# kspalaiologos/bzip3

Hardware: AMD Instinct MI355X
Metric: MiB/s encode+decode round-trip, 8 MiB blocks (higher is better)
Workload: dtype u8

## Files before the change

bzip3_amd/__init__.py:

```python
import ctypes as C
import os

_HERE = os.path.dirname(os.path.abspath(__file__))
LIB_PATH = os.path.join(_HERE, "lib", "libbzip3.so")

BZ3_OK = 0
BZ3_ERR_OUT_OF_BOUNDS = -1
BZ3_ERR_BWT = -2
BZ3_ERR_CRC = -3
BZ3_ERR_MALFORMED_HEADER = -4
BZ3_ERR_TRUNCATED_DATA = -5
BZ3_ERR_DATA_TOO_BIG = -6
BZ3_ERR_INIT = -7
BZ3_ERR_DATA_SIZE_TOO_SMALL = -8

T_NAMES = ["crc", "rle", "lzp", "bwt", "cm", "copy", "_6", "_7"]

_lib = None


def _declare(L, strict=True):
    vp, i32, u32, sz = C.c_void_p, C.c_int32, C.c_uint32, C.c_size_t
    sig = {
        "bz3_version": (C.c_char_p, []),
        "bz3_last_error": (C.c_int8, [vp]),
        "bz3_strerror": (C.c_char_p, [vp]),
        "bz3_new": (vp, [i32]),
        "bz3_free": (None, [vp]),
        "bz3_bound": (sz, [sz]),
        "bz3_compress": (C.c_int, [u32, vp, vp, sz, C.POINTER(sz)]),
        "bz3_decompress": (C.c_int, [vp, vp, sz, C.POINTER(sz)]),
        "bz3_min_memory_needed": (sz, [i32]),
        "bz3_encode_block": (i32, [vp, vp, i32]),
        "bz3_decode_block": (i32, [vp, vp, sz, i32, i32]),
        "bz3_encode_blocks": (None, [vp, vp, vp, i32]),
        "bz3_decode_blocks": (None, [vp, vp, vp, vp, vp, i32]),
        "bz3_orig_size_sufficient_for_decode": (C.c_int, [vp, sz, i32]),
        "bz3_hip_device_count": (C.c_int, []),
        "bz3_hip_bind_device": (C.c_int, [C.c_int]),
        "bz3_hip_state_device": (C.c_int, [vp]),
        "bz3_hip_set_cm_mode": (C.c_int, [C.c_int]),
        "bz3_hip_cm_blocks_given_up": (C.c_uint, []),
        "bz3_hip_cm_blocks_routed_full": (C.c_uint, []),
        "bz3_hip_debug_bwt_big_rounds": (None, [C.c_int]),
        "bz3_hip_debug_set_unbwt_log_stride": (None, [C.c_int]),
        "bz3_hip_debug_peak_concurrent_groups": (C.c_int, [C.c_int]),
        "bz3_hip_debug_front_end_ring": (C.c_int, []),
        "bz3_hip_debug_arena_swap_buffers": (C.c_int, [C.c_int]),
        "bz3_hip_cm_variant_for": (C.c_int, [C.c_int, C.c_int, C.c_int]),
        "bz3_hip_set_lean_states": (C.c_int, [C.c_int]),
        "bz3_hip_release_cached_memory": (None, []),
        "bz3_hip_set_keep_workspace": (C.c_int, [C.c_int]),
        "bz3_hip_set_front_end_duo": (C.c_int, [C.c_int]),
        "bz3_hip_set_workspace_headroom": (None, [C.c_longlong]),
        "bz3_hip_workspace_headroom": (sz, []),
        "bz3_hip_debug_headroom_events": (C.c_uint, [C.c_int, C.POINTER(C.c_uint)]),
        "bz3_hip_debug_ring_contexts": (sz, [sz, sz, sz, sz, sz, sz, C.c_int, sz]),
        "bz3_hip_debug_arena_slack": (sz, [sz]),
        "bz3_hip_debug_cm_launches": (C.c_uint, [C.c_int]),
        "bz3_hip_debug_workspace_bytes": (sz, [sz, C.c_int]),
        "bz3_hip_debug_cached_bytes": (sz, [C.c_int]),
        "bz3_hip_encode_block_device": (i32, [vp, vp, i32]),
        "bz3_hip_decode_block_device": (i32, [vp, vp, sz, i32, i32]),
        "bz3_hip_encode_blocks_device": (None, [vp, vp, vp, i32]),
        "bz3_hip_decode_blocks_device": (None, [vp, vp, vp, vp, vp, i32]),
        "bz3_hip_compress_device": (C.c_int, [u32, vp, vp, sz, C.POINTER(sz)]),
        "bz3_hip_decompress_device": (C.c_int, [vp, vp, sz, C.POINTER(sz)]),
        "bz3_hip_frame_decoded_size_device": (C.c_int, [vp, sz, C.POINTER(sz)]),
        "bz3_hip_compress_device_many": (C.c_int, [u32, i32, C.POINTER(vp), C.POINTER(sz), C.POINTER(vp), C.POINTER(sz), C.POINTER(C.c_int)]),
        "bz3_hip_decompress_device_many": (C.c_int, [i32, C.POINTER(vp), C.POINTER(sz), C.POINTER(vp), C.POINTER(sz), C.POINTER(C.c_int)]),
        "bz3_hip_frame_decoded_sizes_device": (C.c_int, [i32, C.POINTER(vp), C.POINTER(sz), C.POINTER(sz), C.POINTER(C.c_int)]),
        "bz3_hip_debug_copy_segments": (i32, [vp, vp, C.POINTER(C.c_uint64), i32]),
        "bz3_hip_compress_device_planes": (C.c_int, [u32, u32, vp, vp, sz, C.POINTER(sz)]),
        "bz3_hip_decompress_device_planes": (C.c_int, [u32, vp, vp, sz, C.POINTER(sz)]),
        "bz3_hip_compress_device_planes_many": (C.c_int, [u32, i32, C.POINTER(u32), C.POINTER(vp), C.POINTER(sz), C.POINTER(vp), C.POINTER(sz), C.POINTER(C.c_int)]),
        "bz3_hip_decompress_device_planes_many": (C.c_int, [i32, C.POINTER(u32), C.POINTER(vp), C.POINTER(sz), C.POINTER(vp), C.POINTER(sz), C.POINTER(C.c_int)]),
        "bz3_hip_debug_planes": (i32, [vp, vp, C.POINTER(C.c_uint64), i32]),
        "bz3_hip_compress_device_delta": (C.c_int, [u32, u32, vp, vp, vp, sz, C.POINTER(sz)]),
        "bz3_hip_decompress_device_delta": (C.c_int, [u32, vp, vp, sz, vp, sz, C.POINTER(sz)]),
        "bz3_hip_compress_device_delta_many": (C.c_int, [u32, i32, C.POINTER(u32), C.POINTER(vp), C.POINTER(vp), C.POINTER(sz), C.POINTER(vp), C.POINTER(sz), C.POINTER(C.c_int)]),
        "bz3_hip_decompress_device_delta_many": (C.c_int, [i32, C.POINTER(u32), C.POINTER(vp), C.POINTER(sz), C.POINTER(vp), C.POINTER(sz), C.POINTER(vp), C.POINTER(sz), C.POINTER(C.c_int)]),
        "bz3_hip_crc32c_device": (C.c_int, [vp, sz, u32, C.POINTER(u32)]),
        "bz3_hip_crc32c_device_many": (C.c_int, [i32, C.POINTER(vp), C.POINTER(sz), C.POINTER(u32), C.POINTER(u32)]),
        "bz3_hip_debug_crc_launches": (C.c_uint, [C.c_int]),
        "bz3_hip_debug_delta": (i32, [vp, vp, vp, C.POINTER(C.c_uint64), i32]),
        "bz3_hip_decompress_device_range": (C.c_int, [u32, vp, sz, C.c_uint64, vp, sz, vp, C.POINTER(sz)]),
        "bz3_hip_decompress_device_range_many": (C.c_int, [i32, C.POINTER(u32), C.POINTER(vp), C.POINTER(sz), C.POINTER(C.c_uint64), C.POINTER(vp), C.POINTER(sz),
                                                           C.POINTER(vp), C.POINTER(sz), C.POINTER(C.c_int)]),
        "bz3_hip_debug_range": (i32, [vp, vp, vp, C.POINTER(C.c_uint64), i32]),
        "bz3_hip_decompress_device_strided": (C.c_int, [u32, vp, sz, C.c_uint64, C.c_uint64, C.c_uint64, C.c_uint64, vp, sz, vp, C.POINTER(sz)]),
        "bz3_hip_decompress_device_strided_many": (C.c_int, [i32, C.POINTER(u32), C.POINTER(vp), C.POINTER(sz), C.POINTER(C.c_uint64), C.POINTER(vp), C.POINTER(sz),
                                                             C.POINTER(vp), C.POINTER(sz), C.POINTER(C.c_int)]),
        "bz3_hip_debug_strided": (i32, [vp, vp, vp, C.POINTER(C.c_uint64), i32]),
        "bz3_hip_decompress_device_select": (C.c_int, [u32, vp, sz, C.c_uint64, C.c_uint64, C.c_uint64, C.c_uint64, C.POINTER(C.c_uint64), vp, sz, vp, C.POINTER(sz)]),
        "bz3_hip_decompress_device_select_many": (C.c_int, [i32, C.POINTER(u32), C.POINTER(vp), C.POINTER(sz), C.POINTER(C.c_uint64), C.POINTER(C.POINTER(C.c_uint64)),
                                                            C.POINTER(vp), C.POINTER(sz), C.POINTER(vp), C.POINTER(sz), C.POINTER(C.c_int)]),
        "bz3_hip_debug_select": (i32, [vp, vp, vp, C.POINTER(C.c_uint64), i32, C.POINTER(C.c_uint64), C.c_uint64]),
        "bz3_hip_update_device_range": (C.c_int, [u32, vp, sz, C.c_uint64, vp, sz, vp, vp, C.POINTER(sz)]),
        "bz3_hip_update_device_range_many": (C.c_int, [i32, C.POINTER(u32), C.POINTER(vp), C.POINTER(sz), C.POINTER(C.c_uint64), C.POINTER(vp), C.POINTER(sz), C.POINTER(vp),
                                                       C.POINTER(vp), C.POINTER(sz), C.POINTER(C.c_int)]),
        "bz3_hip_debug_patch": (i32, [vp, vp, vp, C.POINTER(C.c_uint64), i32]),
        "bz3_hip_last_timings": (None, [vp, C.POINTER(C.c_float)]),
        "bz3_hip_last_bwt_stats": (None, [vp, C.POINTER(i32), C.POINTER(i32), C.POINTER(C.c_uint64)]),
        "bz3_hip_stage_crc32c": (u32, [vp, sz, u32]),
        "bz3_hip_stage_mrle_encode": (i32, [vp, i32, vp]),
        "bz3_hip_stage_mrle_decode": (C.c_int, [vp, vp, i32, i32]),
        "bz3_hip_stage_lzp_encode": (i32, [vp, i32, vp]),
        "bz3_hip_stage_lzp_decode": (i32, [vp, i32, vp, i32]),
        "bz3_hip_debug_lzp_encode": (i32, [vp, i32, vp, vp]),
        "bz3_hip_stage_bwt": (i32, [vp, vp, i32]),
        "bz3_hip_stage_unbwt": (i32, [vp, vp, i32, i32]),
        "bz3_hip_debug_unbwt_many": (i32, [vp, vp, vp, vp, i32]),
        "bz3_hip_debug_bwt_many": (i32, [vp, vp, vp, vp, i32]),
        "bz3_hip_debug_set_bwt_batch": (None, [C.c_int]),
        "bz3_hip_stage_last_ms": (C.c_float, []),
        "bz3_hip_debug_sort_u32": (i32, [vp, u32, C.c_int, C.c_int, vp, vp]),
        "bz3_hip_debug_scan_u32": (i32, [vp, u32, vp]),
        "bz3_hip_debug_cu_masks": (i32, [C.c_int, C.c_int, vp, vp]),
        "bz3_hip_set_collect_window_us": (None, [C.c_int]),
        "bz3_hip_debug_collected_batches": (C.c_uint, [C.c_int, C.POINTER(C.c_uint)]),
        "bz3_hip_stage_cm_encode": (i32, [vp, i32, vp]),
        "bz3_hip_stage_cm_decode": (None, [vp, i32, vp, i32]),
        "bz3_hip_stage_cm_decode_many": (C.c_float, [vp, i32, vp, i32, i32, vp]),
        "bz3_hip_stage_cm_encode_many": (C.c_float, [vp, i32, vp, C.POINTER(i32), i32]),
        "bz3_hip_encode_stream": (C.c_int, [C.c_int, C.c_int, i32, i32]),
        "bz3_hip_decode_stream": (C.c_int, [C.c_int, C.c_int, i32]),
    }
    for name, (res, args) in sig.items():
        if not strict and not hasattr(L, name):
            continue
        fn = getattr(L, name)
        fn.restype = res
        fn.argtypes = args
    return L


EXPORTED_SYMBOLS = None


def _share_hip_runtime_with_torch():
    if os.environ.get("BZ3_HIP_SYSTEM_RUNTIME") == "1":
        return
    try:
        import importlib.util

        spec = importlib.util.find_spec("torch")
        if spec is None or not spec.origin:
            return
        cand = os.path.join(os.path.dirname(spec.origin), "lib", "libamdhip64.so")
        if os.path.exists(cand):
            C.CDLL(cand, mode=C.RTLD_GLOBAL)
    except Exception:
        pass


def load(path=None):
    global _lib
    if _lib is not None and path is None:
        return _lib
    if path is None:
        _share_hip_runtime_with_torch()
    p = path or LIB_PATH
    if not os.path.exists(p):
        raise RuntimeError(
            f"{p} is missing: the HIP extension has not been built (python -m bzip3_amd.build). "
            "bzip3_amd has no CPU or PyTorch fallback by design."
        )
    L = _declare(C.CDLL(p), strict=path is None)
    if path is None:
        _lib = L
    return L


def _cbuf(data, cap):
    cap = max(1, cap)
    if len(data) == cap:
        return (C.c_uint8 * cap).from_buffer_copy(data)
    buf = (C.c_uint8 * cap)()
    if len(data):
        C.memmove(buf, data if isinstance(data, bytes) else bytes(data), len(data))
    return buf


class StageApi:

    def __init__(self, lib=None):
        self.lib = lib or load()

    def crc32c(self, data, init=1):
        return self.lib.bz3_hip_stage_crc32c(_cbuf(data, len(data)), len(data), init)

    def mrle_encode(self, data):
        out = (C.c_uint8 * (len(data) + 64))()
        n = self.lib.bz3_hip_stage_mrle_encode(_cbuf(data, len(data)), len(data), out)
        return C.string_at(out, n)

    def mrle_decode(self, data, outlen, maxin=None):
        maxin = len(data) if maxin is None else maxin
        out = (C.c_uint8 * max(1, outlen))()
        rc = self.lib.bz3_hip_stage_mrle_decode(_cbuf(data, len(data)), out, outlen, maxin)
        return rc, C.string_at(out, outlen)

    def lzp_encode(self, data):
        out = (C.c_uint8 * (len(data) + 64))()
        n = self.lib.bz3_hip_stage_lzp_encode(_cbuf(data, len(data)), len(data), out)
        return n, (C.string_at(out, n) if n > 0 else b"")

    def lzp_encode_stats(self, data):
        out = (C.c_uint8 * (len(data) + 64))()
        st = (C.c_uint32 * 6)()
        n = self.lib.bz3_hip_debug_lzp_encode(_cbuf(data, len(data)), len(data), out, st)
        keys = ("end_pos", "n_matches", "iterations", "evaluated", "event_cap", "window_positions")
        return n, (C.string_at(out, n) if n > 0 else b""), dict(zip(keys, (int(x) for x in st)))

    def lzp_decode(self, data, maxout):
        out = (C.c_uint8 * max(8, maxout))()
        n = self.lib.bz3_hip_stage_lzp_decode(_cbuf(data, len(data)), len(data), out, maxout)
        return n, (C.string_at(out, n) if n > 0 else b"")

    def bwt(self, data):
        out = (C.c_uint8 * max(1, len(data)))()
        idx = self.lib.bz3_hip_stage_bwt(_cbuf(data, len(data)), out, len(data))
        return idx, C.string_at(out, len(data))

    def unbwt(self, data, idx):
        out = (C.c_uint8 * max(1, len(data)))()
        rc = self.lib.bz3_hip_stage_unbwt(_cbuf(data, len(data)), out, len(data), idx)
        return rc, C.string_at(out, len(data))

    def bwt_many(self, blocks):
        k = len(blocks)
        ins = [_cbuf(d, len(d)) for d in blocks]
        outs = [(C.c_uint8 * max(1, len(d)))() for d in blocks]
        inp = (C.c_void_p * max(1, k))(*[C.cast(b, C.c_void_p) for b in ins])
        outp = (C.c_void_p * max(1, k))(*[C.cast(b, C.c_void_p) for b in outs])
        n = (C.c_int32 * max(1, k))(*[len(d) for d in blocks])
        idx = (C.c_int32 * max(1, k))()
        rc = self.lib.bz3_hip_debug_bwt_many(inp, outp, n, idx, k)
        return rc, [(int(i), C.string_at(o, len(d))) for i, o, d in zip(idx, outs, blocks)]

    def unbwt_many(self, jobs):
        k = len(jobs)
        ins = [_cbuf(d, len(d)) for d, _ in jobs]
        outs = [(C.c_uint8 * max(1, len(d)))() for d, _ in jobs]
        inp = (C.c_void_p * max(1, k))(*[C.cast(b, C.c_void_p) for b in ins])
        outp = (C.c_void_p * max(1, k))(*[C.cast(b, C.c_void_p) for b in outs])
        n = (C.c_int32 * max(1, k))(*[len(d) for d, _ in jobs])
        idx = (C.c_int32 * max(1, k))(*[i for _, i in jobs])
        rc = self.lib.bz3_hip_debug_unbwt_many(inp, outp, n, idx, k)
        return rc, [C.string_at(o, len(d)) for o, (d, _) in zip(outs, jobs)]

    def cm_encode(self, data):
        out = (C.c_uint8 * (len(data) + len(data) // 50 + 64))()
        n = self.lib.bz3_hip_stage_cm_encode(_cbuf(data, len(data)), len(data), out)
        return C.string_at(out, n)

    def cm_decode(self, data, n):
        out = (C.c_uint8 * max(1, n))()
        self.lib.bz3_hip_stage_cm_decode(_cbuf(data, len(data)), len(data), out, n)
        return C.string_at(out, n)


class State:

    def __init__(self, block_size, lib=None):
        self.lib = lib or load()
        self.block_size = block_size
        self.ptr = self.lib.bz3_new(block_size)
        if not self.ptr:
            raise RuntimeError(f"bz3_new({block_size}) returned NULL (invalid size, no HIP device, or out of device memory)")

    def close(self):
        if self.ptr:
            self.lib.bz3_free(self.ptr)
            self.ptr = None

    def __del__(self):
        try:
            self.close()
        except Exception:
            pass

    def __enter__(self):
        return self

    def __exit__(self, *a):
        self.close()

    @property
    def last_error(self):
        return self.lib.bz3_last_error(self.ptr)

    def strerror(self):
        return self.lib.bz3_strerror(self.ptr).decode()

    def timings(self):
        t = (C.c_float * 8)()
        self.lib.bz3_hip_last_timings(self.ptr, t)
        return {T_NAMES[i]: t[i] for i in range(6)}

    def bwt_stats(self):
        r, p, e = C.c_int32(), C.c_int32(), C.c_uint64()
        self.lib.bz3_hip_last_bwt_stats(self.ptr, C.byref(r), C.byref(p), C.byref(e))
        return {"rounds": r.value, "radix_passes": p.value, "sorted_elements": e.value}

    def encode_block(self, data):
        cap = self.lib.bz3_bound(max(len(data), self.block_size)) + 64
        buf = _cbuf(data, cap)
        n = self.lib.bz3_encode_block(self.ptr, buf, len(data))
        return n, self.last_error, (C.string_at(buf, n) if n > 0 else b"")

    def decode_block(self, data, orig_size, buffer_size=None, comp_size=None):
        cap = self.lib.bz3_bound(self.block_size) + 64
        buffer_size = cap if buffer_size is None else buffer_size
        comp_size = len(data) if comp_size is None else comp_size
        buf = _cbuf(data, max(cap, buffer_size, len(data) + 1))
        n = self.lib.bz3_decode_block(self.ptr, buf, buffer_size, comp_size, orig_size)
        return n, self.last_error, (C.string_at(buf, n) if n > 0 else b"")


def encode_block(data, block_size, lib=None):
    with State(block_size, lib) as st:
        return st.encode_block(data)


def decode_block(data, orig_size, block_size, lib=None, **kw):
    with State(block_size, lib) as st:
        return st.decode_block(data, orig_size, **kw)


class Bz3Error(RuntimeError):

    def __init__(self, code, what, out=None, index=None, codes=None, outs=None):
        super().__init__(f"{what} failed with {code} ({_ERR_NAMES.get(code, 'unknown error')})" + ("" if index is None else f" at frame {index}"))
        self.code = code
        self.out = out
        self.index = index
        self.codes = codes
        self.outs = outs


_ERR_NAMES = {v: k for k, v in globals().items() if k.startswith("BZ3_ERR_")}


def _device_u8(x, what):
    import torch

    if not isinstance(x, torch.Tensor) or x.device.type != "cuda" or x.dtype != torch.uint8 or not x.is_contiguous():
        raise TypeError(f"{what} must be a contiguous torch.uint8 tensor on a GPU")
    return x


def _planes_arg(planes, n):
    ks = [int(planes)] * n if isinstance(planes, int) else [int(k) for k in planes]
    if len(ks) != n:
        raise ValueError(f"planes: {len(ks)} element sizes for {n} tensors")
    for k in ks:
        if k not in (1, 2, 4, 8):
            raise ValueError(f"planes must be 1, 2, 4 or 8, not {k}")
    return ks


def _base_u8(base, x, what, same_size=True):
    if base is None:
        return None
    base = _device_u8(base, what)
    if base.device != x.device:
        raise ValueError(f"{what} is on {base.device}, the tensor on {x.device}")
    if same_size and base.numel() != x.numel():
        raise ValueError(f"{what} holds {base.numel()} bytes, the tensor {x.numel()}")
    return base


def _bases_arg(bases, n):
    bases = [None] * n if bases is None else list(bases)
    if len(bases) != n:
        raise ValueError(f"bases: {len(bases)} entries for {n} tensors")
    return bases


def _ptrs_or_null(ts):
    return (C.c_void_p * len(ts))(*[None if t is None else t.data_ptr() for t in ts])


def compress_tensor(x, block_size=16 << 20, lib=None, planes=1, base=None):
    import torch

    x = _device_u8(x, "x")
    (k,) = _planes_arg(planes, 1)
    base = _base_u8(base, x, "base")
    L = lib or load()
    n = x.numel()
    out = torch.empty(L.bz3_bound(n), dtype=torch.uint8, device=x.device)
    size = C.c_size_t(out.numel())
    torch.cuda.synchronize(x.device)
    rc = L.bz3_hip_compress_device_delta(block_size, k, C.c_void_p(x.data_ptr()), None if base is None else C.c_void_p(base.data_ptr()),
                                         C.c_void_p(out.data_ptr()), n, C.byref(size))
    if rc != BZ3_OK:
        raise Bz3Error(rc, "bz3_hip_compress_device_delta")
    return out[: size.value]


def decompress_tensor(frame, out=None, lib=None, planes=1, base=None):
    import torch

    frame = _device_u8(frame, "frame")
    (k,) = _planes_arg(planes, 1)
    base = _base_u8(base, frame, "base", same_size=False)
    L = lib or load()
    torch.cuda.synchronize(frame.device)
    if out is None:
        need = C.c_size_t(0)
        L.bz3_hip_frame_decoded_size_device(C.c_void_p(frame.data_ptr()), frame.numel(), C.byref(need))
        out = torch.empty(need.value, dtype=torch.uint8, device=frame.device)
    else:
        out = _device_u8(out, "out")
    size = C.c_size_t(out.numel())
# ... 947 lines not shown
```

bzip3_amd/csrc/api_context.hip:

```cpp
#include "api_internal.hpp"

using namespace bz3;
using namespace bz3::api;

namespace {

std::mutex g_mu;
std::vector<DeviceCtx *> g_ctx;
int g_device_count = -1;
std::atomic<int> g_bound_device{-2};
std::atomic<unsigned> g_rr{0};
std::atomic<unsigned> g_headroom_trims{0}, g_headroom_releases{0};

#ifndef BZ3_EMU
__attribute__((constructor)) static void bz3_hip_on_load() {
    const char * e = getenv("BZ3_HIP_SET_HW_QUEUES");
    if (!e || atoi(e) != 0) (void)setenv("GPU_MAX_HW_QUEUES", "8", 0);
}
#endif

}

namespace bz3 {
namespace api {

std::atomic<int> g_lean{-1};
std::atomic<int> g_front_end_ring{0};
std::atomic<int> g_arena_swaps{0};
std::atomic<unsigned> g_cm_given_up{0};
std::atomic<unsigned> g_crc_launches{0};
std::atomic<unsigned> g_cm_launches{0};
std::atomic<unsigned> g_cm_routed_full{0};
std::atomic<int> g_cm_mode{-2};
std::atomic<long long> g_ws_headroom{-1};
std::atomic<int> g_keep_ws{-1};
std::atomic<int> g_front_duo{-1};
std::atomic<int> g_groups_running{0}, g_groups_peak{0};
Collector g_collect;
std::atomic<int> g_collect_window_us{200};
std::atomic<unsigned> g_collect_batches{0}, g_collect_largest{0};

void DeviceCtx::cu_masks(int cus, int reserve, std::vector<uint32_t> & side, std::vector<uint32_t> & main) {
    const int words = (cus + 31) / 32;
    side.assign((size_t)words, 0u);
    main.assign((size_t)words, 0u);
    for (int i = 0; i < cus; i++) main[(size_t)(i >> 5)] |= 1u << (i & 31);
    const int per = reserve / 8 > 0 ? reserve / 8 : 1;
    for (int a = 0; a < 8 && a * 32 < cus; a++)
        for (int t = 0; t < per && t < 8; t++) {
            const int j = t & 3;
            const int i = 32 * a + 8 * j + ((a + 2 * j + (t >> 2)) & 7);
            if (i < cus) {
                side[(size_t)(i >> 5)] |= 1u << (i & 31);
                main[(size_t)(i >> 5)] &= ~(1u << (i & 31));
            }
        }
}

void DeviceCtx::ensure_aux() {
    if (aux_ready) return;
    hipStream_t st[AUX] = {}, sm[AUX] = {}, rs = nullptr, du = nullptr;
    hipEvent_t e0[AUX] = {}, e1[AUX] = {}, ep = nullptr;
    int reserved = 0, device_cus = 0;
    try {
        HIP_CHECK(hipEventCreate(&ep));
#ifndef BZ3_EMU
        const int want = cu_reserve_setting();
        int real_cus = 0;
        if (hipDeviceGetAttribute(&real_cus, hipDeviceAttributeMultiprocessorCount, device) != hipSuccess) real_cus = 0;
        if (want >= 8 && real_cus >= 64 && real_cus % 32 == 0) {
            std::vector<uint32_t> side, mainm;
            cu_masks(real_cus, want, side, mainm);
            bool ok = hipExtStreamCreateWithCUMask(&rs, (uint32_t)mainm.size(), mainm.data()) == hipSuccess;
            for (int k = 0; ok && k < RING_SLOTS; k++) ok = hipExtStreamCreateWithCUMask(&sm[k], (uint32_t)side.size(), side.data()) == hipSuccess;
            if (!ok) {
                (void)hipGetLastError();
                if (rs) (void)hipStreamDestroy(rs);
                rs = nullptr;
                for (int k = 0; k < AUX; k++) {
                    if (sm[k]) (void)hipStreamDestroy(sm[k]);
                    sm[k] = nullptr;
                }
            } else {
                for (uint32_t wd : side) reserved += __builtin_popcount(wd);
                device_cus = real_cus;
            }
        }
#endif
        for (int k = 0; k < AUX; k++) {
            HIP_CHECK(hipStreamCreateWithFlags(&st[k], hipStreamNonBlocking));
            HIP_CHECK(hipEventCreate(&e0[k]));
            HIP_CHECK(hipEventCreate(&e1[k]));
        }
        HIP_CHECK(hipStreamCreateWithFlags(&du, hipStreamNonBlocking));
    } catch (...) {
        if (du) (void)hipStreamDestroy(du);
        if (ep) (void)hipEventDestroy(ep);
        if (rs) (void)hipStreamDestroy(rs);
        for (int k = 0; k < AUX; k++)
            if (sm[k]) (void)hipStreamDestroy(sm[k]);
        for (int k = 0; k < AUX; k++) {
            if (st[k]) (void)hipStreamDestroy(st[k]);
            if (e0[k]) (void)hipEventDestroy(e0[k]);
            if (e1[k]) (void)hipEventDestroy(e1[k]);
        }
        throw;
    }
    ev_prep = ep;
    duo = du;
    rest = rs;
    for (int k = 0; k < AUX; k++) aux_m[k] = sm[k];
    reserved_cus = reserved;
    real_cus = device_cus;
    for (int k = 0; k < AUX; k++) {
        aux[k] = st[k];
        ev_d0[k] = e0[k];
        ev_d1[k] = e1[k];
    }
    aux_ready = true;
}

u8 * DeviceCtx::temp_get(size_t cap) {
    std::lock_guard<std::mutex> lk(temp_mu);
    for (size_t k = 0; k < temps_free.size(); k++)
        if (temps_free[k].second >= cap) {
            auto t = temps_free[k];
            temps_free.erase(temps_free.begin() + (long)k);
            temps_out.push_back(t);
            return t.first;
        }
    u8 * p = nullptr;
    if (hipMalloc((void **)&p, cap) != hipSuccess) {
        (void)hipGetLastError();
        (void)hipDeviceSynchronize();
        for (auto & t : temps_free) (void)hipFree(t.first);
        temps_free.clear();
        HIP_CHECK(hipMalloc((void **)&p, cap));
    }
    temps_out.push_back({p, cap});
    return p;
}

void DeviceCtx::temp_put(u8 * p) {
    if (!p) return;
    std::lock_guard<std::mutex> lk(temp_mu);
    for (size_t k = 0; k < temps_out.size(); k++)
        if (temps_out[k].first == p) {
            temps_free.push_back(temps_out[k]);
            temps_out.erase(temps_out.begin() + (long)k);
            return;
        }
}

void DeviceCtx::temp_trim() {
    std::lock_guard<std::mutex> lk(temp_mu);
    if (temps_free.empty()) return;
    (void)hipDeviceSynchronize();
    for (auto & t : temps_free) (void)hipFree(t.first);
    temps_free.clear();
}

size_t DeviceCtx::temp_idle_bytes() {
    std::lock_guard<std::mutex> lk(temp_mu);
    size_t b = 0;
    for (auto & t : temps_free) b += t.second;
    return b;
}

Arena DeviceCtx::arena_for(size_t bytes) {
    if (bytes > ws_cap) {
        if (ws) HIP_CHECK(hipFree(ws));
        ws = nullptr;
        ws_cap = 0;
        size_t want = bytes + arena_slack(bytes);
        HIP_CHECK(hipMalloc((void **)&ws, want));
        ws_cap = want;
    }
    Arena a;
    a.base = ws;
    a.cap = ws_cap;
    a.used = 0;
    return a;
}

int device_count() {
    std::lock_guard<std::mutex> lk(g_mu);
    if (g_device_count < 0) {
        int n = 0;
        if (hipGetDeviceCount(&n) != hipSuccess) n = 0;
        g_device_count = n;
        g_ctx.assign((size_t)(n > 0 ? n : 0), nullptr);
    }
    return g_device_count;
}

DeviceCtx * get_ctx(int dev) {
    const int n = device_count();
    if (dev < 0 || dev >= n) return nullptr;
    std::lock_guard<std::mutex> lk(g_mu);
    if (!g_ctx[dev]) {
        HIP_CHECK(hipSetDevice(dev));
        DeviceCtx * c = new DeviceCtx;
        c->device = dev;
        CrcTables t;
        memset(&t, 0, sizeof t);
        crc_build_tables(t);
        HIP_CHECK(hipMalloc((void **)&c->d_crc, sizeof(CrcTables)));
        HIP_CHECK(hipMemcpy(c->d_crc, &t, sizeof t, hipMemcpyHostToDevice));
#ifndef BZ3_EMU
        int cus = 0;
        if (hipDeviceGetAttribute(&cus, hipDeviceAttributeMultiprocessorCount, dev) == hipSuccess && cus > 0) c->cus = cus;
#endif
        if (const char * e = getenv("BZ3_HIP_CUS"))
            if (atoi(e) > 0) c->cus = atoi(e);
        g_ctx[dev] = c;
    }
    return g_ctx[dev];
}

int pick_device() {
    const int n = device_count();
    if (n <= 0) return -1;
    int b = g_bound_device.load();
    if (b == -2) {
        const char * e = getenv("BZ3_HIP_DEVICE");
        b = (e && *e) ? atoi(e) : -1;
        if (b >= n) b = -1;
        g_bound_device.store(b);
    }
    if (b >= 0) return b;
    return (int)(g_rr.fetch_add(1) % (unsigned)n);
}

void enforce_headroom(DeviceCtx * ctx, hipStream_t s) {
    const size_t h = ws_headroom();
    size_t free_b = 0, total_b = 0;
    if (!h || hipMemGetInfo(&free_b, &total_b) != hipSuccess || free_b >= h) return;
    if (ctx->temp_idle_bytes() > 0) {
        ctx->temp_trim();
        g_headroom_trims.fetch_add(1);
        if (hipMemGetInfo(&free_b, &total_b) != hipSuccess || free_b >= h) return;
    }
    if (ctx->ws) {
        (void)hipStreamSynchronize(s);
        (void)hipDeviceSynchronize();
        (void)hipFree(ctx->ws);
        ctx->ws = nullptr;
        ctx->ws_cap = 0;
        g_headroom_releases.fetch_add(1);
    }
}

void state_release(bz3_state * st) {
    if (!st) return;
    (void)hipSetDevice(st->device);
    if (st->stream) (void)hipStreamSynchronize(st->stream);
    if (st->ev0) (void)hipEventDestroy(st->ev0);
    if (st->ev1) (void)hipEventDestroy(st->ev1);
    if (st->d_swap && st->lean && st->ctx) st->ctx->temp_put(st->d_swap);
    else if (st->d_swap) (void)hipFree(st->d_swap);
    if (st->d_io) (void)hipFree(st->d_io);
    if (st->d_words) (void)hipFree(st->d_words);
    if (st->stream) (void)hipStreamDestroy(st->stream);
    delete st;
}

bz3_state * new_state_on(int32_t block_size, int dev) {
    if (block_size < KiB65 || block_size > MiB511) return nullptr;
    bz3_state * st = nullptr;
    try {
        DeviceCtx * ctx = get_ctx(dev);
        if (!ctx) return nullptr;
        st = new bz3_state;
        st->block_size = block_size;
        st->device = dev;
        st->ctx = ctx;
        HIP_CHECK(hipSetDevice(dev));
        HIP_CHECK(hipStreamCreateWithFlags(&st->stream, hipStreamNonBlocking));
        st->xs = st->stream;
        HIP_CHECK(hipEventCreate(&st->ev0));
        HIP_CHECK(hipEventCreate(&st->ev1));
        st->cap = (bz3_bound((size_t)block_size) + 4096 + 255) & ~(size_t)255;
        st->lean = lean_states();
        if (!st->lean) HIP_CHECK(hipMalloc((void **)&st->d_swap, st->cap));
        HIP_CHECK(hipMalloc((void **)&st->d_words, 64 * sizeof(u32)));
        st->last_error = BZ3_OK;
        return st;
    } catch (const HipError & e) {
        fprintf(stderr, "bzip3_amd: bz3_new failed: %s (%s:%d)\n", e.what, e.file, e.line);
        state_release(st);
        return nullptr;
    } catch (const std::bad_alloc &) {
        state_release(st);
        return nullptr;
    }
}

}
}

extern "C" {

BZIP3_API unsigned bz3_hip_cm_blocks_routed_full(void) { return g_cm_routed_full.load(); }
BZIP3_API void bz3_hip_set_workspace_headroom(long long bytes) { g_ws_headroom.store(bytes < 0 ? -1 : bytes); }
BZIP3_API size_t bz3_hip_workspace_headroom(void) { return ws_headroom(); }
BZIP3_API unsigned bz3_hip_debug_headroom_events(int reset, unsigned * releases) {
    const unsigned t = reset ? g_headroom_trims.exchange(0) : g_headroom_trims.load();
    const unsigned r = reset ? g_headroom_releases.exchange(0) : g_headroom_releases.load();
    if (releases) *releases = r;
    return t;
}
BZIP3_API size_t bz3_hip_debug_ring_contexts(size_t free_b, size_t have, size_t need, size_t fixed, size_t ctx_bytes, size_t cap, int lean, size_t headroom) {
    return ring_contexts_for(free_b, have, need, fixed, ctx_bytes, cap, lean != 0, headroom);
}
BZIP3_API size_t bz3_hip_debug_workspace_bytes(size_t block_bytes, int which) {
    return which == 0 ? workspace_bytes_for((u64)block_bytes + 64) : lzp_encode_ctx_bytes((u64)block_bytes + 64) + 65536;
}
BZIP3_API unsigned bz3_hip_debug_cm_launches(int reset) { return reset ? g_cm_launches.exchange(0) : g_cm_launches.load(); }
BZIP3_API size_t bz3_hip_debug_arena_slack(size_t bytes) { return DeviceCtx::arena_slack(bytes); }
BZIP3_API size_t bz3_hip_debug_cached_bytes(int device) {
    DeviceCtx * c = nullptr;
    {
        std::lock_guard<std::mutex> lk(g_mu);
        if (device >= 0 && (size_t)device < g_ctx.size()) c = g_ctx[(size_t)device];
    }
    if (!c) return 0;
    std::lock_guard<std::mutex> lk(c->mu);
    return c->ws_cap + c->temp_idle_bytes();
}
BZIP3_API int bz3_hip_set_front_end_duo(int on) {
    g_front_duo.store(on < 0 ? -1 : (on ? 1 : 0));
    return 0;
}
BZIP3_API int bz3_hip_set_keep_workspace(int on) {
    g_keep_ws.store(on < 0 ? -1 : (on ? 1 : 0));
    return 0;
}
BZIP3_API void bz3_hip_set_collect_window_us(int us) { g_collect_window_us.store(us < 0 ? 200 : us); }
BZIP3_API unsigned bz3_hip_debug_collected_batches(int reset, unsigned * largest) {
// ... 83 lines not shown
```

bzip3_amd/csrc/api_encode.hip:

```cpp
#include "api_internal.hpp"

using namespace bz3;
using namespace bz3::api;

namespace {

__global__ void k_write_header(u8 * __restrict__ b, const u32 * __restrict__ crc, const u32 * __restrict__ idx_word, u32 model, u32 lzp_size, u32 rle_size) {
    if (threadIdx.x != 0) return;
    const u32 c = *crc, idx = *idx_word;
    b[0] = (u8)c; b[1] = (u8)(c >> 8); b[2] = (u8)(c >> 16); b[3] = (u8)(c >> 24);
    b[4] = (u8)idx; b[5] = (u8)(idx >> 8); b[6] = (u8)(idx >> 16); b[7] = (u8)(idx >> 24);
    b[8] = (u8)model;
    u32 o = 9;
    if (model & 2u) { b[o] = (u8)lzp_size; b[o + 1] = (u8)(lzp_size >> 8); b[o + 2] = (u8)(lzp_size >> 16); b[o + 3] = (u8)(lzp_size >> 24); o += 4; }
    if (model & 4u) { b[o] = (u8)rle_size; b[o + 1] = (u8)(rle_size >> 8); b[o + 2] = (u8)(rle_size >> 16); b[o + 3] = (u8)(rle_size >> 24); }
}

__global__ void __launch_bounds__(64) k_store_small(u8 * __restrict__ b, u32 n, const u32 * __restrict__ crc) {
    const u32 t = threadIdx.x;
    const u8 v = t < n ? b[t] : (u8)0;
    __syncthreads();
    if (t < n) b[8 + t] = v;
    if (t == 0) {
        const u32 c = *crc;
        b[0] = (u8)c; b[1] = (u8)(c >> 8); b[2] = (u8)(c >> 16); b[3] = (u8)(c >> 24);
        b[4] = b[5] = b[6] = b[7] = 0xFF;
    }
}

void encode_front_a(bz3_state * st, u8 * buf, s32 data_size, Arena & arena, Arena & ctx_arena, LzpEncodeCtx & c) {
    st->pending = bz3_state::FAILED;
    st->result = -1;
    c.active = false;
    if (st->skip) return;
    if (data_size > st->block_size || data_size < 0) {
        st->last_error = BZ3_ERR_DATA_TOO_BIG;
        return;
    }
    hipStream_t s = st->xs;
    for (float & x : st->t) x = 0.f;
    double t0 = now_ms();
    crc32c_device(buf, (u64)data_size, 1u, st->ctx->d_crc, st->d_words, s);
    st->user = buf;
    st->size = data_size;
    if (data_size < 64) {
        launch(k_store_small, dim3(1), dim3(64), 0, s, buf, (u32)data_size, (const u32 *)(st->d_words + 1));
        st->pending = bz3_state::ENC_STORED;
        return;
    }
    if (st->timed) {
        HIP_CHECK(hipStreamSynchronize(s));
        st->t[BZ3_HIP_T_CRC] = (float)(now_ms() - t0);
    }

    u32 n = (u32)data_size;
    lean_borrow(st);
    u8 *b1 = buf, *b2 = st->d_swap;
    st->model = 0;
    st->rle_size = 0;
    t0 = now_ms();
    {
        MrleEncScratch sc;
        const size_t mk = arena.mark();
        mrle_encode_size(b1, n, sc, arena, s);
        st->rle_size = (s32)(32u + read_word(s, sc.total));
        if (st->rle_size < (s32)n) {
            mrle_encode_write(b1, n, sc, b2, s);
            if (st->timed) HIP_CHECK(hipStreamSynchronize(s));
            u8 * tmp = b1; b1 = b2; b2 = tmp;
            n = (u32)st->rle_size;
            st->model |= 4;
        }
        arena.release(mk);
    }
    st->t[BZ3_HIP_T_RLE] = (float)(now_ms() - t0);
    st->b1 = b1;
    st->b2 = b2;
    st->n_cm = n;
    t0 = now_ms();
    lzp_encode_prepare(b1, n, c, ctx_arena, arena, s);
    st->t[BZ3_HIP_T_LZP] = (float)(now_ms() - t0);
    st->pending = bz3_state::ENC_CODED;
}

bool encode_front_b_collect(bz3_state * st, Arena & arena, const LzpEncodeCtx & c, float driver_ms, BwtBatchItem & item, u8 *& copy_to) {
    if (st->pending != bz3_state::ENC_CODED) return false;
    st->pending = bz3_state::FAILED;
    hipStream_t s = st->xs;
    u8 *b1 = st->b1, *b2 = st->b2;
    u32 n = st->n_cm;
    double t0 = now_ms();
    const s32 lzp_size = lzp_encode_finish(c, b2, arena, s);
    if (lzp_size > 0 && lzp_size < (s32)n) {
        u8 * tmp = b1; b1 = b2; b2 = tmp;
        n = (u32)lzp_size;
        st->model |= 2;
    }
    st->lzp_size = lzp_size;
    st->t[BZ3_HIP_T_LZP] += driver_ms + (float)(now_ms() - t0);

    u32 * const d_idx = st->d_words + 6;
    u32 * const d_out8 = st->d_words + 8;
    copy_to = nullptr;
    if (!st->lean) {
        item = BwtBatchItem{b1, n, b2, d_idx, d_out8, &st->bwt, 0};
    } else {
        u8 * tail = st->user + bz3_bound((size_t)st->size) - n;
        if (b1 != st->user) {
            item = BwtBatchItem{b1, n, tail, d_idx, d_out8, &st->bwt, 0};
        } else {
            item = BwtBatchItem{b1, n, b2, d_idx, d_out8, &st->bwt, 0};
            copy_to = tail;
        }
    }
    st->b1 = b1;
    st->b2 = b2;
    st->n_cm = n;
    return true;
}

void encode_front_b_transform(bz3_state * const * owners, BwtBatchItem * items, size_t count, Arena & arena, hipStream_t s) {
    std::vector<u32> sizes(count);
    for (size_t k = 0; k < count; k++) sizes[k] = items[k].n;
    for (size_t at = 0; at < count;) {
        const double t0 = now_ms();
        u32 b = 1;
        if (items[at].n < 2) {
            (void)bwt_forward(items[at].in, items[at].n, items[at].out, arena, s, items[at].stats, items[at].d_idx, items[at].d_outside);
        } else {
            u32 avail = 0;
            while (at + avail < count && avail < BWT_MAX_BATCH && items[at + avail].n >= 2) avail++;
            b = bwt_batch_size(sizes.data() + at, avail, arena.cap - arena.used);
            bwt_forward_batch(items + at, b, arena, s);
        }
        bool timed = false;
        for (u32 k = 0; k < b; k++) timed = timed || owners[at + k]->timed;
        if (timed) {
            HIP_CHECK(hipStreamSynchronize(s));
            const float each = (float)(now_ms() - t0) / (float)b;
            for (u32 k = 0; k < b; k++)
                if (owners[at + k]->timed) owners[at + k]->t[BZ3_HIP_T_BWT] = each;
        }
        at += b;
    }
}

void encode_front_b_header(bz3_state * st, const BwtBatchItem & item, u8 * copy_to) {
    hipStream_t s = st->xs;
    u8 *b1 = st->b1, *b2 = st->b2;
    const u32 n = st->n_cm;
    if (st->lean) {
        if (copy_to) HIP_CHECK(hipMemcpyAsync(copy_to, b2, n, hipMemcpyDeviceToDevice, s));
        b2 = copy_to ? copy_to : item.out;
        b1 = st->user;
    }
    s32 overhead = 2;
    if (st->model & 2) overhead++;
    if (st->model & 4) overhead++;
    launch(k_write_header, dim3(1), dim3(64), 0, s, b1, (const u32 *)(st->d_words + 1), (const u32 *)item.d_idx, (u32)st->model, (u32)st->lzp_size, (u32)st->rle_size);
    if (st->lean && !st->hold_swap) lean_return(st);
    st->b1 = b1;
    st->b2 = b2;
    st->overhead = overhead;
    st->pending = bz3_state::ENC_CODED;
}

void encode_finish(bz3_state * st, float cm_ms) {
    const bz3_state::Pending p = st->pending;
    st->pending = bz3_state::NONE;
    if (p == bz3_state::FAILED || p == bz3_state::NONE) return;
    HIP_CHECK(hipStreamSynchronize(st->xs));
    if (p == bz3_state::ENC_STORED) {
        st->result = st->size + 8;
        return;
    }
    st->t[BZ3_HIP_T_CM] = cm_ms;
    const u32 coded = read_word(st->xs, st->d_words + 2);
    if (coded == 0xFFFFFFFFu) {
        st->last_error = BZ3_ERR_BWT;
        return;
    }
    const s32 total = (s32)coded + st->overhead * 4 + 1;
    if (st->lean) {
        const u32 sw = read_word(st->xs, st->d_words + 3);
        if (sw != 0xFFFFFFFFu && coded > sw)
            HIP_CHECK(hipMemcpyAsync(st->user + st->overhead * 4 + 1 + sw, st->side, coded - sw, hipMemcpyDeviceToDevice, st->xs));
        HIP_CHECK(hipStreamSynchronize(st->xs));
    }
    st->last_error = BZ3_OK;
    if (st->b1 != st->user) {
        double t0 = now_ms();
        HIP_CHECK(hipMemcpyAsync(st->user, st->b1, (size_t)total, hipMemcpyDeviceToDevice, st->xs));
        HIP_CHECK(hipStreamSynchronize(st->xs));
        st->t[BZ3_HIP_T_COPY] += (float)(now_ms() - t0);
    }
    st->result = total;
}

void pipeline_shape(s32 contexts, s32 n, s32 & window, s32 & ns) {
    if (contexts < 2) contexts = 2;
    ns = 2;
    for (s32 cand = DeviceCtx::RING_SLOTS; cand > 2; cand--)
        if (contexts / cand >= 3 && n >= cand * 3) {
            ns = cand;
            break;
        }
    window = contexts / ns;
    if (window > 8) window = 8;
    if (const char * e = getenv("BZ3_HIP_LZP_PIPE")) {
        int w = 0, q = 0;
        if (sscanf(e, "%d,%d", &w, &q) == 2 && w >= 1 && q >= 2 && q <= DeviceCtx::AUX) {
            window = w;
            ns = q;
        }
    }
    if (window > n) window = n;
    if (window < 1) window = 1;
}

}

namespace bz3 {
namespace api {

void encode_group(bz3_state ** sts, u8 ** bufs, const s32 * sizes, s32 n) {
    if (n <= 0) return;
    bz3_state * lead = sts[0];
    DeviceGuard g(lead->device);
    std::lock_guard<std::mutex> lk(lead->ctx->mu);
    for (s32 i = 0; i < n; i++) {
        sts[i]->xs = lead->stream;
        sts[i]->timed = i == 0;
    }
    size_t need = 0, need_a = 0, need_b = 0;
    for (s32 i = 0; i < n; i++) {
        const u64 nb = (u64)(sizes[i] > 0 ? sizes[i] : 0) + 64;
        const size_t w = workspace_bytes_for(nb), wa = front_a_scratch_bytes(nb), wb = front_b_scratch_bytes(nb);
        if (w > need) need = w;
        if (wa > need_a) need_a = wa;
        if (wb > need_b) need_b = wb;
    }
    const bool duo_wanted = front_end_duo() && n >= 16;
    if (duo_wanted) need = need_a + need_b + 65536;
    u64 n_max = 64;
    for (s32 i = 0; i < n; i++)
        if (sizes[i] > 0 && (u64)sizes[i] > n_max) n_max = (u64)sizes[i];
    const size_t ctx_bytes = lzp_encode_ctx_bytes(n_max + 64) + 65536;
    const size_t headroom = ws_headroom();
    const size_t fixed = (size_t)n * (sizeof(CmEncodeJob) + CM_SIDE_BYTES + 256) + cm_scratch_bytes((size_t)n) + 65536 + (size_t)DeviceCtx::AUX * 8 * (sizeof(LzpDriverJob) + 256);
    size_t bwt_extra = 0;
    if (n > 1) {
        const u32 sz[BWT_MAX_BATCH] = {(u32)n_max, (u32)n_max, (u32)n_max, (u32)n_max};
        const u32 b = bwt_batch_size(sz, (u32)(n < (s32)BWT_MAX_BATCH ? n : (s32)BWT_MAX_BATCH), ~(size_t)0);
        bwt_extra = (size_t)(b - 1) * bwt_workspace_bytes(n_max + 64);
    }
    size_t contexts = ((size_t)32 << 30) / ctx_bytes, contexts_beside_runs = contexts;
    {
        size_t free_b = 0, total_b = 0;
        const s32 full = DeviceCtx::RING_SLOTS * 8;
        if (lead->lean && lead->ctx->temp_idle_bytes() > 0 && hipMemGetInfo(&free_b, &total_b) == hipSuccess) {
            if (ring_contexts_for(free_b, lead->ctx->ws_cap, need, fixed, ctx_bytes, lead->cap, true, headroom) < (size_t)(n < full ? n : full)) lead->ctx->temp_trim();
        }
        if (hipMemGetInfo(&free_b, &total_b) == hipSuccess) {
            contexts = ring_contexts_for(free_b, lead->ctx->ws_cap, need, fixed, ctx_bytes, lead->cap, lead->lean, headroom);
            contexts_beside_runs = ring_contexts_for(free_b, lead->ctx->ws_cap, need + bwt_extra, fixed, ctx_bytes, lead->cap, lead->lean, headroom);
        }
    }
    s32 window = 1, ns = 2;
    pipeline_shape((s32)(contexts < 1024 ? contexts : 1024), n, window, ns);
    if (contexts_beside_runs < (size_t)ns * (size_t)window) bwt_extra = 0;
    lead->ctx->ensure_aux();
    hipStream_t s = lead->stream;
    DrainOnUnwind drain{s, lead->ctx->aux, DeviceCtx::AUX};
    static const bool front_rest = [] { const char * e = getenv("BZ3_HIP_FRONT_REST"); return e && atoi(e) != 0; }();
    if (front_rest && lead->ctx->rest && n > 1) {
        s = lead->ctx->rest;
        for (s32 i = 0; i < n; i++) sts[i]->xs = s;
    }
    DrainOnUnwind drain_rest{s == lead->stream ? nullptr : s, nullptr, 0};
    Arena arena;
    for (;;) {
        try {
            arena = lead->ctx->arena_for(need + bwt_extra + (size_t)ns * (size_t)window * (ctx_bytes + sizeof(LzpDriverJob) + 256) +
                                         (size_t)n * (sizeof(CmEncodeJob) + CM_SIDE_BYTES + 256) + cm_scratch_bytes((size_t)n) + 65536);
            break;
        } catch (const HipError &) {
            if (ns == 2 && window == 1 && bwt_extra == 0) throw;
            (void)hipGetLastError();
            if (bwt_extra) bwt_extra = 0;
            else if (ns > 2) ns = 2;
            else window = (window + 1) / 2;
        }
    }
    g_front_end_ring.store(window | (ns << 16));
    CmEncodeJob * d_jobs = arena.take<CmEncodeJob>((size_t)n);
    u8 * sides = arena.take<u8>((size_t)n * CM_SIDE_BYTES);
    struct Window {
        s32 w0 = 0, w1 = 0;
        Arena slot;
        LzpDriverJob * d_lz = nullptr;
        std::vector<LzpEncodeCtx> ctxs;
        std::vector<LzpDriverJob> lz;
    } win[DeviceCtx::AUX];
    for (int k = 0; k < ns; k++) {
        win[k].slot.base = arena.take<char>((size_t)window * ctx_bytes);
        win[k].slot.cap = (size_t)window * ctx_bytes;
        win[k].d_lz = arena.take<LzpDriverJob>((size_t)window);
    }
    std::vector<CmEncodeJob> jobs;
    std::vector<s32> job_owner;
    std::vector<BwtBatchItem> fb_items;
    std::vector<bz3_state *> fb_owner;
    std::vector<u8 *> fb_copy;
    std::vector<s32> fb_slot;
    const s32 nwin = (n + window - 1) / window;
    const s32 lag = ns - 1;
    static const bool trace_rings = getenv("BZ3_HIP_TRACE_RINGS") != nullptr;
    double tr_prep = 0, tr_wait = 0, tr_fin = 0, tr_t0 = now_ms();
    auto prepare = [&](s32 k, hipStream_t sp, Arena & scr, hipEvent_t ev) {
        const int q = (int)(k % ns);
        Window & w = win[q];
        w.w0 = k * window;
        w.w1 = (w.w0 + window < n) ? w.w0 + window : n;
        w.slot.used = 0;
        w.ctxs.assign((size_t)(w.w1 - w.w0), LzpEncodeCtx());
        w.lz.clear();
        for (s32 i = w.w0; i < w.w1; i++) {
            sts[i]->xs = sp;
            sts[i]->hold_swap = false;
            encode_front_a(sts[i], bufs[i], sizes[i], scr, w.slot, w.ctxs[(size_t)(i - w.w0)]);
            if (sts[i]->pending == bz3_state::ENC_CODED && w.ctxs[(size_t)(i - w.w0)].active) w.lz.push_back(lzp_driver_job(w.ctxs[(size_t)(i - w.w0)]));
        }
        HIP_CHECK(hipEventRecord(ev, sp));
        if (!w.lz.empty()) {
            hipStream_t sq = lead->ctx->aux[q];
            HIP_CHECK(hipStreamWaitEvent(sq, ev, 0));
            HIP_CHECK(hipEventRecord(lead->ctx->ev_d0[q], sq));
            lzp_driver_batch(w.lz.data(), w.d_lz, (u32)w.lz.size(), sq);
            HIP_CHECK(hipEventRecord(lead->ctx->ev_d1[q], sq));
        }
    };
    auto finish = [&](s32 j, hipStream_t sf, Arena & scr, std::vector<bz3_state *> * held) {
        const int q = (int)(j % ns);
        Window & w = win[q];
        float driver_ms = 0.f;
        if (!w.lz.empty()) {
            const double t0 = now_ms();
            HIP_CHECK(hipEventSynchronize(lead->ctx->ev_d1[q]));
            (void)hipEventElapsedTime(&driver_ms, lead->ctx->ev_d0[q], lead->ctx->ev_d1[q]);
            tr_wait += now_ms() - t0;
        }
        fb_items.clear();
        fb_owner.clear();
        fb_copy.clear();
        fb_slot.assign((size_t)(w.w1 - w.w0), -1);
        for (s32 i = w.w0; i < w.w1; i++) {
            sts[i]->xs = sf;
            BwtBatchItem item{};
            u8 * copy_to = nullptr;
            if (encode_front_b_collect(sts[i], scr, w.ctxs[(size_t)(i - w.w0)], driver_ms, item, copy_to)) {
                fb_slot[(size_t)(i - w.w0)] = (s32)fb_items.size();
                fb_items.push_back(item);
                fb_owner.push_back(sts[i]);
                fb_copy.push_back(copy_to);
            }
        }
        encode_front_b_transform(fb_owner.data(), fb_items.data(), fb_items.size(), scr, sf);
        for (s32 i = w.w0; i < w.w1; i++) {
            const s32 slot = fb_slot[(size_t)(i - w.w0)];
            if (slot >= 0) {
                sts[i]->hold_swap = held != nullptr;
                encode_front_b_header(sts[i], fb_items[(size_t)slot], fb_copy[(size_t)slot]);
                sts[i]->hold_swap = false;
            }
            if (sts[i]->pending == bz3_state::ENC_CODED) {
                CmEncodeJob j2{dev_addr(sts[i]->b2), dev_addr(sts[i]->b1 + sts[i]->overhead * 4 + 1), dev_addr(sts[i]->d_words + 2), sts[i]->n_cm, 0u};
                if (sts[i]->lean) {
                    sts[i]->side = sides + (size_t)i * CM_SIDE_BYTES;
                    j2.gap = (u32)(sts[i]->b2 - (sts[i]->b1 + sts[i]->overhead * 4 + 1));
                    j2.side = dev_addr(sts[i]->side);
                    j2.side_cap = CM_SIDE_BYTES;
                }
                jobs.push_back(j2);
                job_owner.push_back(i);
            }
            if (held) {
                if (sts[i]->lean && sts[i]->d_swap) held->push_back(sts[i]);
            } else {
                lean_return(sts[i]);
            }
        }
    };
    const bool duo = duo_wanted && nwin >= 3 && lead->ctx->aux_ready && s == lead->stream;
    if (!duo) {
        for (s32 k = 0; k < nwin + lag; k++) {
            const double tr_a = now_ms();
            if (k < nwin) prepare(k, s, arena, lead->ctx->ev_prep);
            const double tr_b = now_ms();
            tr_prep += tr_b - tr_a;
            if (k >= lag) finish(k - lag, s, arena, nullptr);
            tr_fin += now_ms() - tr_b;
        }
    } else {
        g_front_end_ring.fetch_or(1 << 29);
        hipStream_t sA = lead->ctx->duo;
        DrainOnUnwind drain_duo{sA, nullptr, 0};
        Arena scr_a;
        scr_a.base = arena.take<char>(need_a);
        scr_a.cap = need_a;
        struct Events {
            std::vector<hipEvent_t> e;
            ~Events() {
                for (hipEvent_t x : e)
                    if (x) (void)hipEventDestroy(x);
            }
        } evs;
        evs.e.assign((size_t)2 * (size_t)nwin, nullptr);
        for (auto & x : evs.e) HIP_CHECK(hipEventCreateWithFlags(&x, hipEventDisableTiming));
        hipEvent_t * evA = evs.e.data(), * evB = evs.e.data() + nwin;
        struct Shared {
            std::mutex m;
            std::condition_variable cv;
            s32 prepared = 0, finished = 0;
            bool abort = false;
            std::exception_ptr err;
            std::mutex pool;
            hipEvent_t last_return = nullptr;
            double prep_ms = 0;
        } sh;
        const int device = lead->device;
        std::thread ta([&] {
            try {
                DeviceGuard gd(device);
                for (s32 k = 0; k < nwin; k++) {
                    {
                        std::unique_lock<std::mutex> ul(sh.m);
                        sh.cv.wait(ul, [&] { return sh.abort || sh.finished >= k - ns + 1; });
                        if (sh.abort) return;
                    }
                    const double t0 = now_ms();
                    if (k >= ns) HIP_CHECK(hipStreamWaitEvent(sA, evB[k - ns], 0));
                    {
                        hipEvent_t ev = nullptr;
                        const s32 w0 = k * window, w1 = (w0 + window < n) ? w0 + window : n;
                        {
                            std::lock_guard<std::mutex> pl(sh.pool);
                            for (s32 i = w0; i < w1; i++) lean_borrow(sts[i]);
                            ev = sh.last_return;
                        }
                        if (ev) HIP_CHECK(hipStreamWaitEvent(sA, ev, 0));
                    }
                    prepare(k, sA, scr_a, evA[k]);
                    {
                        std::lock_guard<std::mutex> ul(sh.m);
                        sh.prepared = k + 1;
                        sh.prep_ms += now_ms() - t0;
                    }
                    sh.cv.notify_all();
                }
            } catch (...) {
                {
                    std::lock_guard<std::mutex> ul(sh.m);
                    sh.err = std::current_exception();
                    sh.abort = true;
                }
                sh.cv.notify_all();
            }
        });
        struct Joiner {
            std::thread & t;
            Shared & sh;
            int live = std::uncaught_exceptions();
            ~Joiner() {
                if (std::uncaught_exceptions() > live) {
                    std::lock_guard<std::mutex> ul(sh.m);
                    sh.abort = true;
                }
                sh.cv.notify_all();
                if (t.joinable()) t.join();
            }
        } joiner{ta, sh};
        std::vector<bz3_state *> held;
        for (s32 j = 0; j < nwin; j++) {
            const double tr_b = now_ms();
            {
                std::unique_lock<std::mutex> ul(sh.m);
                sh.cv.wait(ul, [&] { return sh.abort || sh.prepared >= j + 1; });
                if (sh.abort) break;
            }
            HIP_CHECK(hipStreamWaitEvent(s, evA[j], 0));
            held.clear();
            finish(j, s, arena, &held);
            HIP_CHECK(hipEventRecord(evB[j], s));
            {
                std::lock_guard<std::mutex> pl(sh.pool);
                for (bz3_state * st : held) lean_return(st);
                sh.last_return = evB[j];
            }
            {
                std::lock_guard<std::mutex> ul(sh.m);
                sh.finished = j + 1;
            }
            sh.cv.notify_all();
            tr_fin += now_ms() - tr_b;
        }
        ta.join();
        if (sh.err) std::rethrow_exception(sh.err);
        HIP_CHECK(hipStreamSynchronize(sA));
        tr_prep = sh.prep_ms;
        for (s32 i = 0; i < n; i++) sts[i]->xs = s;
    }
    if (trace_rings)
        fprintf(stderr, "[bz3 rings] encode front end: %d blocks, %d windows of %d x %d slots: %.1f ms = CRC / mRLE / LZP prepare %.1f + waiting for a window's LZP drivers %.1f + LZP emit / BWT / header %.1f\n",
                (int)n, (int)nwin, (int)window, (int)ns, now_ms() - tr_t0, tr_prep, tr_wait, tr_fin - tr_wait);
    if (s != lead->stream) {
        HIP_CHECK(hipStreamSynchronize(s));
        s = lead->stream;
        for (s32 i = 0; i < n; i++) sts[i]->xs = s;
    }
    std::vector<char> to_full(jobs.size(), 0);
    if (jobs.size() > (size_t)lead->ctx->cus) {
        std::vector<u32> outside(jobs.size(), 0u);
        for (size_t k = 0; k < jobs.size(); k++) HIP_CHECK(hipMemcpyAsync(&outside[k], sts[job_owner[k]]->d_words + 8, 4, hipMemcpyDeviceToHost, lead->stream));
        HIP_CHECK(hipStreamSynchronize(lead->stream));
        for (size_t k = 0; k < jobs.size(); k++) to_full[k] = outside[k] > jobs[k].n / 4u ? 1 : 0;
    }
    const float cm_ms = run_cm_jobs(lead->ctx, arena, jobs, d_jobs, lead->stream, lead->ev0, lead->ev1,
                                    [](const CmEncodeJob * j, u32 nj, hipStream_t st, int variant) { cm_encode_batch(j, nj, st, variant); }, &to_full);
    for (s32 i = 0; i < n; i++) encode_finish(sts[i], cm_ms);
    size_t slack = (size_t)16 << 30;
    if (const char * e = getenv("BZ3_HIP_WS_KEEP_MB")) slack = (size_t)strtoull(e, nullptr, 10) << 20;
    if (lead->ctx->ws_cap > 2 * need + slack && !(keep_workspace() && lead->lean)) {
        HIP_CHECK(hipStreamSynchronize(s));
        (void)hipFree(lead->ctx->ws);
        lead->ctx->ws = nullptr;
        lead->ctx->ws_cap = 0;
        g_front_end_ring.fetch_or(1 << 30);
    }
    enforce_headroom(lead->ctx, lead->stream);
}

}
}
```

bzip3_amd/csrc/api_hooks.hip:

```cpp
#include "api_internal.hpp"

using namespace bz3;
using namespace bz3::api;

namespace {

struct StageEnv {
    DeviceCtx * ctx = nullptr;
    hipStream_t s = nullptr;
    std::vector<void *> allocs;
    std::unique_lock<std::mutex> lock;
    StageEnv() {
        int dev = pick_device();
        if (dev < 0) {
            fprintf(stderr, "bzip3_amd: no HIP device available -- this library has no CPU code path\n");
            abort();
        }
        ctx = get_ctx(dev);
        HIP_CHECK(hipSetDevice(dev));
        HIP_CHECK(hipStreamCreateWithFlags(&s, hipStreamNonBlocking));
        lock = std::unique_lock<std::mutex>(ctx->mu);
    }
    ~StageEnv() {
        (void)hipStreamSynchronize(s);
        for (void * p : allocs) (void)hipFree(p);
        (void)hipStreamDestroy(s);
    }
    u8 * dev(size_t bytes, const void * init = nullptr, size_t init_bytes = 0) {
        void * p = nullptr;
        HIP_CHECK(hipMalloc(&p, bytes + 4096));
        allocs.push_back(p);
        if (init && init_bytes) HIP_CHECK(hipMemcpy(p, init, init_bytes, hipMemcpyHostToDevice));
        return (u8 *)p;
    }
    void down(void * host, const void * d, size_t bytes) {
        HIP_CHECK(hipStreamSynchronize(s));
        if (bytes) HIP_CHECK(hipMemcpy(host, d, bytes, hipMemcpyDeviceToHost));
    }
    u32 word(const u32 * d) {
        u32 v = 0;
        down(&v, d, 4);
        return v;
    }
};

template <typename F>
auto stage_guard(F && f) -> decltype(f()) {
    try {
        return f();
    } catch (const HipError & e) {
        fprintf(stderr, "bzip3_amd: HIP failure '%s' at %s:%d\n", e.what, e.file, e.line);
        abort();
    }
}

}

extern "C" {

BZIP3_API uint32_t bz3_hip_stage_crc32c(const uint8_t * data, size_t n, uint32_t init) {
    return stage_guard([&]() -> u32 {
        StageEnv e;
        u8 * d = e.dev(n + 16, data, n);
        u32 * w = (u32 *)e.dev(64);
        crc32c_device(d, n, init, e.ctx->d_crc, w, e.s);
        return e.word(w + 1);
    });
}

BZIP3_API int32_t bz3_hip_stage_mrle_encode(const uint8_t * in, int32_t n, uint8_t * out) {
    return stage_guard([&]() -> s32 {
        StageEnv e;
        u8 * d = e.dev((size_t)n + 16, in, (size_t)n);
        u8 * o = e.dev((size_t)n + 64);
        Arena a = e.ctx->arena_for(workspace_bytes_for((u64)n + 64));
        MrleEncScratch sc;
        mrle_encode_size(d, (u32)n, sc, a, e.s);
        const s32 size = (s32)(32u + e.word(sc.total));
        mrle_encode_write(d, (u32)n, sc, o, e.s);
        e.down(out, o, (size_t)size);
        return size;
    });
}

BZIP3_API int bz3_hip_stage_mrle_decode(const uint8_t * in, uint8_t * out, int32_t outlen, int32_t maxin) {
    return stage_guard([&]() -> int {
        if (maxin < 32) return 1;
        StageEnv e;
        u8 * d = e.dev((size_t)maxin + 16, in, (size_t)maxin);
        u8 * o = e.dev((size_t)outlen + 64);
        u32 * w = (u32 *)e.dev(64);
        Arena a = e.ctx->arena_for(workspace_bytes_for((u64)maxin + 64));
        mrle_decode(d, (u32)maxin, o, (u32)outlen, w, a, e.s);
        const u32 got = e.word(w);
        e.down(out, o, (size_t)(got < (u32)outlen ? got : (u32)outlen));
        return got != (u32)outlen;
    });
}

BZIP3_API int32_t bz3_hip_stage_lzp_encode(const uint8_t * in, int32_t n, uint8_t * out) {
    return stage_guard([&]() -> s32 {
        StageEnv e;
        u8 * d = e.dev((size_t)n + 64, in, (size_t)n);
        u8 * o = e.dev((size_t)n + 64);
        Arena a = e.ctx->arena_for(workspace_bytes_for((u64)n + 64));
        const s32 r = lzp_encode(d, (u32)n, o, a, e.s);
        if (r > 0) e.down(out, o, (size_t)r);
        return r;
    });
}

BZIP3_API int32_t bz3_hip_debug_lzp_encode(const uint8_t * in, int32_t n, uint8_t * out, uint32_t stats[6]) {
    return stage_guard([&]() -> s32 {
        StageEnv e;
        u8 * d = e.dev((size_t)n + 64, in, (size_t)n);
        u8 * o = e.dev((size_t)n + 64);
        Arena a = e.ctx->arena_for(workspace_bytes_for((u64)n + 64));
        LzDriverOut drv;
        const s32 r = lzp_encode(d, (u32)n, o, a, e.s, &drv);
        if (r > 0) e.down(out, o, (size_t)r);
        if (stats) {
            stats[0] = drv.end_pos;
            stats[1] = drv.n_matches;
            stats[2] = drv.iterations;
            stats[3] = drv.evaluated;
            lzp_driver_geometry(stats[4], stats[5]);
        }
        return r;
    });
}

BZIP3_API int32_t bz3_hip_stage_lzp_decode(const uint8_t * in, int32_t n, uint8_t * out, int32_t max) {
    return stage_guard([&]() -> s32 {
        StageEnv e;
        u8 * d = e.dev((size_t)n + 64, in, (size_t)n);
        u8 * o = e.dev((size_t)max + 64);
        Arena a = e.ctx->arena_for(workspace_bytes_for((u64)n + 64));
        if (n < 4) return -1;
        u32 * d_result = a.take<u32>(4);
        LzpDecodeJob job{dev_addr(d), dev_addr(o), dev_addr(a.take<u32>(LZP_LUT_WORDS)), dev_addr(d_result), (u32)n, (u32)max};
        LzpDecodeJob * d_job = a.take<LzpDecodeJob>(1);
        lzp_decode_batch(&job, d_job, 1, e.s);
        const s32 r = (s32)e.word(d_result);
        if (r > 0) e.down(out, o, (size_t)r);
        return r;
    });
}

static std::atomic<float> g_stage_ms{0.f};
BZIP3_API float bz3_hip_stage_last_ms(void) { return g_stage_ms.load(); }

BZIP3_API int32_t bz3_hip_stage_bwt(const uint8_t * in, uint8_t * out, int32_t n) {
    return stage_guard([&]() -> s32 {
        StageEnv e;
        u8 * d = e.dev((size_t)n + 64, in, (size_t)n);
        u8 * o = e.dev((size_t)n + 64);
        Arena a = e.ctx->arena_for(workspace_bytes_for((u64)n + 64));
        HIP_CHECK(hipStreamSynchronize(e.s));
        const auto t0 = std::chrono::steady_clock::now();
        const s32 idx = bwt_forward(d, (u32)n, o, a, e.s, nullptr);
        g_stage_ms.store(std::chrono::duration<float, std::milli>(std::chrono::steady_clock::now() - t0).count());
        e.down(out, o, (size_t)n);
        return idx;
    });
}

BZIP3_API int32_t bz3_hip_debug_bwt_many(const uint8_t * const * in, uint8_t * const * out, const int32_t * n, int32_t * idx_out, int32_t count) {
    return stage_guard([&]() -> s32 {
        if (count < 0 || (count > 0 && (!in || !out || !n || !idx_out))) return -1;
        u64 largest = 0;
        for (s32 k = 0; k < count; k++) {
            if (n[k] < 0) return -1;
            if ((u64)n[k] > largest) largest = (u64)n[k];
        }
        std::vector<BwtBatchItem> items;
        std::vector<u32> sizes;
        std::vector<s32> owner;
        StageEnv e;
        for (s32 k = 0; k < count; k++) {
            idx_out[k] = n[k];
            if (n[k] == 1) out[k][0] = in[k][0];
            if (n[k] < 2) continue;
            const u8 * d = e.dev((size_t)n[k] + 64, in[k], (size_t)n[k]);
            items.push_back(BwtBatchItem{d, (u32)n[k], e.dev((size_t)n[k] + 64), nullptr, nullptr, nullptr, 0});
            sizes.push_back((u32)n[k]);
            owner.push_back(k);
        }
        if (items.empty()) return 0;
        const size_t plain = workspace_bytes_for(largest + 64), full = (size_t)BWT_MAX_BATCH * bwt_workspace_bytes(largest + 64);
        Arena a = e.ctx->arena_for(plain > full ? plain : full);
        HIP_CHECK(hipStreamSynchronize(e.s));
        const auto t0 = std::chrono::steady_clock::now();
        for (size_t at = 0; at < items.size();) {
            const u32 b = bwt_batch_size(sizes.data() + at, (u32)(items.size() - at), a.cap - a.used);
            bwt_forward_batch(items.data() + at, b, a, e.s);
            at += b;
        }
        g_stage_ms.store(std::chrono::duration<float, std::milli>(std::chrono::steady_clock::now() - t0).count());
        for (size_t j = 0; j < items.size(); j++) {
            e.down(out[owner[j]], items[j].out, (size_t)items[j].n);
            idx_out[owner[j]] = items[j].idx;
        }
        return 0;
    });
}
BZIP3_API void bz3_hip_debug_set_bwt_batch(int b) { bwt_set_batch(b); }

BZIP3_API int32_t bz3_hip_stage_unbwt(const uint8_t * in, uint8_t * out, int32_t n, int32_t idx) {
    return stage_guard([&]() -> s32 {
        if (n < 0) return -1;
        if (n <= 1) {
            if (idx != n) return -1;
            if (n == 1) out[0] = in[0];
            return 0;
        }
        if (idx <= 0 || idx > n) return -1;
        StageEnv e;
        u8 * d = e.dev((size_t)n + 64, in, (size_t)n);
        u8 * o = e.dev((size_t)n + 64);
        Arena a = e.ctx->arena_for(workspace_bytes_for((u64)n + 64));
        HIP_CHECK(hipStreamSynchronize(e.s));
        const auto t0 = std::chrono::steady_clock::now();
        bwt_inverse(d, (u32)n, (u32)idx, o, a, e.s);
        HIP_CHECK(hipStreamSynchronize(e.s));
        g_stage_ms.store(std::chrono::duration<float, std::milli>(std::chrono::steady_clock::now() - t0).count());
        e.down(out, o, (size_t)n);
        return 0;
    });
}

BZIP3_API int32_t bz3_hip_debug_unbwt_many(const uint8_t * const * in, uint8_t * const * out, const int32_t * n, const int32_t * idx, int32_t count) {
    return stage_guard([&]() -> s32 {
        if (count < 0 || (count > 0 && (!in || !out || !n || !idx))) return -1;
        u64 largest = 0;
        for (s32 k = 0; k < count; k++) {
            if (n[k] < 0 || (n[k] <= 1 ? idx[k] != n[k] : (idx[k] <= 0 || idx[k] > n[k]))) return -1;
            if ((u64)n[k] > largest) largest = (u64)n[k];
        }
        std::vector<UbBatchItem> items;
        std::vector<u32> sizes;
        std::vector<s32> owner;
        StageEnv e;
        for (s32 k = 0; k < count; k++) {
            if (n[k] == 1) out[k][0] = in[k][0];
            if (n[k] < 2) continue;
            const u8 * d = e.dev((size_t)n[k] + 64, in[k], (size_t)n[k]);
            items.push_back(UbBatchItem{d, e.dev((size_t)n[k] + 64), (u32)n[k], (u32)idx[k]});
            sizes.push_back((u32)n[k]);
            owner.push_back(k);
        }
        if (items.empty()) return 0;
        const size_t plain = workspace_bytes_for(largest + 64), full = unbwt_batch_workspace_bytes(largest + 64, UB_MAX_BATCH);
        Arena a = e.ctx->arena_for(plain > full ? plain : full);
        HIP_CHECK(hipStreamSynchronize(e.s));
        const auto t0 = std::chrono::steady_clock::now();
        for (size_t at = 0; at < items.size();) {
            const u32 b = unbwt_batch_size(sizes.data() + at, (u32)(items.size() - at), a.cap - a.used, 0u);
            bwt_inverse_batch(items.data() + at, b, a, e.s);
            HIP_CHECK(hipStreamSynchronize(e.s));
            at += b;
        }
        g_stage_ms.store(std::chrono::duration<float, std::milli>(std::chrono::steady_clock::now() - t0).count());
        for (size_t j = 0; j < items.size(); j++) e.down(out[owner[j]], items[j].out, (size_t)items[j].n);
        return 0;
    });
}

BZIP3_API int32_t bz3_hip_debug_cu_masks(int cus, int reserve, uint32_t * side, uint32_t * rest) {
    if (cus < 32 || cus > 1024 || reserve < 8 || !side || !rest) return -1;
    std::vector<uint32_t> a, b;
    DeviceCtx::cu_masks(cus, reserve, a, b);
    for (size_t k = 0; k < a.size(); k++) {
        side[k] = a[k];
        rest[k] = b[k];
    }
    return (int32_t)a.size();
}

BZIP3_API int32_t bz3_hip_debug_scan_u32(uint32_t * data, uint32_t n, uint32_t * total) {
    return stage_guard([&]() -> s32 {
        if (n == 0) return -1;
        StageEnv e;
        u32 * d = (u32 *)e.dev((size_t)n * 4 + 64, data, (size_t)n * 4);
        u32 * t = (u32 *)e.dev(64);
        Arena a = e.ctx->arena_for(scan_temp_words(n) * 4 + (1u << 20));
        exclusive_scan_u32(d, n, t, a, e.s);
        e.down(data, d, (size_t)n * 4);
        if (total) *total = e.word(t);
        return 0;
    });
}

BZIP3_API int32_t bz3_hip_debug_sort_u32(const uint32_t * keys, uint32_t n, int key_bits, int digit_bits, uint32_t * sorted_keys, uint32_t * sorted_index) {
    return stage_guard([&]() -> s32 {
        if ((digit_bits != 8 && digit_bits != 9) || key_bits < 1 || key_bits > 32 || n == 0) return -1;
        StageEnv e;
        u32 * k[2] = {(u32 *)e.dev((size_t)n * 4 + 64, keys, (size_t)n * 4), (u32 *)e.dev((size_t)n * 4 + 64)};
        u32 * v[2] = {(u32 *)e.dev((size_t)n * 4 + 64), (u32 *)e.dev((size_t)n * 4 + 64)};
        Arena a = e.ctx->arena_for(radix_temp_bytes(n, digit_bits) + (1u << 20));
        int cur = 0, passes = 0;
        for (int shift = 0; shift < key_bits; shift += digit_bits, passes++) {
            const u32 * vin = passes ? v[cur] : nullptr;
            if (digit_bits == 9) radix_pass_bits<u32, 9>(k[cur], k[cur ^ 1], vin, v[cur ^ 1], n, shift, 0xFFFFFFFFu, 0u, a, e.s);
            else radix_pass<u32>(k[cur], k[cur ^ 1], vin, v[cur ^ 1], n, shift, 0xFFFFFFFFu, 0u, a, e.s);
            cur ^= 1;
        }
        e.down(sorted_keys, k[cur], (size_t)n * 4);
        e.down(sorted_index, v[cur], (size_t)n * 4);
        return passes;
    });
}

extern "C++" template <class Job, class Launch>
void stage_cm_job(StageEnv & e, Job job, Launch && go) {
    const int variant = cm_variant_for(e.ctx, 1, std::is_same<Job, CmEncodeJob>::value);
    u32 * status = nullptr;
    if (cm_variant_has_rows(variant)) {
        job.spill = dev_addr(e.dev(CM_SPILL_BYTES));
        status = (u32 *)e.dev(64);
        HIP_CHECK(hipMemsetAsync(status, 0, 64, e.s));
        job.status = dev_addr(status);
        job.miss_base = cm_variant_is_test(variant) ? 64u : CM_MISS_BASE;
        job.miss_shift = cm_variant_is_test(variant) ? 3u : CM_MISS_SHIFT;
    }
    Job * d_job = (Job *)e.dev(sizeof job, &job, sizeof job);
    go(d_job, 1u, e.s, variant);
    if (cm_variant_has_rows(variant) && e.word(status) != 0u) {
        g_cm_given_up.fetch_add(1u);
        go(d_job, 1u, e.s, (int)CM_VARIANT_FULL);
    }
}

BZIP3_API int32_t bz3_hip_stage_cm_encode(const uint8_t * in, int32_t n, uint8_t * out) {
    return stage_guard([&]() -> s32 {
        StageEnv e;
        u8 * d = e.dev((size_t)n + 64, in, (size_t)n);
        u8 * o = e.dev(bz3_bound((size_t)n) + 64);
        u32 * w = (u32 *)e.dev(64);
        const char * dbg = getenv("BZ3_CM_DEBUG");
        CmEncodeJob job{dev_addr(d), dev_addr(o), dev_addr(w), (u32)n, dbg ? (u32)atoi(dbg) : 0u};
        const char * tg = getenv("BZ3_CM_TEST_GAP");
        u8 * side = nullptr;
        if (tg) {
            const size_t g = (size_t)atol(tg);
            const char * ts = getenv("BZ3_CM_TEST_SIDE");
            const size_t side_cap = ts ? (size_t)atol(ts) : CM_SIDE_BYTES;
            u8 * both = e.dev(g + (size_t)n + 64);
            HIP_CHECK(hipMemcpy(both + g, d, (size_t)n, hipMemcpyDeviceToDevice));
            side = e.dev(side_cap + 64);
            o = both;
            job.in = dev_addr(both + g);
            job.out = dev_addr(both);
            job.gap = (u32)g;
            job.side = dev_addr(side);
            job.side_cap = (u32)side_cap;
        }
        stage_cm_job(e, job, [](const CmEncodeJob * j, u32 nj, hipStream_t st, int variant) { cm_encode_batch(j, nj, st, variant); });
        const u32 coded = e.word(w), sw = e.word(w + 1);
        if (coded == 0xFFFFFFFFu) return -1;
        const u32 head = (tg && sw < coded) ? sw : coded;
        e.down(out, o, (size_t)head);
        if (head < coded) e.down(out + head, side, (size_t)(coded - head));
        return (s32)coded;
    });
}

BZIP3_API void bz3_hip_stage_cm_decode(const uint8_t * in, int32_t in_size, uint8_t * out, int32_t n) {
    stage_guard([&]() -> int {
        StageEnv e;
        u8 * d = e.dev((size_t)in_size + 64, in, (size_t)in_size);
        u8 * o = e.dev((size_t)n + 64);
        const char * dbg = getenv("BZ3_CM_DEBUG");
        CmDecodeJob job{dev_addr(d), dev_addr(o), (u32)in_size, (u32)n, dbg ? (u32)atoi(dbg) : 0u, 0u};
        stage_cm_job(e, job, [](const CmDecodeJob * j, u32 nj, hipStream_t st, int variant) { cm_decode_batch(j, nj, st, variant); });
        e.down(out, o, (size_t)n);
        return 0;
    });
}

BZIP3_API float bz3_hip_stage_cm_decode_many(const uint8_t * in, int32_t in_size, uint8_t * out, int32_t n, int32_t copies, uint64_t * counters) {
    return stage_guard([&]() -> float {
        StageEnv e;
        if (copies < 1 || n < 256) return -1.f;
        u8 * d = e.dev((size_t)in_size + 64, in, (size_t)in_size);
        const size_t stride = ((size_t)n + 64 + 255) & ~(size_t)255;
        u8 * o = e.dev(stride * (size_t)copies);
        const char * dbg = getenv("BZ3_CM_DEBUG");
        const u32 debug = dbg ? (u32)atoi(dbg) : 0u;
        const int variant = cm_variant_for(e.ctx, (size_t)copies, false);
        u8 * spill = cm_variant_has_rows(variant) ? e.dev(CM_SPILL_BYTES * (size_t)copies) : nullptr;
        u32 * status = (u32 *)e.dev(4 * (size_t)copies + 64);
        HIP_CHECK(hipMemsetAsync(status, 0, 4 * (size_t)copies, e.s));
        std::vector<CmDecodeJob> jobs;
        for (int32_t k = 0; k < copies; k++) {
            CmDecodeJob j{dev_addr(d), dev_addr(o + stride * (size_t)k), (u32)in_size, (u32)n, debug, 0u};
            if (spill) {
                j.spill = dev_addr(spill + CM_SPILL_BYTES * (size_t)k);
                j.status = dev_addr(status + k);
                j.miss_base = CM_MISS_BASE;
                j.miss_shift = CM_MISS_SHIFT;
            }
            jobs.push_back(j);
        }
        CmDecodeJob * d_jobs = (CmDecodeJob *)e.dev(sizeof(CmDecodeJob) * jobs.size(), jobs.data(), sizeof(CmDecodeJob) * jobs.size());
        hipEvent_t e0, e1;
        HIP_CHECK(hipEventCreate(&e0));
        HIP_CHECK(hipEventCreate(&e1));
        HIP_CHECK(hipEventRecord(e0, e.s));
        cm_decode_batch(d_jobs, (u32)copies, e.s, variant, (debug & 15u) == 3u);
        HIP_CHECK(hipEventRecord(e1, e.s));
        HIP_CHECK(hipStreamSynchronize(e.s));
        float ms = 0.f;
        (void)hipEventElapsedTime(&ms, e0, e1);
        (void)hipEventDestroy(e0);
        (void)hipEventDestroy(e1);
        e.down(out, o, (size_t)n);
        if (counters)
            for (int32_t k = 0; k < copies; k++) e.down(counters + 16 * (size_t)k, o + stride * (size_t)k, 128);
        if (getenv("BZ3_CM_MANY_CHECK")) {
            std::vector<u8> other((size_t)n);
            for (int32_t k = 1; k < copies; k++) {
                e.down(other.data(), o + stride * (size_t)k, (size_t)n);
                if (memcmp(other.data(), out, (size_t)n) != 0) return -2.f;
            }
        }
        return ms;
    });
}

BZIP3_API float bz3_hip_stage_cm_encode_many(const uint8_t * in, int32_t n, uint8_t * out, int32_t * coded, int32_t copies) {
    return stage_guard([&]() -> float {
        StageEnv e;
        if (copies < 1 || n < 1) return -1.f;
        u8 * d = e.dev((size_t)n + 64, in, (size_t)n);
        const size_t stride = (bz3_bound((size_t)n) + 64 + 255) & ~(size_t)255;
        u8 * o = e.dev(stride * (size_t)copies);
        u32 * w = (u32 *)e.dev(16 * (size_t)copies + 64);
        const char * dbg = getenv("BZ3_CM_DEBUG");
        const u32 debug = dbg ? (u32)atoi(dbg) : 0u;
        const int variant = cm_variant_for(e.ctx, (size_t)copies, true);
        u8 * spill = cm_variant_has_rows(variant) ? e.dev(CM_SPILL_BYTES * (size_t)copies) : nullptr;
        u32 * status = (u32 *)e.dev(4 * (size_t)copies + 64);
        HIP_CHECK(hipMemsetAsync(status, 0, 4 * (size_t)copies, e.s));
        u32 * claim = getenv("BZ3_CM_NO_CLAIM") ? nullptr : (u32 *)e.dev(CM_CLAIM_WORDS * 4);
        if (claim) HIP_CHECK(hipMemsetAsync(claim, 0, CM_CLAIM_WORDS * 4, e.s));
        std::vector<CmEncodeJob> jobs;
        for (int32_t k = 0; k < copies; k++) {
            CmEncodeJob j{dev_addr(d), dev_addr(o + stride * (size_t)k), dev_addr(w + 4 * (size_t)k), (u32)n, debug};
            j.claim = claim ? dev_addr(claim) : 0;
            if (spill) {
                j.spill = dev_addr(spill + CM_SPILL_BYTES * (size_t)k);
                j.status = dev_addr(status + k);
                j.miss_base = CM_MISS_BASE;
                j.miss_shift = CM_MISS_SHIFT;
            }
            jobs.push_back(j);
        }
        CmEncodeJob * d_jobs = (CmEncodeJob *)e.dev(sizeof(CmEncodeJob) * jobs.size(), jobs.data(), sizeof(CmEncodeJob) * jobs.size());
        hipEvent_t e0, e1;
        HIP_CHECK(hipEventCreate(&e0));
        HIP_CHECK(hipEventCreate(&e1));
        HIP_CHECK(hipEventRecord(e0, e.s));
        cm_encode_batch(d_jobs, (u32)copies, e.s, variant);
        HIP_CHECK(hipEventRecord(e1, e.s));
        HIP_CHECK(hipStreamSynchronize(e.s));
        float ms = 0.f;
        (void)hipEventElapsedTime(&ms, e0, e1);
        (void)hipEventDestroy(e0);
        (void)hipEventDestroy(e1);
        const u32 got = e.word(w);
        if (coded) *coded = (int32_t)got;
        if (got != 0xFFFFFFFFu && got <= bz3_bound((size_t)n) && !(debug & 15u)) {
            e.down(out, o, (size_t)got);
            if (getenv("BZ3_CM_MANY_CHECK")) {
                std::vector<u8> other((size_t)got);
                for (int32_t k = 1; k < copies; k++) {
                    if (e.word(w + 4 * (size_t)k) != got) return -2.f;
                    e.down(other.data(), o + stride * (size_t)k, (size_t)got);
                    if (memcmp(other.data(), out, (size_t)got) != 0) return -2.f;
                }
            }
        }
        return ms;
    });
}

}
```

bzip3_amd/csrc/api_internal.hpp:

```cpp
#pragma once
#include <atomic>
#include <chrono>
#include <condition_variable>
#include <cstdio>
#include <cstdlib>
#include <exception>
#include <mutex>
#include <new>
#include <stdexcept>
#include <thread>
#include <type_traits>
#include <vector>

#include "../../include/bz3_hip.h"
#include "prims.hpp"
#include "sort.hpp"
#include "stages.hpp"

namespace bz3 {
namespace api {

constexpr s32 KiB65 = 65 * 1024;
constexpr s32 MiB511 = 511 * 1024 * 1024;

inline double now_ms() {
    return std::chrono::duration<double, std::milli>(std::chrono::steady_clock::now().time_since_epoch()).count();
}

inline u32 rd_le32(const u8 * p) { return (u32)p[0] | ((u32)p[1] << 8) | ((u32)p[2] << 16) | ((u32)p[3] << 24); }
inline void wr_le32(u8 * p, u32 v) {
    p[0] = (u8)v; p[1] = (u8)(v >> 8); p[2] = (u8)(v >> 16); p[3] = (u8)(v >> 24);
}

struct DeviceCtx {
    int device = 0;
    std::mutex mu;
    CrcTables * d_crc = nullptr;
    char * ws = nullptr;
    size_t ws_cap = 0;
    int cus = 256;
    static constexpr int AUX = 8;
    static constexpr int RING_SLOTS = 4;
    hipStream_t aux[AUX] = {};
    hipStream_t duo = nullptr;
    hipEvent_t ev_prep = nullptr, ev_d0[AUX] = {}, ev_d1[AUX] = {};
    bool aux_ready = false;
    hipStream_t rest = nullptr;
    hipStream_t aux_m[AUX] = {};
    int reserved_cus = 0;
    int real_cus = 0;
    static int reserved_cus_wanted() { return cu_reserve_setting(); }
    static int cu_reserve_setting() {
        static const int v = [] {
            const char * e = getenv("BZ3_HIP_CU_RESERVE");
            return e ? atoi(e) : 64;
        }();
        return v;
    }
    static void cu_masks(int cus, int reserve, std::vector<uint32_t> & side, std::vector<uint32_t> & main);
    void ensure_aux();

    std::mutex temp_mu;
    std::vector<std::pair<u8 *, size_t>> temps_free;
    std::vector<std::pair<u8 *, size_t>> temps_out;
    u8 * temp_get(size_t cap);
    void temp_put(u8 * p);
    void temp_trim();
    size_t temp_idle_bytes();

    static size_t arena_slack(size_t bytes) {
        const size_t s16 = bytes >> 4, cap = (size_t)512 << 20;
        return (s16 < cap ? s16 : cap) + ((size_t)1 << 20);
    }
    Arena arena_for(size_t bytes);
};

extern std::atomic<int> g_lean, g_cm_mode, g_keep_ws, g_front_duo;
extern std::atomic<long long> g_ws_headroom;
extern std::atomic<int> g_front_end_ring, g_arena_swaps, g_groups_running, g_groups_peak;
extern std::atomic<unsigned> g_cm_given_up, g_crc_launches, g_cm_launches, g_cm_routed_full;

inline size_t front_a_scratch_bytes(u64 n) { return (size_t)n * 30 + radix_temp_bytes(n, 9) + scan_temp_words(n / 8 + 4096) * 4 + (4u << 20); }
inline size_t front_b_scratch_bytes(u64 n) { return bwt_workspace_bytes(n) + (size_t)(n / 1024 + 4096) * 4; }
inline size_t workspace_bytes_for(u64 n) {
    size_t a = bwt_workspace_bytes(n), b = unbwt_workspace_bytes(n);
    size_t c = (size_t)n * 30 + radix_temp_bytes(n, 9) + scan_temp_words(n / 8 + 4096) * 4 + (4u << 20);
    size_t m = a > b ? a : b;
    return m > c ? m : c;
}

inline int cm_mode() {
    int m = g_cm_mode.load();
    if (m == -2) {
        const char * e = getenv("BZ3_HIP_CM_MODE");
        m = -1;
        if (e && !strcmp(e, "full")) m = CM_VARIANT_FULL;
        else if (e && !strcmp(e, "rows")) m = CM_VARIANT_ROWS;
        else if (e && !strcmp(e, "rows3")) m = CM_VARIANT_ROWS3;
#ifdef BZ3_EMU
        else if (e && !strcmp(e, "rows-test")) m = CM_VARIANT_ROWS_TEST;
#endif
        g_cm_mode.store(m);
    }
    return m;
}

inline bool lean_states() {
    int v = g_lean.load();
    if (v < 0) {
        const char * e = getenv("BZ3_HIP_LEAN");
        v = (e && *e && strcmp(e, "0")) ? 1 : 0;
        g_lean.store(v);
    }
    return v != 0;
}

inline int cm_variant_for(const DeviceCtx * ctx, size_t njobs, bool encode) {
    (void)encode;
    const int m = cm_mode();
    const size_t c = (size_t)ctx->cus;
    if (m >= 0) return m;
    if (njobs > 2 * c) return CM_VARIANT_ROWS3;
    if (njobs > c) return CM_VARIANT_ROWS;
    return CM_VARIANT_FULL;
}

inline size_t cm_scratch_bytes(size_t njobs) { return njobs * (CM_SPILL_BYTES + 256) + 4096 + CM_CLAIM_WORDS * 4 + 256; }

template <class Job, class Launch>
float run_cm_jobs(const DeviceCtx * ctx, Arena & arena, std::vector<Job> & jobs, Job * d_jobs, hipStream_t s, hipEvent_t ev0, hipEvent_t ev1, Launch && go,
                  const std::vector<char> * to_full = nullptr) {
    if (jobs.empty()) return 0.f;
    std::vector<Job> direct;
    if (to_full && cm_mode() < 0 && cm_variant_has_rows(cm_variant_for(ctx, jobs.size(), std::is_same<Job, CmEncodeJob>::value))) {
        std::vector<Job> keep;
        for (size_t i = 0; i < jobs.size(); i++) ((*to_full)[i] ? direct : keep).push_back(jobs[i]);
        if (!direct.empty()) {
            g_cm_routed_full.fetch_add((unsigned)direct.size());
            jobs.swap(keep);
        }
    }
    if (jobs.empty()) {
        float ms0 = 0.f;
        HIP_CHECK(hipMemcpyAsync(d_jobs, direct.data(), sizeof(Job) * direct.size(), hipMemcpyHostToDevice, s));
        HIP_CHECK(hipEventRecord(ev0, s));
        g_cm_launches.fetch_add(1);
        go(d_jobs, (u32)direct.size(), s, (int)CM_VARIANT_FULL);
        HIP_CHECK(hipEventRecord(ev1, s));
        HIP_CHECK(hipStreamSynchronize(s));
        (void)hipEventElapsedTime(&ms0, ev0, ev1);
        jobs.swap(direct);
        return ms0;
    }
    const int variant = cm_variant_for(ctx, jobs.size(), std::is_same<Job, CmEncodeJob>::value);
    const size_t mk = arena.mark();
    if constexpr (std::is_same<Job, CmEncodeJob>::value) {
        static const bool no_claim = getenv("BZ3_CM_NO_CLAIM") != nullptr;
        if (!no_claim) {
            u32 * claim = arena.take<u32>(CM_CLAIM_WORDS);
            HIP_CHECK(hipMemsetAsync(claim, 0, CM_CLAIM_WORDS * sizeof(u32), s));
            for (auto & j : jobs) j.claim = dev_addr(claim);
            for (auto & j : direct) j.claim = dev_addr(claim);
        }
    }
    u32 * d_status = nullptr;
    if (cm_variant_has_rows(variant)) {
        u8 * spill = arena.take<u8>(jobs.size() * CM_SPILL_BYTES);
        d_status = arena.take<u32>(jobs.size());
        HIP_CHECK(hipMemsetAsync(d_status, 0, jobs.size() * 4, s));
        for (size_t i = 0; i < jobs.size(); i++) {
            jobs[i].spill = dev_addr(spill + i * CM_SPILL_BYTES);
            jobs[i].status = dev_addr(d_status + i);
            jobs[i].miss_base = cm_variant_is_test(variant) ? 64u : CM_MISS_BASE;
            jobs[i].miss_shift = cm_variant_is_test(variant) ? 3u : CM_MISS_SHIFT;
        }
    }
    float ms = 0.f, ms2 = 0.f;
    HIP_CHECK(hipMemcpyAsync(d_jobs, jobs.data(), sizeof(Job) * jobs.size(), hipMemcpyHostToDevice, s));
    HIP_CHECK(hipEventRecord(ev0, s));
    g_cm_launches.fetch_add(1);
    go(d_jobs, (u32)jobs.size(), s, variant);
    HIP_CHECK(hipEventRecord(ev1, s));
    HIP_CHECK(hipStreamSynchronize(s));
    (void)hipEventElapsedTime(&ms, ev0, ev1);
    if (cm_variant_has_rows(variant)) {
        std::vector<u32> status(jobs.size());
        HIP_CHECK(hipMemcpyAsync(status.data(), d_status, jobs.size() * 4, hipMemcpyDeviceToHost, s));
        HIP_CHECK(hipStreamSynchronize(s));
        std::vector<Job> again;
        for (size_t i = 0; i < jobs.size(); i++)
            if (status[i]) again.push_back(jobs[i]);
        g_cm_given_up.fetch_add((unsigned)again.size());
        again.insert(again.end(), direct.begin(), direct.end());
        direct.clear();
        if (!again.empty()) {
            HIP_CHECK(hipMemcpyAsync(d_jobs, again.data(), sizeof(Job) * again.size(), hipMemcpyHostToDevice, s));
            HIP_CHECK(hipEventRecord(ev0, s));
            g_cm_launches.fetch_add(1);
            go(d_jobs, (u32)again.size(), s, (int)CM_VARIANT_FULL);
            HIP_CHECK(hipEventRecord(ev1, s));
            HIP_CHECK(hipStreamSynchronize(s));
            (void)hipEventElapsedTime(&ms2, ev0, ev1);
        }
    }
    if (!direct.empty()) {
        HIP_CHECK(hipMemcpyAsync(d_jobs, direct.data(), sizeof(Job) * direct.size(), hipMemcpyHostToDevice, s));
        HIP_CHECK(hipEventRecord(ev0, s));
        g_cm_launches.fetch_add(1);
        go(d_jobs, (u32)direct.size(), s, (int)CM_VARIANT_FULL);
        HIP_CHECK(hipEventRecord(ev1, s));
        HIP_CHECK(hipStreamSynchronize(s));
        float ms3 = 0.f;
        (void)hipEventElapsedTime(&ms3, ev0, ev1);
        ms2 += ms3;
    }
    arena.release(mk);
    return ms + ms2;
}

}
}

struct bz3_state {
    s32 block_size = 0;
    s8 last_error = BZ3_OK;
    int device = 0;
    bz3::api::DeviceCtx * ctx = nullptr;
    hipStream_t stream = nullptr;
    hipStream_t xs = nullptr;
    u8 * d_swap = nullptr;
    bool lean = false;
    bool timed = true;
    u8 * d_io = nullptr;
    size_t cap = 0;
    u32 * d_words = nullptr;
    hipEvent_t ev0 = nullptr, ev1 = nullptr;
    float t[BZ3_HIP_T_COUNT] = {0};
    bz3::BwtStats bwt;

    enum Pending { NONE, ENC_STORED, ENC_CODED, DEC_STORED, DEC_CODED, FAILED } pending = NONE;
    u8 * user = nullptr;
    u8 * b1 = nullptr, * b2 = nullptr;
    s32 size = 0, overhead = 0, result = -1;
    u32 n_cm = 0;
    const u8 * cm_in = nullptr;
    u32 cm_in_size = 0;
    u8 * side = nullptr;
    bool hold_swap = false;
    bool skip = false;
    size_t buffer_size = 0;
    u32 crc = 0;
    s32 bwt_idx = 0, model = 0, lzp_size = -1, rle_size = -1, orig_size = 0, size_before_bwt = 0, size_src = 0;
};

namespace bz3 {
namespace api {

struct DeviceGuard {
    explicit DeviceGuard(int d) { HIP_CHECK(hipSetDevice(d)); }
};

struct DrainOnUnwind {
    hipStream_t main;
    hipStream_t * side;
    int n_side;
    int live = std::uncaught_exceptions();
    ~DrainOnUnwind() {
        if (std::uncaught_exceptions() > live) {
            if (main) (void)hipStreamSynchronize(main);
            for (int k = 0; k < n_side; k++)
                if (side[k]) (void)hipStreamSynchronize(side[k]);
        }
    }
};

inline u32 read_word(hipStream_t s, const u32 * d) {
    u32 v = 0;
    HIP_CHECK(hipMemcpyAsync(&v, d, 4, hipMemcpyDeviceToHost, s));
    HIP_CHECK(hipStreamSynchronize(s));
    return v;
}

inline bool sizes_fit(size_t buffer_size, s32 lzp_size, s32 rle_size, s32 orig_size) {
    const size_t a = lzp_size < 0 ? 0 : (size_t)lzp_size, b = rle_size < 0 ? 0 : (size_t)rle_size, c = orig_size < 0 ? 0 : (size_t)orig_size;
    return a <= buffer_size && b <= buffer_size && c <= buffer_size;
}

inline size_t ws_headroom() {
    static const long long env = [] {
        const char * e = getenv("BZ3_HIP_WS_HEADROOM_MB");
        return e && *e ? (long long)strtoull(e, nullptr, 10) << 20 : (long long)4 << 30;
    }();
    const long long v = g_ws_headroom.load();
    return (size_t)(v < 0 ? env : v);
}
inline size_t ring_contexts_for(size_t free_b, size_t have, size_t need, size_t fixed, size_t ctx_bytes, size_t cap, bool lean, size_t headroom) {
    const size_t total = free_b + have;
    const size_t base = need + fixed;
    if (total <= base || !ctx_bytes) return 0;
    size_t by_share = (total - base) / 10 * 7 / ctx_bytes;
    const size_t aside = headroom + ((size_t)513 << 20) + ((size_t)64 << 20);
    const size_t room = total > base + aside ? total - base - aside : 0;
    if (!lean) {
        const size_t by_room = room / ctx_bytes;
        return by_share < by_room ? by_share : by_room;
    }
    return room / (ctx_bytes + cap);
}
void enforce_headroom(DeviceCtx * ctx, hipStream_t s);

#ifndef BZ3_FRONT_DUO_DEFAULT
#define BZ3_FRONT_DUO_DEFAULT 0
#endif
inline bool keep_workspace() {
    static const bool env_on = [] {
        const char * e = getenv("BZ3_HIP_KEEP_WS");
        return e && atoi(e) != 0;
    }();
    const int v = g_keep_ws.load();
    return v < 0 ? env_on : v != 0;
}
inline bool front_end_duo() {
    static const int env_on = [] {
        const char * e = getenv("BZ3_HIP_FRONT_DUO");
        return e ? (atoi(e) != 0 ? 1 : 0) : BZ3_FRONT_DUO_DEFAULT;
    }();
    const int v = g_front_duo.load();
    return v < 0 ? env_on != 0 : v != 0;
}
inline void lean_borrow(bz3_state * st) {
    if (st->lean && !st->d_swap) st->d_swap = st->ctx->temp_get(st->cap);
}
inline void lean_return(bz3_state * st) {
    if (st->lean && st->d_swap) {
        st->ctx->temp_put(st->d_swap);
        st->d_swap = nullptr;
    }
}
constexpr u32 CM_SIDE_BYTES = 64 * 1024;

struct SingleReq {
    bz3_state * st;
    u8 * buffer;
    size_t buffer_size;
    s32 size, orig_size;
    bool done = false;
};
struct Collector {
    std::mutex mu;
    std::condition_variable cv;
    std::vector<SingleReq *> pending[2];
    bool leader[2] = {false, false};
    size_t last_size[2] = {0, 0};
    int lonely[2] = {0, 0};
};
extern Collector g_collect;
extern std::atomic<int> g_collect_window_us;
extern std::atomic<unsigned> g_collect_batches, g_collect_largest;

int device_count();
DeviceCtx * get_ctx(int dev);
int pick_device();
bz3_state * new_state_on(int32_t block_size, int dev);
void state_release(bz3_state * st);
void encode_group(bz3_state ** sts, u8 ** bufs, const s32 * sizes, s32 n);
void decode_group(bz3_state ** sts, u8 ** bufs, const size_t * buffer_sizes, const s32 * sizes, const s32 * orig_sizes, const u8 * hdrs, s32 n);
void run_encode(bz3_state ** states, void ** buffers, s32 * sizes, s32 n, bool host);
void run_decode(bz3_state ** states, void ** buffers, const size_t * buffer_sizes, const s32 * sizes, const s32 * orig_sizes, const u8 * hdrs, s32 n, bool host);

}
}
```

bzip3_amd/csrc/lzp.hip:

```cpp
#include "prims.hpp"
#include "sort.hpp"
#include "stages.hpp"

namespace bz3 {

constexpr int LZ_HASH_BITS = 18;
constexpr int LZ_MIN = 40;
constexpr u8 LZ_ESC = 0xF2;
constexpr int LZ_DRV = 1024;
constexpr int LZ_BLOCK = 256;
constexpr int LZ_ITEMS = 16;
constexpr int LZ_ETILE = LZ_BLOCK * LZ_ITEMS;

__device__ __forceinline__ u32 lz_hash(u32 ctx) { return ((ctx >> 15) ^ ctx ^ (ctx >> 3)) & ((1u << LZ_HASH_BITS) - 1u); }
__device__ __forceinline__ bool lz_eq4(const u8 * __restrict__ a, const u8 * __restrict__ b) { return load_u32_any(a) == load_u32_any(b); }
__device__ __forceinline__ bool lz_skipped(const u32 * __restrict__ skip, u32 p) { return (skip[p >> 5] >> (p & 31)) & 1u; }

__global__ void __launch_bounds__(LZ_BLOCK) k_lzp_hash(const u8 * __restrict__ in, u32 n, u32 * __restrict__ keys) {
    const u32 k = blockIdx.x * LZ_BLOCK + threadIdx.x;
    if (k + 4 < n) keys[k] = lz_hash(load_be32(in + k));
}

__device__ __forceinline__ size_t lz_lk(u32 p) { return 2 * (size_t)p; }

// ... 135 lines not shown
    __syncthreads();
    const u64 left = (u64)m - tile_base;
    const u32 count = left < (u64)RS_TILE ? (u32)left : (u32)RS_TILE;
#pragma unroll
    for (int q = 0; q < LZB_ROUNDS; q++) {
        const u32 j = (u32)q * RS_BLOCK + threadIdx.x;
        if (j < count) {
            LzLinkRec rec{stage[3u * j], stage[3u * j + 1u], stage[3u * j + 2u]};
            out[gdelta[((rec.p - 4u) >> shift) & (LZB_RADIX - 1u)] + j] = rec;
        }
    }
}

constexpr int LZL_ITEMS = 8;
__global__ void __launch_bounds__(LZ_BLOCK) k_lzp_links_local(const LzLinkRec * __restrict__ rec, u32 m, u32 tiles, u32 * __restrict__ link) {
    const u32 tile = lzb_tile_of_block(blockIdx.x, tiles);
    if (tile >= tiles) return;
    const u64 base = (u64)tile * (LZ_BLOCK * LZL_ITEMS) + threadIdx.x;
    LzLinkRec x[LZL_ITEMS];
#pragma unroll
    for (int k = 0; k < LZL_ITEMS; k++) {
        const u64 i = base + (u64)k * LZ_BLOCK;
        x[k] = rec[i < m ? i : (u64)m - 1];
    }
#pragma unroll
    for (int k = 0; k < LZL_ITEMS; k++)
        if (base + (u64)k * LZ_BLOCK < m) *reinterpret_cast<uint2 *>(link + lz_lk(x[k].p)) = make_uint2(x[k].prev, x[k].next);
}

__device__ __forceinline__ u32 lz_candidate(u32 * __restrict__ prev, const u32 * __restrict__ skip, u32 p) {
    u32 v = prev[lz_lk(p)];
    if (v == 0 || !lz_skipped(skip, v)) return v;
    u32 steps = 0;
    while (v != 0 && lz_skipped(skip, v)) { v = prev[lz_lk(v)]; steps++; }
    if (steps > 1) {
        u32 x = prev[lz_lk(p)];
        prev[lz_lk(p)] = v;
        while (x != v && x != 0) {
            const u32 nx = prev[lz_lk(x)];
            prev[lz_lk(x)] = v;
            x = nx;
        }
    }
    return v;
}

__device__ __forceinline__ bool lz_pretest(const u8 * __restrict__ in, u32 p, u32 v) {
    const u32 a0 = load_u32_any(in + p), b0 = load_u32_any(in + v);
    const u32 a1 = load_u32_any(in + p + LZ_MIN - 4), b1 = load_u32_any(in + v + LZ_MIN - 4);
    return ((a0 ^ b0) | (a1 ^ b1)) == 0;
}

__device__ __forceinline__ u64 lz_eqmask48(const u8 * __restrict__ in, u32 p, u32 v) {
    u32 x[12];
#pragma unroll
    for (int w = 0; w < 12; w++) x[w] = load_u32_any(in + p + 4 * w) ^ load_u32_any(in + v + 4 * w);
    u64 mask = 0;
#pragma unroll
    for (int w = 0; w < 12; w++) {
        const u32 t = x[w];
        const u32 nib = ((t & 0xFFu) == 0 ? 1u : 0u) | ((t & 0xFF00u) == 0 ? 2u : 0u) | ((t & 0xFF0000u) == 0 ? 4u : 0u) | ((t & 0xFF000000u) == 0 ? 8u : 0u);
        mask |= (u64)nib << (4 * w);
    }
    return mask;
}

__global__ void __launch_bounds__(LZ_BLOCK) k_lzp_static(const u8 * __restrict__ in, u32 n, const u32 * __restrict__ prev, u32 * __restrict__ cand_bits,
                                                        u32 nwords) {
    const u32 main_end = n - (LZ_MIN + 32);
    const u64 wave_global = (u64)blockIdx.x * (LZ_BLOCK / WAVE) + wave_id();
    const u64 stride = (u64)gridDim.x * (LZ_BLOCK / WAVE);
    const u64 last = (u64)n - 1;
    for (u64 base = wave_global * (4 * WAVE); base < (u64)nwords * 32; base += stride * (4 * WAVE)) {
        u32 v[4];
        bool live[4];
#pragma unroll
        for (int q = 0; q < 4; q++) {
            const u64 p = base + (u64)q * WAVE + lane_id();
            live[q] = p >= 4 && p < main_end;
            v[q] = prev[lz_lk((u32)(p < last ? p : last))];
        }
        u32 a0[4], b0[4], a1[4], b1[4];
#pragma unroll
        for (int q = 0; q < 4; q++) {
            const u64 p = base + (u64)q * WAVE + lane_id();
            const u32 pp = live[q] ? (u32)p : 0u, vv = live[q] ? v[q] : 0u;
            a0[q] = load_u32_any(in + pp);
            b0[q] = load_u32_any(in + vv);
            a1[q] = load_u32_any(in + pp + LZ_MIN - 4);
            b1[q] = load_u32_any(in + vv + LZ_MIN - 4);
        }
#pragma unroll
        for (int q = 0; q < 4; q++) {
            const bool ev = live[q] && v[q] > 0 && ((a0[q] ^ b0[q]) | (a1[q] ^ b1[q])) == 0;
            const u64 bits = __ballot(ev);
            if (lane_id() == 0) {
                const u32 w = (u32)((base + (u64)q * WAVE) >> 5);
                if (w < nwords) cand_bits[w] = (u32)bits;
                if (w + 1 < nwords) cand_bits[w + 1] = (u32)(bits >> 32);
            }
        }
    }
}

constexpr int LZ_EV_CAP = 2048;
constexpr int LZ_WIN_WORDS = 4 * LZ_DRV;



__global__ void __launch_bounds__(LZ_DRV) k_lzp_driver(const LzpDriverJob * __restrict__ jobs) {
    const u8 * __restrict__ in = global_ptr<const u8>(jobs[blockIdx.x].in);
    const u32 n = jobs[blockIdx.x].n;
    u32 * __restrict__ prev = global_ptr<u32>(jobs[blockIdx.x].prev);
    const u32 * __restrict__ next = global_ptr<const u32>(jobs[blockIdx.x].next);
    u32 * __restrict__ cand_bits = global_ptr<u32>(jobs[blockIdx.x].cand_bits);
    const u32 nwords = jobs[blockIdx.x].nwords;
    u32 * __restrict__ skip = global_ptr<u32>(jobs[blockIdx.x].skip);
    u32 * __restrict__ mstart = global_ptr<u32>(jobs[blockIdx.x].mstart);
    u32 * __restrict__ mpos = global_ptr<u32>(jobs[blockIdx.x].mpos);
    u32 * __restrict__ mlen = global_ptr<u32>(jobs[blockIdx.x].mlen);
    LzDriverOut * __restrict__ result = global_ptr<LzDriverOut>(jobs[blockIdx.x].result);
    __shared__ u32 cq[LZ_EV_CAP];
    __shared__ u32 ev_ref[LZ_EV_CAP];
    __shared__ u64 ev_mask[LZ_EV_CAP];
    __shared__ u32 red[LZ_DRV / WAVE + 1];
    __shared__ u32 s_cur, s_heur, s_accept, s_len, s_matches;
    const u32 tid = threadIdx.x;
    const u32 main_end = n - (LZ_MIN + 32);
    u32 iterations = 0, evaluated = 0;
    if (tid == 0) { s_cur = 4; s_heur = 0; s_matches = 0; }
    __syncthreads();
    for (;;) {
        const u32 cur = s_cur;
        if (cur >= main_end) break;
        iterations++;
        const u32 w0 = (cur >> 5) & ~3u;
        u32 word[4];
        u32 cnt = 0;
        {
            const u32 wb = w0 + 4u * tid;
            uint4 q4 = make_uint4(0u, 0u, 0u, 0u);
            if (wb + 3 < nwords) q4 = *reinterpret_cast<const uint4 *>(cand_bits + wb);
            else {
                if (wb < nwords) q4.x = cand_bits[wb];
                if (wb + 1 < nwords) q4.y = cand_bits[wb + 1];
                if (wb + 2 < nwords) q4.z = cand_bits[wb + 2];
            }
            word[0] = q4.x; word[1] = q4.y; word[2] = q4.z; word[3] = q4.w;
#pragma unroll
            for (int k = 0; k < 4; k++) {
                const u32 w = wb + (u32)k;
                if (w < (cur >> 5)) word[k] = 0;
                else if (w == (cur >> 5)) word[k] &= 0xFFFFFFFFu << (cur & 31u);
                cnt += (u32)__popc(word[k]);
            }
        }
        u32 total;
        const u32 pre = block_excl_add<LZ_DRV>(cnt, red, total);
        const bool included = pre + cnt <= (u32)LZ_EV_CAP;
        const u32 cut_word = block_min<LZ_DRV>(included ? 0xFFFFFFFFu : w0 + 4u * tid, red);
        const u32 cut_events = block_min<LZ_DRV>(included ? 0xFFFFFFFFu : pre, red);
        const u32 nev = cut_events == 0xFFFFFFFFu ? total : cut_events;
        u32 window_end = cut_word == 0xFFFFFFFFu ? (w0 + (u32)LZ_WIN_WORDS) * 32u : cut_word * 32u;
        if (window_end > main_end || window_end < cur) window_end = main_end;
        if (included && cnt) {
            u32 o = pre;
#pragma unroll
            for (int k = 0; k < 4; k++) {
                u32 b = word[k];
                const u32 pos0 = (w0 + 4u * tid + (u32)k) * 32u;
                while (b) {
                    const int bit = __ffs((int)b) - 1;
                    b &= b - 1;
                    cq[o++] = pos0 + (u32)bit;
                }
            }
        }
        __syncthreads();
        if (nev == 0) {
            if (tid == 0) s_cur = window_end;
            __syncthreads();
            continue;
        }
        if (tid == 0) s_accept = 0xFFFFFFFFu;
        for (u32 b0 = 0, sub = WAVE; b0 < nev; b0 += sub, sub = LZ_DRV) {
            const u32 b1 = (nev - b0 < sub) ? nev : b0 + sub;
            evaluated += b1 - b0;
            {
                const u32 e = b0 + tid;
                if (e < b1) {
                    const u32 q = cq[e];
                    u32 v = 0;
                    if (q < main_end) {
                        v = lz_candidate(prev, skip, q);
                        if (v > 0 && !lz_pretest(in, q, v)) v = 0;
                    }
                    ev_mask[e] = v > 0 ? lz_eqmask48(in, q, v) : 0ull;
                    ev_ref[e] = v;
                }
            }
            __syncthreads();
            if (tid == 0) {
                u32 heur = s_heur;
                u32 accept = 0xFFFFFFFFu;
                for (u32 e = b0; e < b1; e++) {
                    if (ev_ref[e] == 0) continue;
                    const u32 p = cq[e];
                    const u64 mask = ev_mask[e];
                    if (heur > p && ((mask >> (heur - p)) & 0xFull) != 0xFull) continue;
                    u32 len = 4;
                    while (len < (u32)LZ_MIN && p + len < main_end && ((mask >> len) & 0xFull) == 0xFull) len += 4;
                    if (len < (u32)LZ_MIN) {
                        if (heur < p + len) heur = p + len;
                        continue;
                    }
                    accept = e;
                    break;
                }
                s_heur = heur;
                s_accept = accept;
            }
            __syncthreads();
            if (s_accept != 0xFFFFFFFFu) break;
        }
        const u32 accept = s_accept;
        if (accept == 0xFFFFFFFFu) {
            if (tid == 0) s_cur = window_end;
            __syncthreads();
            continue;
        }
        const u32 p = cq[accept], v = ev_ref[accept];
        u32 len = LZ_MIN;
        for (;;) {
            const u32 off = len + 4u * tid;
            const bool ok = (p + off < main_end) && lz_eq4(in + p + off, in + v + off);
            const u32 first_bad = block_min<LZ_DRV>(ok ? 0xFFFFFFFFu : off, red);
            if (first_bad != 0xFFFFFFFFu) { len = first_bad; break; }
            len += 4u * LZ_DRV;
        }
        if (tid == 0) {
            len += in[p + len] == in[v + len];
            len += in[p + len] == in[v + len];
            len += in[p + len] == in[v + len];
            const u32 k = s_matches;
            mpos[k] = p;
            mlen[k] = len;
            mstart[p >> 5] |= 1u << (p & 31u);
            s_len = len;
            s_matches = k + 1;
            s_cur = p + len;
        }
        __syncthreads();
        len = s_len;
        {
            const u32 a = p + 1, b = p + len;
            for (u32 w = (a >> 5) + tid; w <= ((b - 1) >> 5); w += LZ_DRV) {
                const u32 lo = w << 5;
                u32 m = 0xFFFFFFFFu;
                if (lo < a) m &= 0xFFFFFFFFu << (a - lo);
                if (lo + 32 > b) m &= 0xFFFFFFFFu >> (lo + 32 - b);
                skip[w] |= m;
            }
            for (u32 sidx = a + tid; sidx < b; sidx += LZ_DRV) {
                const u32 nq = next[lz_lk(sidx)];
                if (nq >= b && nq < main_end) atomicOr(&cand_bits[nq >> 5], 1u << (nq & 31u));
            }
        }
        __threadfence_block();
        __syncthreads();
        l1_invalidate();
    }
    if (tid == 0) {
        result->end_pos = s_cur;
        result->n_matches = s_matches;
        result->iterations = iterations;
        result->evaluated = evaluated;
    }
}

__device__ __forceinline__ u32 lz_match_len(const u32 * __restrict__ mpos, const u32 * __restrict__ mlen, u32 nm, u32 p) {
    u32 lo = 0, hi = nm;
    while (hi - lo > 1) {
        const u32 mid = (lo + hi) >> 1;
        if (mpos[mid] <= p) lo = mid; else hi = mid;
    }
    return mlen[lo];
}

__device__ __forceinline__ u32 lz_emit_count(const u8 * __restrict__ in, u32 * __restrict__ prev, const u32 * __restrict__ skip,
                                             const u32 * __restrict__ mstart, const u32 * __restrict__ mpos, const u32 * __restrict__ mlen, u32 nm, u32 p,
                                             u32 & ml) {
    ml = 0;
    if (p < 4) return 1u;
    if (lz_skipped(skip, p)) return 0u;
    if (lz_skipped(mstart, p)) {
        ml = lz_match_len(mpos, mlen, nm, p);
        return 2u + (ml - LZ_MIN) / 254u;
    }
    if (in[p] != LZ_ESC) return 1u;
    return lz_candidate(prev, skip, p) > 0 ? 2u : 1u;
}

template <int MODE>
__global__ void __launch_bounds__(LZ_BLOCK) k_lzp_emit(const u8 * __restrict__ in, u32 n, u32 * __restrict__ prev, const u32 * __restrict__ skip,
                                                      const u32 * __restrict__ mstart, const u32 * __restrict__ mpos, const u32 * __restrict__ mlen,
                                                      const LzDriverOut * __restrict__ drv, u32 * __restrict__ tile_sum, u8 * __restrict__ out) {
    __shared__ u32 lds[LZ_BLOCK / WAVE + 1];
    const u32 nm = drv->n_matches;
    const u64 base = (u64)blockIdx.x * LZ_ETILE + (u64)threadIdx.x * LZ_ITEMS;
    u32 cnt[LZ_ITEMS], ml[LZ_ITEMS];
    u32 sum = 0;
#pragma unroll 4
    for (int k = 0; k < LZ_ITEMS; k++) {
        ml[k] = 0;
        cnt[k] = (base + k < n) ? lz_emit_count(in, prev, skip, mstart, mpos, mlen, nm, (u32)(base + k), ml[k]) : 0u;
        sum += cnt[k];
    }
    u32 tot;
    const u32 pre = block_excl_add<LZ_BLOCK>(sum, lds, tot);
    if (MODE == 0) {
        if (threadIdx.x == 0) tile_sum[blockIdx.x] = tot;
        return;
    }
    u64 o = (u64)tile_sum[blockIdx.x] + pre;
#pragma unroll 1
    for (int k = 0; k < LZ_ITEMS; k++) {
        if (cnt[k] == 0) continue;
        const u32 p = (u32)(base + k);
        if (ml[k]) {
            u32 rest = ml[k] - LZ_MIN;
            out[o++] = LZ_ESC;
            while (rest >= 254u) { rest -= 254u; out[o++] = 254; }
            out[o++] = (u8)rest;
        } else {
            out[o++] = in[p];
            if (cnt[k] == 2) out[o++] = 255;
        }
    }
}

size_t lzp_encode_ctx_bytes(u64 n) { return n * 8 + (n / 32 + 8) * 12 + (n / LZ_MIN + 8) * 8 + 4096; }

void lzp_encode_prepare(const u8 * d_in, u32 n, LzpEncodeCtx & c, Arena & tmp, hipStream_t s) { lzp_encode_prepare(d_in, n, c, tmp, tmp, s); }

void lzp_encode_prepare(const u8 * d_in, u32 n, LzpEncodeCtx & c, Arena & ctx, Arena & tmp, hipStream_t s) {
    c.active = false;
    c.in = d_in;
    c.n = n;
    if (n < LZ_MIN + 32) return;
    c.active = true;
    const u32 m = n - 4;
    c.nwords = (n + 31) / 32 + 2;
    c.prev = ctx.take<u32>(2 * (size_t)n);
    c.next = c.prev + 1;
    c.skip = ctx.take<u32>(c.nwords);
    c.mstart = ctx.take<u32>(c.nwords);
    c.cand_bits = ctx.take<u32>(c.nwords);
    c.mpos = ctx.take<u32>(n / LZ_MIN + 2);
    c.mlen = ctx.take<u32>(n / LZ_MIN + 2);
    c.d_res = reinterpret_cast<LzDriverOut *>(ctx.take<u32>(8));
    {
        const size_t mk2 = tmp.mark();
        u32 * k0 = tmp.take<u32>(m);
        u32 * v0 = tmp.take<u32>(m);
        u32 * k1 = tmp.take<u32>(3 * (size_t)m + 64);
        u32 * v1 = k1 + (((size_t)m + 63) & ~(size_t)63);
        launch(k_lzp_hash, dim3((m + LZ_BLOCK - 1) / LZ_BLOCK), dim3(LZ_BLOCK), 0, s, d_in, n, k0);
        HIP_CHECK(hipMemsetAsync(c.prev, 0, 32, s));
        static const int form = [] { const char * e = getenv("BZ3_LZP_LINKS"); return e ? atoi(e) : 2; }();
        if (form == 0) {
            radix_pass<u32>(k0, k1, (const u32 *)nullptr, v1, m, 0, 0xFFFFFFFFu, 0u, tmp, s);
            radix_pass<u32>(k1, k0, (const u32 *)v1, v0, m, 8, 0xFFFFFFFFu, 0u, tmp, s);
            radix_pass<u32>(k0, k1, (const u32 *)v0, v1, m, 16, 0xFFFFFFFFu, 0u, tmp, s);
            launch(k_lzp_links, dim3((m + LZ_BLOCK - 1) / LZ_BLOCK), dim3(LZ_BLOCK), 0, s, (const u32 *)k1, (const u32 *)v1, m, c.prev);
        } else {
            static_assert(LZ_HASH_BITS == 2 * LZB_BITS, "two digits cover the hash");
            radix_pass_bits<u32, LZB_BITS>(k0, k1, (const u32 *)nullptr, v1, m, 0, 0xFFFFFFFFu, 0u, tmp, s);
            radix_pass_bits<u32, LZB_BITS>(k1, k0, (const u32 *)v1, v0, m, LZB_BITS, 0xFFFFFFFFu, 0u, tmp, s);
            if (form == 1 || m <= 2u * RS_TILE) {
                launch(k_lzp_links, dim3((m + LZ_BLOCK - 1) / LZ_BLOCK), dim3(LZ_BLOCK), 0, s, (const u32 *)k0, (const u32 *)v0, m, c.prev);
            } else {
                LzLinkRec * rec = reinterpret_cast<LzLinkRec *>(k1);
                static_assert(sizeof(LzLinkRec) == 12, "three words");
                int nbits = 0;
                for (u32 x = m - 1; x; x >>= 1) nbits++;
                const int shift = nbits > LZB_BITS ? nbits - LZB_BITS : 0;
                const u32 tiles = (m + RS_TILE - 1) / RS_TILE;
                const size_t mk3 = tmp.mark();
                u32 * hist = tmp.take<u32>((size_t)tiles * LZB_RADIX);
                const dim3 sgrid(8u * ((tiles + 7u) / 8u));
                radix_hist_bits9(v0, m, shift, hist, tiles, s);
                exclusive_scan_u32(hist, (u64)tiles * LZB_RADIX, nullptr, tmp, s);
                launch(k_lzp_bin_scatter, sgrid, dim3(RS_BLOCK), 0, s, (const u32 *)k0, (const u32 *)v0, m, shift, (const u32 *)hist, tiles, rec);
                const u32 ltiles = (m + LZ_BLOCK * LZL_ITEMS - 1) / (LZ_BLOCK * LZL_ITEMS);
                launch(k_lzp_links_local, dim3(8u * ((ltiles + 7u) / 8u)), dim3(LZ_BLOCK), 0, s, (const LzLinkRec *)rec, m, ltiles, c.prev);
                tmp.release(mk3);
            }
        }
        tmp.release(mk2);
    }
    HIP_CHECK(hipMemsetAsync(c.skip, 0, (size_t)c.nwords * 4, s));
    HIP_CHECK(hipMemsetAsync(c.mstart, 0, (size_t)c.nwords * 4, s));
    u32 grid = (c.nwords * 32u / (4 * WAVE) + (LZ_BLOCK / WAVE)) / (LZ_BLOCK / WAVE);
    if (grid > 8192) grid = 8192;
    launch(k_lzp_static, dim3(grid), dim3(LZ_BLOCK), 0, s, d_in, n, (const u32 *)c.prev, c.cand_bits, c.nwords);
}

LzpDriverJob lzp_driver_job(const LzpEncodeCtx & c) {
    return LzpDriverJob{dev_addr(c.in), dev_addr(c.prev), dev_addr(c.next), dev_addr(c.cand_bits), dev_addr(c.skip), dev_addr(c.mstart), dev_addr(c.mpos),
                        dev_addr(c.mlen), dev_addr(c.d_res), c.n, c.nwords};
}

void lzp_driver_batch(const LzpDriverJob * h_jobs, LzpDriverJob * d_jobs, u32 njobs, hipStream_t s) {
    if (!njobs) return;
    HIP_CHECK(hipMemcpyAsync(d_jobs, h_jobs, sizeof(LzpDriverJob) * njobs, hipMemcpyHostToDevice, s));
    launch(k_lzp_driver, dim3(njobs), dim3(LZ_DRV), 0, s, (const LzpDriverJob *)d_jobs);
}

s32 lzp_encode_finish(const LzpEncodeCtx & c, u8 * d_out, Arena & tmp, hipStream_t s) {
    if (!c.active) return -1;
    const size_t mk = tmp.mark();
    const u32 n = c.n;
    const u32 tiles = (n + LZ_ETILE - 1) / LZ_ETILE;
    u32 * tile_sum = tmp.take<u32>(tiles + 1);
    u32 * d_total = tmp.take<u32>(1);
    launch(k_lzp_emit<0>, dim3(tiles), dim3(LZ_BLOCK), 0, s, c.in, n, c.prev, (const u32 *)c.skip, (const u32 *)c.mstart, (const u32 *)c.mpos, (const u32 *)c.mlen,
           (const LzDriverOut *)c.d_res, tile_sum, (u8 *)nullptr);
    exclusive_scan_u32(tile_sum, tiles, d_total, tmp, s);
    u32 total = 0;
    HIP_CHECK(hipMemcpyAsync(&total, d_total, 4, hipMemcpyDeviceToHost, s));
    HIP_CHECK(hipStreamSynchronize(s));
    static const bool trace = getenv("BZ3_HIP_TRACE") != nullptr;
    if (trace) {
        LzDriverOut h;
        HIP_CHECK(hipMemcpy(&h, c.d_res, sizeof h, hipMemcpyDeviceToHost));
        fprintf(stderr, "[bz3 lzp] n=%u matches=%u driver_iterations=%u evaluated=%u out=%u\n", n, h.n_matches, h.iterations, h.evaluated, total);
    }
    s32 result = -1;
    if (total < n - 8) {
        launch(k_lzp_emit<1>, dim3(tiles), dim3(LZ_BLOCK), 0, s, c.in, n, c.prev, (const u32 *)c.skip, (const u32 *)c.mstart, (const u32 *)c.mpos,
               (const u32 *)c.mlen, (const LzDriverOut *)c.d_res, tile_sum, d_out);
        result = (s32)total;
    }
    tmp.release(mk);
    return result;
}

s32 lzp_encode(const u8 * d_in, u32 n, u8 * d_out, Arena & tmp, hipStream_t s, LzDriverOut * h_drv) {
    const size_t mk = tmp.mark();
    LzpEncodeCtx c;
    lzp_encode_prepare(d_in, n, c, tmp, s);
    s32 r = -1;
    if (h_drv) *h_drv = LzDriverOut{0u, 0u, 0u, 0u};
    if (c.active) {
        LzpDriverJob job = lzp_driver_job(c);
        LzpDriverJob * d_job = tmp.take<LzpDriverJob>(1);
        lzp_driver_batch(&job, d_job, 1, s);
        r = lzp_encode_finish(c, d_out, tmp, s);
        if (h_drv) {
            HIP_CHECK(hipMemcpyAsync(h_drv, c.d_res, sizeof *h_drv, hipMemcpyDeviceToHost, s));
            HIP_CHECK(hipStreamSynchronize(s));
        }
    }
    tmp.release(mk);
    return r;
}

void lzp_driver_geometry(u32 & event_cap, u32 & window_positions) {
    event_cap = (u32)LZ_EV_CAP;
    window_positions = (u32)LZ_WIN_WORDS * 32u;
}

constexpr int LZD_CHUNK = 16384;

__device__ __forceinline__ u64 lz_clock() {
#ifdef BZ3_EMU
    return 0;
#else
    return (u64)__builtin_readcyclecounter();
#endif
}
template <bool PROF>
__device__ __forceinline__ void lzp_decode_block(const LzpDecodeJob * __restrict__ jobs) {
    const u8 * __restrict__ in = global_ptr<const u8>(jobs[blockIdx.x].in);
    const u32 n = jobs[blockIdx.x].n;
    u8 * __restrict__ out = global_ptr<u8>(jobs[blockIdx.x].out);
    const u32 max_out = jobs[blockIdx.x].max_out;
    u32 * __restrict__ lut = global_ptr<u32>(jobs[blockIdx.x].lut);
    s32 * __restrict__ result = global_ptr<s32>(jobs[blockIdx.x].result);
    __shared__ __attribute__((aligned(16))) u8 stage[LZD_CHUNK + 32];
    __shared__ u32 red[LZ_DRV / WAVE + 1];
    __shared__ u32 s_ip, s_op, s_copy_src, s_copy_cnt, s_fail;
    const u32 tid = threadIdx.x;
    {
        uint4 * __restrict__ lz = reinterpret_cast<uint4 *>(lut);
        for (u32 k = tid; k < (u32)(LZP_LUT_WORDS / 4); k += LZ_DRV) lz[k] = make_uint4(0u, 0u, 0u, 0u);
    }
    if (tid < 4) out[tid] = in[tid];
    if (tid == 0) { s_ip = 4; s_op = 4; s_fail = 0; }
    __threadfence();
    __syncthreads();
    u64 pc_stage = 0, pc_lits = 0, pc_lane0 = 0, pc_copy = 0, pt0 = 0, pt1 = 0, pt2 = 0, pt3 = 0;
    u32 pc_trips = 0, pc_matches = 0;
    for (;;) {
        if (PROF) pt0 = lz_clock();
        const u32 ip = s_ip, op = s_op;
        if (s_fail || ip >= n || op >= max_out) break;
        const u32 chunk = (n - ip > (u32)LZD_CHUNK) ? (u32)LZD_CHUNK : n - ip;
        const u32 j0 = tid * 16u;
        u32 w[4] = {0u, 0u, 0u, 0u};
        if (j0 + 16u <= chunk) {
            const PackedU128 q = *reinterpret_cast<const PackedU128 *>(in + ip + j0);
            w[0] = q.v[0]; w[1] = q.v[1]; w[2] = q.v[2]; w[3] = q.v[3];
        } else {
            for (u32 k = 0; k < 16u; k++)
                if (j0 + k < chunk) w[k >> 2] |= (u32)in[ip + j0 + k] << (8u * (k & 3u));
        }
        if (tid < 4) stage[12 + tid] = out[op - 4 + tid];
        *reinterpret_cast<uint4 *>(&stage[16 + j0]) = make_uint4(w[0], w[1], w[2], w[3]);
        u32 first = 0xFFFFFFFFu;
#pragma unroll
        for (int k = 3; k >= 0; k--) {
            const u32 x = w[k] ^ (0x01010101u * (u32)LZ_ESC);
            const u32 z = (x - 0x01010101u) & ~x & 0x80808080u;
            if (z) first = j0 + 4u * (u32)k + ((u32)__ffs((int)z) - 1u) / 8u;
        }
        if (first != 0xFFFFFFFFu && first >= chunk) first = 0xFFFFFFFFu;
        first = block_min<LZ_DRV>(first, red);
        if (PROF) pt1 = lz_clock();
        const bool hit = first != 0xFFFFFFFFu;
        u32 lit = hit ? first : chunk;
        bool room = true;
        if (lit > max_out - op) { lit = max_out - op; room = false; }
        if (j0 < lit) {
            u32 before = *reinterpret_cast<const u32 *>(&stage[12 + j0]);
            if (j0 + 16u <= lit) {
                PackedU128 q;
                q.v[0] = w[0]; q.v[1] = w[1]; q.v[2] = w[2]; q.v[3] = w[3];
                *reinterpret_cast<PackedU128 *>(out + op + j0) = q;
            } else {
                for (u32 k = 0; j0 + k < lit; k++) out[op + j0 + k] = (u8)(w[k >> 2] >> (8u * (k & 3u)));
            }
#pragma unroll
            for (int k = 0; k < 16; k++) {
                const u32 j = j0 + (u32)k;
                if (j < lit) atomicMax(&lut[lz_hash(__builtin_bswap32(before))], op + j);
                before = (before >> 8) | (((w[k >> 2] >> (8 * (k & 3))) & 0xFFu) << 24);
            }
        }
        __threadfence_block();
        __syncthreads();
        if (PROF) pt2 = lz_clock();
        if (tid == 0) {
            u32 i2 = ip + lit, o2 = op + lit;
            s_copy_cnt = 0;
            if (hit && room && o2 < max_out) {
                const u32 ctx = ((u32)stage[12 + lit] << 24) | ((u32)stage[13 + lit] << 16) | ((u32)stage[14 + lit] << 8) | (u32)stage[15 + lit];
                const u32 cand = atomicExch(&lut[lz_hash(ctx)], o2);
                auto rd = [&](u32 x) -> u8 { return x - ip < chunk ? stage[16u + (x - ip)] : in[x]; };
                if (cand > 0) {
                    i2++;
                    if (i2 == n) s_fail = 1;
                    else if (rd(i2) != 255) {
                        u32 len = LZ_MIN;
                        for (;;) {
                            if (i2 == n) { s_fail = 1; break; }
                            const u8 b = rd(i2++);
                            len += b;
                            if (b != 254) break;
                        }
                        if (!s_fail) {
                            u64 stop = (u64)o2 + len;
                            if (stop > max_out) stop = max_out;
                            s_copy_src = cand;
                            s_copy_cnt = (u32)(stop - o2);
                        }
                    } else {
                        i2++;
                        out[o2++] = LZ_ESC;
                    }
                } else {
                    out[o2++] = rd(i2++);
                }
            }
            s_ip = i2;
            s_op = o2;
        }
        __threadfence_block();
        __syncthreads();
        if (PROF) pt3 = lz_clock();
        const u32 cnt = s_copy_cnt;
        if (cnt) {
            const u32 dst = s_op, src = s_copy_src;
            const u32 period = dst - src;
            for (u32 j = tid; j < cnt; j += LZ_DRV) out[dst + j] = out[src + (j % period)];
            __threadfence_block();
            __syncthreads();
            if (tid == 0) s_op = dst + cnt;
            __syncthreads();
        }
        if (PROF) {
            const u64 pt4 = lz_clock();
            pc_stage += pt1 - pt0; pc_lits += pt2 - pt1; pc_lane0 += pt3 - pt2; pc_copy += pt4 - pt3;
            pc_trips++;
            pc_matches += cnt ? 1u : 0u;
        }
    }
    if (tid == 0) *result = s_fail ? -1 : (s32)s_op;
    if (PROF && tid == 0)
        printf("[bz3 lzp-decode prof] n=%u trips=%u matches=%u cycles: stage+search %llu  literals+inserts+fence %llu  lane0+fence %llu  copy %llu\n", n, pc_trips, pc_matches,
               (unsigned long long)pc_stage, (unsigned long long)pc_lits, (unsigned long long)pc_lane0, (unsigned long long)pc_copy);
}
__global__ void __launch_bounds__(LZ_DRV) k_lzp_decode(const LzpDecodeJob * __restrict__ jobs) { lzp_decode_block<false>(jobs); }
__global__ void __launch_bounds__(LZ_DRV) k_lzp_decode_prof(const LzpDecodeJob * __restrict__ jobs) { lzp_decode_block<true>(jobs); }

void lzp_decode_batch(const LzpDecodeJob * h_jobs, LzpDecodeJob * d_jobs, u32 njobs, hipStream_t s) {
    if (!njobs) return;
    HIP_CHECK(hipMemcpyAsync(d_jobs, h_jobs, sizeof(LzpDecodeJob) * njobs, hipMemcpyHostToDevice, s));
    static const bool prof = [] { const char * e = getenv("BZ3_LZP_PROF"); return e && atoi(e) != 0; }();
    if (prof) launch(k_lzp_decode_prof, dim3(njobs), dim3(LZ_DRV), 0, s, (const LzpDecodeJob *)d_jobs);
    else launch(k_lzp_decode, dim3(njobs), dim3(LZ_DRV), 0, s, (const LzpDecodeJob *)d_jobs);
}

}
```

bzip3_amd/csrc/mrle.hip:

```cpp
#include "prims.hpp"
#include "sort.hpp"
#include "stages.hpp"

namespace bz3 {

constexpr int MR_BLOCK = 256;
constexpr int MR_ITEMS = 16;
constexpr int MR_TILE = MR_BLOCK * MR_ITEMS;

__device__ __forceinline__ void load16(const u8 * __restrict__ in, u64 base, u64 n, u8 (&b)[MR_ITEMS]) {
    if (base + MR_ITEMS <= n && ((reinterpret_cast<uintptr_t>(in) + base) & 15) == 0) {
        uint4 q = *reinterpret_cast<const uint4 *>(in + base);
        const u32 w[4] = {q.x, q.y, q.z, q.w};
#pragma unroll
        for (int k = 0; k < MR_ITEMS; k++) b[k] = (u8)(w[k >> 2] >> (8 * (k & 3)));
    } else {
#pragma unroll
        for (int k = 0; k < MR_ITEMS; k++) b[k] = (base + k < n) ? in[base + k] : (u8)0;
    }
}


__global__ void __launch_bounds__(MR_BLOCK) k_mrle_heads(const u8 * __restrict__ in, u32 n, u32 * __restrict__ tile_head) {
    __shared__ u32 lds[MR_BLOCK / WAVE];
    const u64 base = (u64)blockIdx.x * MR_TILE + (u64)threadIdx.x * MR_ITEMS;
    u8 b[MR_ITEMS];
    load16(in, base, n, b);
    u8 prev = (base > 0 && base < n) ? in[base - 1] : (u8)0;
    u32 best = 0;
#pragma unroll
    for (int k = 0; k < MR_ITEMS; k++) {
        const u64 i = base + k;
        if (i < n && (i == 0 || b[k] != prev)) best = (u32)i + 1;
        prev = b[k];
    }
    best = block_max<MR_BLOCK>(best, lds);
    if (threadIdx.x == 0) tile_head[blockIdx.x] = best;
}

__global__ void __launch_bounds__(1024) k_mrle_head_spine(u32 * __restrict__ tile_head, u32 tiles) {
    __shared__ u32 lds[1024 / WAVE];
    __shared__ u32 carry_s;
    if (threadIdx.x == 0) carry_s = 0;
    __syncthreads();
    for (u32 base = 0; base < tiles; base += 1024) {
        const u32 t = base + threadIdx.x;
        const u32 v = t < tiles ? tile_head[t] : 0u;
        u32 incl = block_incl_max<1024>(v, lds);
        const u32 carry = carry_s;
        if (incl < carry) incl = carry;
        u32 excl = __shfl_up(incl, 1u);
        __shared__ u32 wave_last[1024 / WAVE];
        if (lane_id() == WAVE - 1) wave_last[wave_id()] = incl;
        __syncthreads();
        if (lane_id() == 0) excl = wave_id() == 0 ? carry : wave_last[wave_id() - 1];
        if (t < tiles) tile_head[t] = excl;
        __syncthreads();
        if (threadIdx.x == 1023) carry_s = incl;
        __syncthreads();
    }
}

struct MrleView {
    u8 b[MR_ITEMS];
    u32 r[MR_ITEMS];
    bool last[MR_ITEMS];
};

template <int BLOCK>
__device__ __forceinline__ void mrle_view(const u8 * __restrict__ in, u32 n, u32 carry, u32 * lds, MrleView & v) {
    const u64 base = (u64)blockIdx.x * MR_TILE + (u64)threadIdx.x * MR_ITEMS;
    load16(in, base, n, v.b);
    u8 prev = (base > 0 && base < n) ? in[base - 1] : (u8)0;
    u32 head1[MR_ITEMS];
    u32 run = 0;
#pragma unroll
    for (int k = 0; k < MR_ITEMS; k++) {
        const u64 i = base + k;
        if (i < n && (i == 0 || v.b[k] != prev)) run = (u32)i + 1;
        head1[k] = run;
        prev = v.b[k];
    }
    u32 incl = block_incl_max<BLOCK>(run, lds);
    u32 excl = __shfl_up(incl, 1u);
    __shared__ u32 wl[BLOCK / WAVE];
    if (lane_id() == WAVE - 1) wl[wave_id()] = incl;
    __syncthreads();
    if (lane_id() == 0) excl = wave_id() == 0 ? 0u : wl[wave_id() - 1];
    if (excl < carry) excl = carry;
    __syncthreads();
    const u8 next = (base + MR_ITEMS < n) ? in[base + MR_ITEMS] : (u8)0;
#pragma unroll
    for (int k = 0; k < MR_ITEMS; k++) {
        const u64 i = base + k;
        const u32 h1 = head1[k] ? head1[k] : excl;
        v.r[k] = (i < n) ? (u32)i - (h1 - 1) : 0u;
        const u8 nb = (k + 1 < MR_ITEMS) ? v.b[(k + 1) & (MR_ITEMS - 1)] : next;
        v.last[k] = (i < n) && (i + 1 == n || nb != v.b[k]);
    }
}

__global__ void __launch_bounds__(MR_BLOCK) k_mrle_gain(const u8 * __restrict__ in, u32 n, const u32 * __restrict__ carry, s32 * __restrict__ gain) {
    __shared__ u32 lds[MR_BLOCK / WAVE];
    __shared__ s32 g[256];
    g[threadIdx.x] = 0;
    __syncthreads();
    MrleView v;
    mrle_view<MR_BLOCK>(in, n, carry[blockIdx.x], lds, v);
    const u64 base = (u64)blockIdx.x * MR_TILE + (u64)threadIdx.x * MR_ITEMS;
    s32 acc = 0;
    int sym = -1;
#pragma unroll
    for (int k = 0; k < MR_ITEMS; k++) {
        if (base + k >= n) break;
        if ((int)v.b[k] != sym) {
            if (sym >= 0 && acc != 0) atomicAdd(&g[sym], acc);
            sym = v.b[k];
            acc = 0;
        }
        acc += (v.r[k] == 0) ? -1 : ((v.r[k] % 255u) != 0u ? 1 : 0);
    }
    if (sym >= 0 && acc != 0) atomicAdd(&g[sym], acc);
    __syncthreads();
    if (g[threadIdx.x] != 0) atomicAdd(&gain[threadIdx.x], g[threadIdx.x]);
}

__device__ __forceinline__ u32 mrle_emit_count(bool flagged, u32 r, bool last) {
    if (!flagged) return 1u;
    return (r == 0 ? 1u : 0u) + ((r > 0 && r % 255u == 0) ? 1u : 0u) + (last ? 1u : 0u);
}

template <int MODE>
__global__ void __launch_bounds__(MR_BLOCK) k_mrle_emit(const u8 * __restrict__ in, u32 n, const u32 * __restrict__ carry, const s32 * __restrict__ gain,
                                                       u32 * __restrict__ tile_sum, u8 * __restrict__ out) {
    __shared__ u32 lds[MR_BLOCK / WAVE + 1];
    __shared__ u8 flag[256];
    flag[threadIdx.x] = gain[threadIdx.x] > 0;
    __syncthreads();
    MrleView v;
    mrle_view<MR_BLOCK>(in, n, carry[blockIdx.x], lds, v);
    const u64 base = (u64)blockIdx.x * MR_TILE + (u64)threadIdx.x * MR_ITEMS;
    u32 cnt = 0;
#pragma unroll
    for (int k = 0; k < MR_ITEMS; k++)
        if (base + k < n) cnt += mrle_emit_count(flag[v.b[k]], v.r[k], v.last[k]);
    u32 tot;
    u32 pre = block_excl_add<MR_BLOCK>(cnt, lds, tot);
    if (MODE == 0) {
        if (threadIdx.x == 0) tile_sum[blockIdx.x] = tot;
        return;
    }
    if (blockIdx.x == 0 && threadIdx.x < 32) {
        u8 m = 0;
#pragma unroll
        for (int j = 0; j < 8; j++) m |= (u8)(flag[threadIdx.x * 8 + j] << j);
        out[threadIdx.x] = m;
    }
    u64 o = 32ull + tile_sum[blockIdx.x] + pre;
    if (base + MR_ITEMS <= n && cnt == (u32)MR_ITEMS) {
        bool plain = true;
        PackedU128 q;
        q.v[0] = q.v[1] = q.v[2] = q.v[3] = 0u;
#pragma unroll
        for (int k = 0; k < MR_ITEMS; k++) {
            plain = plain && !flag[v.b[k]];
            q.v[k >> 2] |= (u32)v.b[k] << (8 * (k & 3));
        }
        if (plain) {
            *reinterpret_cast<PackedU128 *>(out + o) = q;
            return;
        }
    }
#pragma unroll
    for (int k = 0; k < MR_ITEMS; k++) {
        if (base + k >= n) break;
        const u8 c = v.b[k];
        const u32 r = v.r[k];
        if (!flag[c]) {
            out[o++] = c;
        } else {
            if (r == 0) out[o++] = c;
            if (r > 0 && r % 255u == 0) out[o++] = 255;
            if (v.last[k]) out[o++] = (u8)(r % 255u);
        }
    }
}

void mrle_encode_size(const u8 * d_in, u32 n, MrleEncScratch & sc, Arena & tmp, hipStream_t s) {
    const u32 tiles = n ? (n + MR_TILE - 1) / MR_TILE : 1u;
    sc.tiles = tiles;
    sc.carry = tmp.take<u32>(tiles + 1);
    sc.tile_sum = tmp.take<u32>(tiles + 1);
    sc.gain = tmp.take<s32>(256);
    sc.total = tmp.take<u32>(1);
    HIP_CHECK(hipMemsetAsync(sc.gain, 0, 256 * sizeof(s32), s));
    launch(k_mrle_heads, dim3(tiles), dim3(MR_BLOCK), 0, s, d_in, n, sc.carry);
    launch(k_mrle_head_spine, dim3(1), dim3(1024), 0, s, sc.carry, tiles);
    launch(k_mrle_gain, dim3(tiles), dim3(MR_BLOCK), 0, s, d_in, n, (const u32 *)sc.carry, sc.gain);
    launch(k_mrle_emit<0>, dim3(tiles), dim3(MR_BLOCK), 0, s, d_in, n, (const u32 *)sc.carry, (const s32 *)sc.gain, sc.tile_sum, (u8 *)nullptr);
    exclusive_scan_u32(sc.tile_sum, tiles, sc.total, tmp, s);
}

void mrle_encode_write(const u8 * d_in, u32 n, const MrleEncScratch & sc, u8 * d_out, hipStream_t s) {
    launch(k_mrle_emit<1>, dim3(sc.tiles), dim3(MR_BLOCK), 0, s, d_in, n, (const u32 *)sc.carry, (const s32 *)sc.gain, sc.tile_sum, d_out);
}

__device__ __forceinline__ u32 mr_compose(u32 f, u32 g) {
    const u32 a = (g >> (f & 1u)) & 1u;
    const u32 b = (g >> ((f >> 1) & 1u)) & 1u;
    return a | (b << 1);
}
__device__ __forceinline__ u32 mr_byte_map(u8 byte, bool flagged) { return (flagged ? 1u : 0u) | ((byte == 255) ? 2u : 0u); }

template <typename F>
__device__ __forceinline__ u32 wave_incl_compose(u32 f, F) {
    const int l = lane_id();
#pragma unroll
    for (int d = 1; d < WAVE; d <<= 1) {
        u32 t = __shfl_up(f, (unsigned)d);
        if (l >= d) f = mr_compose(t, f);
    }
    return f;
}

struct MrdView {
    u8 b[MR_ITEMS];
    u32 fmap[MR_ITEMS];
};

__device__ __forceinline__ bool mr_flagged(const u8 * __restrict__ enc, u8 c) { return (enc[c >> 3] >> (c & 7)) & 1; }

__global__ void __launch_bounds__(MR_BLOCK) k_mrd_tile_maps(const u8 * __restrict__ enc, u32 m, u32 * __restrict__ tile_map) {
    __shared__ u8 flag[256];
    __shared__ u32 wmap[MR_BLOCK / WAVE];
    flag[threadIdx.x] = mr_flagged(enc, (u8)threadIdx.x);
    __syncthreads();
    const u64 base = 32ull + (u64)blockIdx.x * MR_TILE + (u64)threadIdx.x * MR_ITEMS;
    u8 b[MR_ITEMS];
    load16(enc, base, m, b);
    u32 f = 2u;
#pragma unroll
    for (int k = 0; k < MR_ITEMS; k++)
        if (base + k < m) f = mr_compose(f, mr_byte_map(b[k], flag[b[k]]));
    f = wave_incl_compose(f, 0);
    if (lane_id() == WAVE - 1) wmap[wave_id()] = f;
    __syncthreads();
    if (threadIdx.x == 0) {
        u32 t = 2u;
        for (int w = 0; w < MR_BLOCK / WAVE; w++) t = mr_compose(t, wmap[w]);
        tile_map[blockIdx.x] = t;
    }
}

__global__ void __launch_bounds__(1024) k_mrd_spine(u32 * __restrict__ tile_map, u32 tiles) {
    __shared__ u32 wl[1024 / WAVE];
    __shared__ u32 state_s;
    if (threadIdx.x == 0) state_s = 0;
    __syncthreads();
    for (u32 base = 0; base < tiles; base += 1024) {
        const u32 t = base + threadIdx.x;
        u32 f = t < tiles ? tile_map[t] : 2u;
        u32 incl = wave_incl_compose(f, 0);
        if (lane_id() == WAVE - 1) wl[wave_id()] = incl;
        __syncthreads();
        u32 pre = 2u;
        for (int w = 0; w < wave_id(); w++) pre = mr_compose(pre, wl[w]);
        incl = mr_compose(pre, incl);
        u32 excl = __shfl_up(incl, 1u);
        if (lane_id() == 0) excl = pre;
        const u32 st0 = state_s;
        const u32 entry = (excl >> st0) & 1u;
        const u32 exit_state = (incl >> st0) & 1u;
        __syncthreads();
        if (t < tiles) tile_map[t] = entry;
        if (threadIdx.x == 1023) state_s = exit_state;
        __syncthreads();
    }
}

struct MrdItems {
    u8 b[MR_ITEMS];
    bool is_sym[MR_ITEMS];
    u32 cnt[MR_ITEMS];
    u32 sym1[MR_ITEMS];
};

template <int BLOCK>
__device__ __forceinline__ void mrd_analyse(const u8 * __restrict__ enc, u32 m, u32 entry_state, u32 sym_carry, const u8 * flag, u32 * lds,
                                            MrdItems & it, u32 & thread_cnt, u32 & last_len_pos1, u32 * st_end = nullptr) {
    __shared__ u32 wmap[BLOCK / WAVE];
    __shared__ u32 wl[BLOCK / WAVE];
    const u64 base = 32ull + (u64)blockIdx.x * MR_TILE + (u64)threadIdx.x * MR_ITEMS;
    load16(enc, base, m, it.b);
    u32 f = 2u;
#pragma unroll
    for (int k = 0; k < MR_ITEMS; k++)
        if (base + k < m) f = mr_compose(f, mr_byte_map(it.b[k], flag[it.b[k]]));
    u32 incl = wave_incl_compose(f, 0);
    if (lane_id() == WAVE - 1) wmap[wave_id()] = incl;
    __syncthreads();
    u32 pre = 2u;
    for (int w = 0; w < wave_id(); w++) pre = mr_compose(pre, wmap[w]);
    u32 excl = __shfl_up(incl, 1u);
    if (lane_id() == 0) excl = 2u;
    excl = mr_compose(pre, excl);
    u32 st = (excl >> entry_state) & 1u;
    u32 symrun = 0;
    u32 local_sym[MR_ITEMS];
    thread_cnt = 0;
    last_len_pos1 = 0;
#pragma unroll
    for (int k = 0; k < MR_ITEMS; k++) {
        const u64 i = base + k;
        const bool ok = i < m;
        const u8 c = it.b[k];
        it.is_sym[k] = ok && st == 0;
        u32 cnt = 0;
        if (ok) {
            if (st == 0) {
                symrun = (u32)i + 1;
                cnt = flag[c] ? 0u : 1u;
                st = flag[c] ? 1u : 0u;
            } else {
                cnt = (c == 255) ? 255u : (u32)c + 1u;
                st = (c == 255) ? 1u : 0u;
                last_len_pos1 = (u32)i + 1;
            }
        }
        it.cnt[k] = cnt;
        local_sym[k] = symrun;
        thread_cnt += cnt;
    }
    if (st_end) *st_end = st;
    u32 sincl = block_incl_max<BLOCK>(symrun, lds);
    u32 sexcl = __shfl_up(sincl, 1u);
    if (lane_id() == WAVE - 1) wl[wave_id()] = sincl;
    __syncthreads();
    if (lane_id() == 0) sexcl = wave_id() == 0 ? 0u : wl[wave_id() - 1];
    if (sexcl < sym_carry) sexcl = sym_carry;
    __syncthreads();
#pragma unroll
    for (int k = 0; k < MR_ITEMS; k++) it.sym1[k] = local_sym[k] ? local_sym[k] : sexcl;
}

__global__ void __launch_bounds__(MR_BLOCK) k_mrd_tile_counts(const u8 * __restrict__ enc, u32 m, const u32 * __restrict__ tile_entry, u32 * __restrict__ tile_cnt,
                                                              u32 * __restrict__ tile_sym, u32 * __restrict__ last_len1) {
    __shared__ u8 flag[256];
    __shared__ u32 lds[MR_BLOCK / WAVE + 1];
    flag[threadIdx.x] = mr_flagged(enc, (u8)threadIdx.x);
    __syncthreads();
    MrdItems it;
    u32 tc, ll, st_end;
    mrd_analyse<MR_BLOCK>(enc, m, tile_entry[blockIdx.x], 0u, flag, lds, it, tc, ll, &st_end);
    {
        const u64 b0 = 32ull + (u64)blockIdx.x * MR_TILE + (u64)threadIdx.x * MR_ITEMS;
        if (b0 < (u64)m && (u64)m <= b0 + MR_ITEMS) last_len1[1] = st_end + 1u;
    }
    u32 symrun = 0;
#pragma unroll
    for (int k = 0; k < MR_ITEMS; k++)
        if (it.is_sym[k]) symrun = (u32)(32ull + (u64)blockIdx.x * MR_TILE + (u64)threadIdx.x * MR_ITEMS + k) + 1;
    const u32 tot = block_sum<MR_BLOCK>(tc, lds);
    const u32 smax = block_max<MR_BLOCK>(symrun, lds);
    const u32 lmax = block_max<MR_BLOCK>(ll, lds);
    if (threadIdx.x == 0) {
        tile_cnt[blockIdx.x] = tot;
        tile_sym[blockIdx.x] = smax;
        if (lmax) atomicMax(last_len1, lmax);
    }
}

__global__ void __launch_bounds__(1024) k_mrd_spine2(u32 * __restrict__ tile_cnt, u32 * __restrict__ tile_sym, u32 tiles, u32 cap, u32 * __restrict__ total) {
    __shared__ u64 lds64[1024 / WAVE + 1];
    __shared__ u32 lds[1024 / WAVE];
    __shared__ u32 wl[1024 / WAVE];
    __shared__ u64 sum_s;
    __shared__ u32 sym_s;
    if (threadIdx.x == 0) { sum_s = 0; sym_s = 0; }
    __syncthreads();
    for (u32 base = 0; base < tiles; base += 1024) {
        const u32 t = base + threadIdx.x;
        const u64 c = t < tiles ? tile_cnt[t] : 0u;
        const u32 sy = t < tiles ? tile_sym[t] : 0u;
        u64 tot;
        u64 pre = block_excl_add<1024, u64>(c, lds64, tot);
        u32 sincl = block_incl_max<1024>(sy, lds);
        u32 sexcl = __shfl_up(sincl, 1u);
        if (lane_id() == WAVE - 1) wl[wave_id()] = sincl;
        __syncthreads();
        if (lane_id() == 0) sexcl = wave_id() == 0 ? 0u : wl[wave_id() - 1];
        const u64 s0 = sum_s;
        const u32 y0 = sym_s;
        if (sexcl < y0) sexcl = y0;
        if (sincl < y0) sincl = y0;
        u64 off = s0 + pre;
        if (off > cap) off = cap;
        __syncthreads();
        if (t < tiles) { tile_cnt[t] = (u32)off; tile_sym[t] = sexcl; }
        if (threadIdx.x == 1023) { sum_s = s0 + tot; sym_s = sincl; }
        __syncthreads();
    }
    if (threadIdx.x == 0) *total = (u32)(sum_s > cap ? cap : sum_s);
}

__global__ void __launch_bounds__(MR_BLOCK) k_mrd_fill(const u8 * __restrict__ enc, u32 m, const u32 * __restrict__ tile_entry, const u32 * __restrict__ tile_off,
                                                       const u32 * __restrict__ tile_sym, u8 * __restrict__ out, u32 outlen) {
    __shared__ u8 flag[256];
    __shared__ u32 lds[MR_BLOCK / WAVE + 1];
    flag[threadIdx.x] = mr_flagged(enc, (u8)threadIdx.x);
    __syncthreads();
    MrdItems it;
    u32 tc, ll;
    mrd_analyse<MR_BLOCK>(enc, m, tile_entry[blockIdx.x], tile_sym[blockIdx.x], flag, lds, it, tc, ll);
    u32 tot;
    u32 pre = block_excl_add<MR_BLOCK>(tc, lds, tot);
    u64 o = (u64)tile_off[blockIdx.x] + pre;
    if (tc == (u32)MR_ITEMS && o + MR_ITEMS <= (u64)outlen) {
        bool plain = true;
        PackedU128 q;
        q.v[0] = q.v[1] = q.v[2] = q.v[3] = 0u;
#pragma unroll
        for (int k = 0; k < MR_ITEMS; k++) {
            plain = plain && it.is_sym[k] && it.cnt[k] == 1u;
            q.v[k >> 2] |= (u32)it.b[k] << (8 * (k & 3));
        }
        if (plain) {
            *reinterpret_cast<PackedU128 *>(out + o) = q;
            return;
        }
    }
#pragma unroll 1
    for (int k = 0; k < MR_ITEMS; k++) {
        const u32 cnt = it.cnt[k];
        if (cnt == 0) continue;
        const u8 c = it.is_sym[k] ? it.b[k] : enc[it.sym1[k] - 1];
        for (u32 j = 0; j < cnt && o + j < outlen; j++) out[o + j] = c;
        o += cnt;
    }
}

__global__ void k_mrd_tail(const u8 * __restrict__ enc, u32 m, const u32 * __restrict__ tile_entry, const u32 * __restrict__ tile_sym, u32 tiles,
                           const u32 * __restrict__ last_len1, u8 * __restrict__ out, u32 outlen, u32 * __restrict__ total) {
    if (threadIdx.x != 0 || m <= 32) return;
    if (last_len1[1] == 1u) return;
    u32 st = tile_entry[tiles - 1];
    u32 sym1 = tile_sym[tiles - 1];
    const u32 start = 32u + (tiles - 1) * MR_TILE;
    for (u32 i = start; i < m; i++) {
        const u8 c = enc[i];
        if (st == 0) { sym1 = i + 1; st = mr_flagged(enc, c) ? 1u : 0u; }
        else st = (c == 255) ? 1u : 0u;
    }
    if (st != 1 || sym1 == 0) return;
    const u32 ll = *last_len1;
    const s32 pc = ll ? (s32)enc[ll - 1] : -1;
    const u32 extra = (u32)(pc + 1);
    u32 t = *total;
    const u8 c = enc[sym1 - 1];
    for (u32 j = 0; j < extra && t < outlen; j++) out[t++] = c;
    *total = t;
}

void mrle_decode(const u8 * d_enc, u32 m, u8 * d_out, u32 outlen, u32 * d_total, Arena & tmp, hipStream_t s) {
    if (m <= 32) {
        HIP_CHECK(hipMemsetAsync(d_total, 0, 4, s));
        return;
    }
    const u32 tiles = (m - 32 + MR_TILE - 1) / MR_TILE;
    size_t mk = tmp.mark();
    u32 * tile_entry = tmp.take<u32>(tiles + 1);
    u32 * tile_cnt = tmp.take<u32>(tiles + 1);
    u32 * tile_sym = tmp.take<u32>(tiles + 1);
    u32 * last_len1 = tmp.take<u32>(2);
    HIP_CHECK(hipMemsetAsync(last_len1, 0, 8, s));
    launch(k_mrd_tile_maps, dim3(tiles), dim3(MR_BLOCK), 0, s, d_enc, m, tile_entry);
    launch(k_mrd_spine, dim3(1), dim3(1024), 0, s, tile_entry, tiles);
    launch(k_mrd_tile_counts, dim3(tiles), dim3(MR_BLOCK), 0, s, d_enc, m, (const u32 *)tile_entry, tile_cnt, tile_sym, last_len1);
    launch(k_mrd_spine2, dim3(1), dim3(1024), 0, s, tile_cnt, tile_sym, tiles, outlen, d_total);
    launch(k_mrd_fill, dim3(tiles), dim3(MR_BLOCK), 0, s, d_enc, m, (const u32 *)tile_entry, (const u32 *)tile_cnt, (const u32 *)tile_sym, d_out, outlen);
    launch(k_mrd_tail, dim3(1), dim3(64), 0, s, d_enc, m, (const u32 *)tile_entry, (const u32 *)tile_sym, tiles, (const u32 *)last_len1, d_out, outlen, d_total);
    tmp.release(mk);
}

}
```

bzip3_amd/csrc/stages.hpp:

```cpp
#pragma once
#include "hipx.hpp"
#include "sort.hpp"

namespace bz3 {

struct CrcTables {
    u32 pow2[64];
    u32 lane[64];
    u32 row;
    u32 pad[3];
};
void crc_build_tables(CrcTables & t);
void crc32c_device(const u8 * d_data, u64 n, u32 init, const CrcTables * d_tables, u32 * d_scratch, hipStream_t s);
struct CrcBuf {
    u64 ptr;
    u64 size;
    u32 init;
    u32 first_seg;
};
u64 crc_many_segments(const void * ptr, u64 size);
unsigned crc32c_device_many(const CrcBuf * d_bufs, u32 n, u32 total_seg, const CrcTables * d_tables, u32 * d_crcs, hipStream_t s);

struct MrleEncScratch {
    u32 tiles = 0;
    u32 * carry = nullptr;
    u32 * tile_sum = nullptr;
    s32 * gain = nullptr;
    u32 * total = nullptr;
};
void mrle_encode_size(const u8 * d_in, u32 n, MrleEncScratch & sc, Arena & tmp, hipStream_t s);
void mrle_encode_write(const u8 * d_in, u32 n, const MrleEncScratch & sc, u8 * d_out, hipStream_t s);
void mrle_decode(const u8 * d_enc, u32 m, u8 * d_out, u32 outlen, u32 * d_total, Arena & tmp, hipStream_t s);

struct LzDriverOut {
    u32 end_pos;
    u32 n_matches;
    u32 iterations;
    u32 evaluated;
};
struct LzpEncodeCtx {
    bool active = false;
    const u8 * in = nullptr;
    u32 n = 0, nwords = 0;
    u32 *prev = nullptr, *next = nullptr, *skip = nullptr, *mstart = nullptr, *cand_bits = nullptr, *mpos = nullptr, *mlen = nullptr;
    LzDriverOut * d_res = nullptr;
};
struct LzpDriverJob {
    u64 in;
    u64 prev, next, cand_bits, skip, mstart, mpos, mlen;
    u64 result;
    u32 n, nwords;
};
size_t lzp_encode_ctx_bytes(u64 n);
void lzp_encode_prepare(const u8 * d_in, u32 n, LzpEncodeCtx & c, Arena & tmp, hipStream_t s);
void lzp_encode_prepare(const u8 * d_in, u32 n, LzpEncodeCtx & c, Arena & ctx, Arena & tmp, hipStream_t s);
LzpDriverJob lzp_driver_job(const LzpEncodeCtx & c);
void lzp_driver_batch(const LzpDriverJob * h_jobs, LzpDriverJob * d_jobs, u32 njobs, hipStream_t s);
s32 lzp_encode_finish(const LzpEncodeCtx & c, u8 * d_out, Arena & tmp, hipStream_t s);
s32 lzp_encode(const u8 * d_in, u32 n, u8 * d_out, Arena & tmp, hipStream_t s, LzDriverOut * h_drv = nullptr);
void lzp_driver_geometry(u32 & event_cap, u32 & window_positions);
struct LzpDecodeJob {
    u64 in;
    u64 out;
    u64 lut;
    u64 result;
    u32 n, max_out;
};
constexpr size_t LZP_LUT_WORDS = (size_t)1 << 18;
void lzp_decode_batch(const LzpDecodeJob * h_jobs, LzpDecodeJob * d_jobs, u32 njobs, hipStream_t s);

struct BwtStats {
    int rounds = 0;
    u64 sorted_elements = 0;
    int radix_passes = 0;
};
constexpr int BWT_ROUTE_KEEP = 40;
s32 bwt_forward(const u8 * d_in, u32 n, u8 * d_out, Arena & tmp, hipStream_t s, BwtStats * stats, u32 * d_idx = nullptr, u32 * d_outside = nullptr);
size_t bwt_workspace_bytes(u64 n);
void bwt_set_big_rounds(int k);
constexpr u32 BWT_MAX_BATCH = 4;
struct BwtBatchItem {
    const u8 * in;
    u32 n;
    u8 * out;
    u32 * d_idx;
    u32 * d_outside;
    BwtStats * stats;
    s32 idx;
};
void bwt_forward_batch(BwtBatchItem * items, u32 count, Arena & tmp, hipStream_t s);
constexpr u32 BWT_BATCH_MAX_N = 64u << 20;
u32 bwt_batch_size(const u32 * n, u32 count, size_t arena_free);
void bwt_set_batch(int b);

constexpr u32 UNBWT_LANES_PER_CU = 2048;
void bwt_inverse(const u8 * d_in, u32 n, u32 idx, u8 * d_out, Arena & tmp, hipStream_t s, u32 lanes = 0);
constexpr u32 UB_MAX_BATCH = 4;
struct UbBatchItem {
    const u8 * in;
    u8 * out;
    u32 n, idx;
};
void bwt_inverse_batch(const UbBatchItem * items, u32 count, Arena & tmp, hipStream_t s, u32 lanes = 0);
u32 unbwt_batch_size(const u32 * n, u32 count, size_t arena_free, u32 lanes);
size_t unbwt_batch_workspace_bytes(u64 n, u32 b);
size_t unbwt_workspace_bytes(u64 n);
int unbwt_log_stride(u32 rows, u32 lanes);
void unbwt_set_log_stride(int v);

constexpr u32 CM_NO_GAP = 0xFFFFFFFFu;
struct CmEncodeJob {
    u64 in;
    u64 out;
    u64 out_size;
    u32 n;
    u32 debug;
    u64 spill = 0;
    u64 status = 0;
    u32 miss_base = 0, miss_shift = 0;
    u32 gap = CM_NO_GAP, side_cap = 0;
    u64 side = 0;
    u64 claim = 0;
};
constexpr u32 CM_CLAIM_WORDS = 4096;
struct CmDecodeJob {
    u64 in;
    u64 out;
    u32 in_size;
    u32 n;
    u32 debug;
    u32 pad;
    u64 spill = 0, status = 0;
    u32 miss_base = 0, miss_shift = 0;
};
enum { CM_VARIANT_FULL = 0, CM_VARIANT_ROWS = 1, CM_VARIANT_ROWS3 = 2, CM_VARIANT_ROWS_TEST = 9  };
inline bool cm_variant_has_rows(int v) { return v != CM_VARIANT_FULL; }
inline bool cm_variant_is_test(int v) { return v == CM_VARIANT_ROWS_TEST; }
constexpr size_t CM_SPILL_BYTES = 256 * 256 * 2;
constexpr u32 CM_MISS_BASE = 1024, CM_MISS_SHIFT = 5;
void cm_encode_batch(const CmEncodeJob * d_jobs, u32 njobs, hipStream_t s, int variant = CM_VARIANT_FULL);
void cm_decode_batch(const CmDecodeJob * d_jobs, u32 njobs, hipStream_t s, int variant = CM_VARIANT_FULL, bool prof = false);

}
```

include/bz3_hip.h:

```cpp
#ifndef BZ3_HIP_H
#define BZ3_HIP_H
#include <stddef.h>
#include <stdint.h>
#include "libbz3.h"
#define BZ3_HIP 1

#ifdef __cplusplus
extern "C" {
#endif

BZIP3_API int bz3_hip_device_count(void);
BZIP3_API int bz3_hip_bind_device(int device);
BZIP3_API int bz3_hip_state_device(struct bz3_state * state);

BZIP3_API int bz3_hip_set_cm_mode(int mode);
BZIP3_API void bz3_hip_debug_bwt_big_rounds(int k);
BZIP3_API void bz3_hip_debug_set_unbwt_log_stride(int log_stride);
BZIP3_API unsigned bz3_hip_cm_blocks_given_up(void);
BZIP3_API unsigned bz3_hip_cm_blocks_routed_full(void);

BZIP3_API int bz3_hip_cm_variant_for(int device, int blocks, int encode);

BZIP3_API int bz3_hip_debug_peak_concurrent_groups(int reset);

BZIP3_API int bz3_hip_debug_front_end_ring(void);
BZIP3_API int bz3_hip_set_keep_workspace(int on);
BZIP3_API int bz3_hip_set_front_end_duo(int on);
BZIP3_API void bz3_hip_set_workspace_headroom(long long bytes);
BZIP3_API size_t bz3_hip_workspace_headroom(void);
BZIP3_API unsigned bz3_hip_debug_headroom_events(int reset, unsigned * releases);
BZIP3_API size_t bz3_hip_debug_ring_contexts(size_t free_bytes, size_t have, size_t need, size_t fixed, size_t ctx_bytes, size_t cap, int lean, size_t headroom);
BZIP3_API size_t bz3_hip_debug_arena_slack(size_t bytes);
BZIP3_API unsigned bz3_hip_debug_cm_launches(int reset);
BZIP3_API size_t bz3_hip_debug_workspace_bytes(size_t block_bytes, int which);
BZIP3_API size_t bz3_hip_debug_cached_bytes(int device);
BZIP3_API int bz3_hip_debug_arena_swap_buffers(int reset);

BZIP3_API int bz3_hip_set_lean_states(int on);
BZIP3_API void bz3_hip_release_cached_memory(void);

BZIP3_API int32_t bz3_hip_encode_block_device(struct bz3_state * state, void * buffer, int32_t size);
BZIP3_API int32_t bz3_hip_decode_block_device(struct bz3_state * state, void * buffer, size_t buffer_size, int32_t compressed_size,
                                              int32_t orig_size);
BZIP3_API void bz3_hip_encode_blocks_device(struct bz3_state * states[], void * buffers[], int32_t sizes[], int32_t n);
BZIP3_API void bz3_hip_decode_blocks_device(struct bz3_state * states[], void * buffers[], size_t buffer_sizes[], int32_t sizes[],
                                            int32_t orig_sizes[], int32_t n);

BZIP3_API int bz3_hip_compress_device(uint32_t block_size, const void * in, void * out, size_t in_size, size_t * out_size);
BZIP3_API int bz3_hip_decompress_device(const void * in, void * out, size_t in_size, size_t * out_size);
BZIP3_API int bz3_hip_frame_decoded_size_device(const void * in, size_t in_size, size_t * decoded_size);
BZIP3_API int bz3_hip_compress_device_many(uint32_t block_size, int32_t n, const void * const ins[], const size_t in_sizes[],
                                           void * const outs[], size_t out_sizes[], int rcs[]);
BZIP3_API int bz3_hip_decompress_device_many(int32_t n, const void * const ins[], const size_t in_sizes[],
                                             void * const outs[], size_t out_sizes[], int rcs[]);
BZIP3_API int bz3_hip_frame_decoded_sizes_device(int32_t n, const void * const ins[], const size_t in_sizes[],
                                                 size_t decoded_sizes[], int rcs[]);
BZIP3_API int32_t bz3_hip_debug_copy_segments(const void * src, void * dst, const uint64_t * segs, int32_t n);

BZIP3_API int bz3_hip_compress_device_planes(uint32_t block_size, uint32_t elem_size, const void * in, void * out, size_t in_size,
                                             size_t * out_size);
BZIP3_API int bz3_hip_decompress_device_planes(uint32_t elem_size, const void * in, void * out, size_t in_size, size_t * out_size);
BZIP3_API int bz3_hip_compress_device_planes_many(uint32_t block_size, int32_t n, const uint32_t elem_sizes[], const void * const ins[],
                                                  const size_t in_sizes[], void * const outs[], size_t out_sizes[], int rcs[]);
BZIP3_API int bz3_hip_decompress_device_planes_many(int32_t n, const uint32_t elem_sizes[], const void * const ins[],
                                                    const size_t in_sizes[], void * const outs[], size_t out_sizes[], int rcs[]);
BZIP3_API int32_t bz3_hip_debug_planes(const void * src, void * dst, const uint64_t * segs, int32_t n);

BZIP3_API int bz3_hip_compress_device_delta(uint32_t block_size, uint32_t elem_size, const void * in, const void * base, void * out,
                                            size_t in_size, size_t * out_size);
BZIP3_API int bz3_hip_decompress_device_delta(uint32_t elem_size, const void * in, const void * base, size_t base_size, void * out,
                                              size_t in_size, size_t * out_size);
BZIP3_API int bz3_hip_compress_device_delta_many(uint32_t block_size, int32_t n, const uint32_t elem_sizes[], const void * const ins[],
                                                 const void * const bases[], const size_t in_sizes[], void * const outs[],
                                                 size_t out_sizes[], int rcs[]);
BZIP3_API int bz3_hip_decompress_device_delta_many(int32_t n, const uint32_t elem_sizes[], const void * const ins[],
                                                   const size_t in_sizes[], const void * const bases[], const size_t base_sizes[],
                                                   void * const outs[], size_t out_sizes[], int rcs[]);
BZIP3_API int bz3_hip_crc32c_device(const void * p, size_t n, uint32_t init, uint32_t * crc);
BZIP3_API int bz3_hip_crc32c_device_many(int32_t n, const void * const * ptrs, const size_t * sizes, const uint32_t * inits, uint32_t * crcs);
BZIP3_API unsigned bz3_hip_debug_crc_launches(int reset);
BZIP3_API int32_t bz3_hip_debug_delta(const void * src, const void * base, void * dst, const uint64_t * segs, int32_t n);

BZIP3_API int bz3_hip_decompress_device_range(uint32_t elem_size, const void * in, size_t in_size, uint64_t offset, const void * base,
                                              size_t base_size, void * out, size_t * out_size);
BZIP3_API int bz3_hip_decompress_device_range_many(int32_t n, const uint32_t elem_sizes[], const void * const ins[], const size_t in_sizes[],
                                                   const uint64_t offsets[], const void * const bases[], const size_t base_sizes[],
                                                   void * const outs[], size_t out_sizes[], int rcs[]);
BZIP3_API int32_t bz3_hip_debug_range(const void * src, const void * base, void * dst, const uint64_t * segs, int32_t n);

BZIP3_API int bz3_hip_decompress_device_strided(uint32_t elem_size, const void * in, size_t in_size, uint64_t offset, uint64_t run,
                                                uint64_t stride, uint64_t count, const void * base, size_t base_size, void * out,
                                                size_t * out_size);
BZIP3_API int bz3_hip_decompress_device_strided_many(int32_t n, const uint32_t elem_sizes[], const void * const ins[], const size_t in_sizes[],
                                                     const uint64_t params[], const void * const bases[], const size_t base_sizes[],
                                                     void * const outs[], size_t out_sizes[], int rcs[]);
BZIP3_API int32_t bz3_hip_debug_strided(const void * src, const void * base, void * dst, const uint64_t * segs, int32_t n);

BZIP3_API int bz3_hip_decompress_device_select(uint32_t elem_size, const void * in, size_t in_size, uint64_t offset, uint64_t stride,
                                               uint64_t count, uint64_t m, const uint64_t * pieces, const void * base, size_t base_size,
                                               void * out, size_t * out_size);
BZIP3_API int bz3_hip_decompress_device_select_many(int32_t n, const uint32_t elem_sizes[], const void * const ins[], const size_t in_sizes[],
                                                    const uint64_t params[], const uint64_t * const pieces[], const void * const bases[],
                                                    const size_t base_sizes[], void * const outs[], size_t out_sizes[], int rcs[]);
BZIP3_API int32_t bz3_hip_debug_select(const void * src, const void * base, void * dst, const uint64_t * segs, int32_t n,
                                       const uint64_t * pieces, uint64_t n_pieces);

BZIP3_API int bz3_hip_update_device_range(uint32_t elem_size, const void * in, size_t in_size, uint64_t offset, const void * data, size_t w,
                                          const void * base, void * out, size_t * out_size);
BZIP3_API int bz3_hip_update_device_range_many(int32_t n, const uint32_t elem_sizes[], const void * const ins[], const size_t in_sizes[],
                                               const uint64_t offsets[], const void * const datas[], const size_t ws[],
                                               const void * const bases[], void * const outs[], size_t out_sizes[], int rcs[]);
BZIP3_API int32_t bz3_hip_debug_patch(const void * src, const void * base, void * dst, const uint64_t * segs, int32_t n);

enum {
    BZ3_HIP_T_CRC = 0,
    BZ3_HIP_T_RLE = 1,
    BZ3_HIP_T_LZP = 2,
    BZ3_HIP_T_BWT = 3,
    BZ3_HIP_T_CM = 4,
    BZ3_HIP_T_COPY = 5,
    BZ3_HIP_T_COUNT = 8
};
BZIP3_API void bz3_hip_last_timings(struct bz3_state * state, float ms[BZ3_HIP_T_COUNT]);
BZIP3_API void bz3_hip_last_bwt_stats(struct bz3_state * state, int32_t * rounds, int32_t * radix_passes, uint64_t * sorted_elements);

BZIP3_API void bz3_hip_set_collect_window_us(int us);
BZIP3_API unsigned bz3_hip_debug_collected_batches(int reset, unsigned * largest);

BZIP3_API uint32_t bz3_hip_stage_crc32c(const uint8_t * data, size_t n, uint32_t init);
BZIP3_API int32_t bz3_hip_stage_mrle_encode(const uint8_t * in, int32_t n, uint8_t * out);
BZIP3_API int bz3_hip_stage_mrle_decode(const uint8_t * in, uint8_t * out, int32_t outlen, int32_t maxin);
BZIP3_API int32_t bz3_hip_stage_lzp_encode(const uint8_t * in, int32_t n, uint8_t * out);
BZIP3_API int32_t bz3_hip_stage_lzp_decode(const uint8_t * in, int32_t n, uint8_t * out, int32_t max);
BZIP3_API int32_t bz3_hip_debug_lzp_encode(const uint8_t * in, int32_t n, uint8_t * out, uint32_t stats[6]);
BZIP3_API int32_t bz3_hip_stage_bwt(const uint8_t * in, uint8_t * out, int32_t n);
BZIP3_API int32_t bz3_hip_stage_unbwt(const uint8_t * in, uint8_t * out, int32_t n, int32_t idx);
BZIP3_API int32_t bz3_hip_debug_cu_masks(int cus, int reserve, uint32_t * side, uint32_t * rest);
BZIP3_API int32_t bz3_hip_debug_scan_u32(uint32_t * data, uint32_t n, uint32_t * total);
BZIP3_API int32_t bz3_hip_debug_sort_u32(const uint32_t * keys, uint32_t n, int key_bits, int digit_bits, uint32_t * sorted_keys, uint32_t * sorted_index);
BZIP3_API int32_t bz3_hip_debug_unbwt_many(const uint8_t * const * in, uint8_t * const * out, const int32_t * n, const int32_t * idx, int32_t count);
BZIP3_API int32_t bz3_hip_debug_bwt_many(const uint8_t * const * in, uint8_t * const * out, const int32_t * n, int32_t * idx_out, int32_t count);
BZIP3_API void bz3_hip_debug_set_bwt_batch(int b);
BZIP3_API float bz3_hip_stage_last_ms(void);
BZIP3_API int32_t bz3_hip_stage_cm_encode(const uint8_t * in, int32_t n, uint8_t * out);
BZIP3_API void bz3_hip_stage_cm_decode(const uint8_t * in, int32_t in_size, uint8_t * out, int32_t n);

#define BZ3_HIP_ERR_IO (-100)
BZIP3_API int bz3_hip_encode_stream(int in_fd, int out_fd, int32_t block_size, int32_t blocks_per_batch);
BZIP3_API int bz3_hip_decode_stream(int in_fd, int out_fd, int32_t blocks_per_batch);

BZIP3_API float bz3_hip_stage_cm_decode_many(const uint8_t * in, int32_t in_size, uint8_t * out, int32_t n, int32_t copies, uint64_t * counters);

BZIP3_API float bz3_hip_stage_cm_encode_many(const uint8_t * in, int32_t n, uint8_t * out, int32_t * coded, int32_t copies);

#ifdef __cplusplus
}
#endif
#endif
```

Measured before the change: 691.0.

## Batch mRLE and LZP emit kernels across up to four blocks per launch

Groups up to four blocks in the encode front end so the mRLE size/write and LZP emit/scan stages run as single 2D-grid launches, with blockIdx.y selecting the job, instead of one set of launches per block. The aim is to cut kernel launch count and host syncs, since each stage previously waited on a device-to-host size readback per block. In exchange the grid is padded to the largest block in the group, more arena scratch is held at once, and a block group falls back to the old per-block path when scratch is short.

After: 695.7 (median of 6 runs). About the same (+0.7%).

```diff
diff --git a/bzip3_amd/__init__.py b/bzip3_amd/__init__.py
--- a/bzip3_amd/__init__.py
+++ b/bzip3_amd/__init__.py
@@ -113,6 +113,8 @@
         "bz3_hip_debug_unbwt_many": (i32, [vp, vp, vp, vp, i32]),
         "bz3_hip_debug_bwt_many": (i32, [vp, vp, vp, vp, i32]),
         "bz3_hip_debug_set_bwt_batch": (None, [C.c_int]),
+        "bz3_hip_debug_set_front_batch": (None, [C.c_int]),
+        "bz3_hip_debug_front_geometry": (None, [vp]),
         "bz3_hip_stage_last_ms": (C.c_float, []),
         "bz3_hip_debug_sort_u32": (i32, [vp, u32, C.c_int, C.c_int, vp, vp]),
         "bz3_hip_debug_scan_u32": (i32, [vp, u32, vp]),
diff --git a/bzip3_amd/csrc/api_context.hip b/bzip3_amd/csrc/api_context.hip
--- a/bzip3_amd/csrc/api_context.hip
+++ b/bzip3_amd/csrc/api_context.hip
@@ -35,6 +35,7 @@
 std::atomic<long long> g_ws_headroom{-1};
 std::atomic<int> g_keep_ws{-1};
 std::atomic<int> g_front_duo{-1};
+std::atomic<int> g_front_batch{-1};
 std::atomic<int> g_groups_running{0}, g_groups_peak{0};
 Collector g_collect;
 std::atomic<int> g_collect_window_us{200};
diff --git a/bzip3_amd/csrc/api_encode.hip b/bzip3_amd/csrc/api_encode.hip
--- a/bzip3_amd/csrc/api_encode.hip
+++ b/bzip3_amd/csrc/api_encode.hip
@@ -83,14 +83,122 @@
     st->pending = bz3_state::ENC_CODED;
 }
 
-bool encode_front_b_collect(bz3_state * st, Arena & arena, const LzpEncodeCtx & c, float driver_ms, BwtBatchItem & item, u8 *& copy_to) {
+constexpr u32 FRONT_BATCH_MAX_N = 32u << 20;
+inline size_t front_run_scratch_bytes(u64 n) { return mrle_encode_scratch_bytes(n) + lzp_encode_finish_scratch_bytes(n); }
+u32 front_batch_size(const u32 * n, u32 count, size_t arena_free) {
+    const int forced = g_front_batch.load();
+    u32 want = forced > 0 ? (u32)forced : FRONT_MAX_BATCH;
+    if (want > count) want = count;
+    u32 b = 0;
+    size_t held = 0;
+    while (b < want && n[b] <= FRONT_BATCH_MAX_N) {
+        held += front_run_scratch_bytes(n[b]);
+        if (held > arena_free) break;
+        b++;
+    }
+    return b ? b : 1;
+}
+
+void encode_front_a_run(bz3_state * const * sts, u8 * const * bufs, const s32 * sizes, u32 count, Arena & arena, Arena & ctx_arena, LzpEncodeCtx * ctxs) {
+    bz3_state * live[FRONT_MAX_BATCH];
+    LzpEncodeCtx * live_ctx[FRONT_MAX_BATCH];
+    u32 nl = 0;
+    bool timed = false;
+    double t0 = now_ms();
+    for (u32 k = 0; k < count; k++) {
+        bz3_state * st = sts[k];
+        st->pending = bz3_state::FAILED;
+        st->result = -1;
+        ctxs[k].active = false;
+        if (st->skip) continue;
+        if (sizes[k] > st->block_size || sizes[k] < 0) {
+            st->last_error = BZ3_ERR_DATA_TOO_BIG;
+            continue;
+        }
+        for (float & x : st->t) x = 0.f;
+        crc32c_device(bufs[k], (u64)sizes[k], 1u, st->ctx->d_crc, st->d_words, st->xs);
+        st->user = bufs[k];
+        st->size = sizes[k];
+        if (sizes[k] < 64) {
+            launch(k_store_small, dim3(1), dim3(64), 0, st->xs, bufs[k], (u32)sizes[k], (const u32 *)(st->d_words + 1));
+            st->pending = bz3_state::ENC_STORED;
+            continue;
+        }
+        timed = timed || st->timed;
+        live[nl] = st;
+        live_ctx[nl] = &ctxs[k];
+        nl++;
+    }
+    if (!nl) return;
+    hipStream_t s = live[0]->xs;
+    if (timed) {
+        HIP_CHECK(hipStreamSynchronize(s));
+        for (u32 k = 0; k < nl; k++)
+            if (live[k]->timed) live[k]->t[BZ3_HIP_T_CRC] = (float)(now_ms() - t0) / (float)nl;
+    }
+    t0 = now_ms();
+    {
+        const u8 * in[FRONT_MAX_BATCH];
+        u32 n[FRONT_MAX_BATCH];
+        MrleEncScratch sc[FRONT_MAX_BATCH];
+        for (u32 k = 0; k < nl; k++) {
+            bz3_state * st = live[k];
+            lean_borrow(st);
+            st->b1 = st->user;
+            st->b2 = st->d_swap;
+            st->model = 0;
+            st->rle_size = 0;
+            in[k] = st->b1;
+            n[k] = (u32)st->size;
+        }
+        const size_t mk = arena.mark();
+        mrle_encode_size_many(in, n, sc, nl, arena, s);
+        u32 total[FRONT_MAX_BATCH] = {0u, 0u, 0u, 0u};
+        HIP_CHECK(hipMemcpyAsync(total, sc[0].total, sizeof(u32) * nl, hipMemcpyDeviceToHost, s));
+        HIP_CHECK(hipStreamSynchronize(s));
+        const u8 * w_in[FRONT_MAX_BATCH];
+        u8 * w_out[FRONT_MAX_BATCH];
+        u32 w_n[FRONT_MAX_BATCH];
+        MrleEncScratch w_sc[FRONT_MAX_BATCH];
+        u32 nw = 0;
+        for (u32 k = 0; k < nl; k++) {
+            bz3_state * st = live[k];
+            st->rle_size = (s32)(32u + total[k]);
+            st->n_cm = n[k];
+            if (st->rle_size < (s32)n[k]) {
+                w_in[nw] = st->b1;
+                w_out[nw] = st->b2;
+                w_n[nw] = n[k];
+                w_sc[nw] = sc[k];
+                nw++;
+                u8 * tmp = st->b1; st->b1 = st->b2; st->b2 = tmp;
+                st->n_cm = (u32)st->rle_size;
+                st->model |= 4;
+            }
+        }
+        if (nw) {
+            mrle_encode_write_many(w_in, w_n, w_sc, w_out, nw, s);
+            if (timed) HIP_CHECK(hipStreamSynchronize(s));
+        }
+        arena.release(mk);
+    }
+    for (u32 k = 0; k < nl; k++) live[k]->t[BZ3_HIP_T_RLE] = (float)(now_ms() - t0) / (float)nl;
+    t0 = now_ms();
+    for (u32 k = 0; k < nl; k++) lzp_encode_prepare(live[k]->b1, live[k]->n_cm, *live_ctx[k], ctx_arena, arena, s);
+    for (u32 k = 0; k < nl; k++) {
+        live[k]->t[BZ3_HIP_T_LZP] = (float)(now_ms() - t0) / (float)nl;
+        live[k]->pending = bz3_state::ENC_CODED;
+    }
+}
+
+bool encode_front_b_collect(bz3_state * st, Arena & arena, const LzpEncodeCtx & c, float driver_ms, BwtBatchItem & item, u8 *& copy_to, const s32 * lzp_done = nullptr) {
     if (st->pending != bz3_state::ENC_CODED) return false;
     st->pending = bz3_state::FAILED;
     hipStream_t s = st->xs;
     u8 *b1 = st->b1, *b2 = st->b2;
     u32 n = st->n_cm;
     double t0 = now_ms();
-    const s32 lzp_size = lzp_encode_finish(c, b2, arena, s);
+    const s32 lzp_size = lzp_done ? *lzp_done : lzp_encode_finish(c, b2, arena, s);
     if (lzp_size > 0 && lzp_size < (s32)n) {
         u8 * tmp = b1; b1 = b2; b2 = tmp;
         n = (u32)lzp_size;
@@ -313,6 +421,9 @@
     std::vector<bz3_state *> fb_owner;
     std::vector<u8 *> fb_copy;
     std::vector<s32> fb_slot;
+    std::vector<s32> fb_lzp;
+    std::vector<float> fb_lzp_ms;
+    std::vector<char> fb_lzp_done;
     const s32 nwin = (n + window - 1) / window;
     const s32 lag = ns - 1;
     static const bool trace_rings = getenv("BZ3_HIP_TRACE_RINGS") != nullptr;
@@ -328,9 +439,17 @@
         for (s32 i = w.w0; i < w.w1; i++) {
             sts[i]->xs = sp;
             sts[i]->hold_swap = false;
-            encode_front_a(sts[i], bufs[i], sizes[i], scr, w.slot, w.ctxs[(size_t)(i - w.w0)]);
+        }
+        for (s32 i = w.w0; i < w.w1;) {
+            u32 rn[FRONT_MAX_BATCH], avail = 0;
+            for (; avail < FRONT_MAX_BATCH && i + (s32)avail < w.w1; avail++) rn[avail] = sizes[i + avail] > 0 ? (u32)sizes[i + avail] : 0u;
+            const u32 b = front_batch_size(rn, avail, scr.cap - scr.used);
+            if (b == 1) encode_front_a(sts[i], bufs[i], sizes[i], scr, w.slot, w.ctxs[(size_t)(i - w.w0)]);
+            else encode_front_a_run(sts + i, bufs + i, sizes + i, b, scr, w.slot, &w.ctxs[(size_t)(i - w.w0)]);
+            i += (s32)b;
+        }
+        for (s32 i = w.w0; i < w.w1; i++)
             if (sts[i]->pending == bz3_state::ENC_CODED && w.ctxs[(size_t)(i - w.w0)].active) w.lz.push_back(lzp_driver_job(w.ctxs[(size_t)(i - w.w0)]));
-        }
         HIP_CHECK(hipEventRecord(ev, sp));
         if (!w.lz.empty()) {
             hipStream_t sq = lead->ctx->aux[q];
@@ -354,11 +473,43 @@
         fb_owner.clear();
         fb_copy.clear();
         fb_slot.assign((size_t)(w.w1 - w.w0), -1);
+        fb_lzp.assign((size_t)(w.w1 - w.w0), 0);
+        fb_lzp_ms.assign((size_t)(w.w1 - w.w0), 0.f);
+        fb_lzp_done.assign((size_t)(w.w1 - w.w0), 0);
+        for (s32 i = w.w0; i < w.w1;) {
+            const LzpEncodeCtx * rc[FRONT_MAX_BATCH];
+            u8 * rout[FRONT_MAX_BATCH];
+            s32 at[FRONT_MAX_BATCH];
+            u32 rn[FRONT_MAX_BATCH], avail = 0;
+            for (; i < w.w1 && avail < FRONT_MAX_BATCH; i++) {
+                if (sts[i]->pending != bz3_state::ENC_CODED || !w.ctxs[(size_t)(i - w.w0)].active) continue;
+                rc[avail] = &w.ctxs[(size_t)(i - w.w0)];
+                rout[avail] = sts[i]->b2;
+                rn[avail] = sts[i]->n_cm;
+                at[avail++] = i - w.w0;
+            }
+            for (u32 k = 0; k < avail;) {
+                const u32 b = front_batch_size(rn + k, avail - k, scr.cap - scr.used);
+                if (b > 1) {
+                    const double t0 = now_ms();
+                    s32 res[FRONT_MAX_BATCH];
+                    lzp_encode_finish_many(rc + k, rout + k, res, b, scr, sf);
+                    const float each = (float)(now_ms() - t0) / (float)b;
+                    for (u32 r = 0; r < b; r++) {
+                        fb_lzp[(size_t)at[k + r]] = res[r];
+                        fb_lzp_ms[(size_t)at[k + r]] = each;
+                        fb_lzp_done[(size_t)at[k + r]] = 1;
+                    }
+                }
+                k += b;
+            }
+        }
         for (s32 i = w.w0; i < w.w1; i++) {
             sts[i]->xs = sf;
             BwtBatchItem item{};
             u8 * copy_to = nullptr;
-            if (encode_front_b_collect(sts[i], scr, w.ctxs[(size_t)(i - w.w0)], driver_ms, item, copy_to)) {
+            const size_t wi = (size_t)(i - w.w0);
+            if (encode_front_b_collect(sts[i], scr, w.ctxs[wi], driver_ms + fb_lzp_ms[wi], item, copy_to, fb_lzp_done[wi] ? &fb_lzp[wi] : nullptr)) {
                 fb_slot[(size_t)(i - w.w0)] = (s32)fb_items.size();
                 fb_items.push_back(item);
                 fb_owner.push_back(sts[i]);
diff --git a/bzip3_amd/csrc/api_hooks.hip b/bzip3_amd/csrc/api_hooks.hip
--- a/bzip3_amd/csrc/api_hooks.hip
+++ b/bzip3_amd/csrc/api_hooks.hip
@@ -205,6 +205,13 @@
     });
 }
 BZIP3_API void bz3_hip_debug_set_bwt_batch(int b) { bwt_set_batch(b); }
+BZIP3_API void bz3_hip_debug_front_geometry(uint32_t * out) {
+    out[0] = mrle_tile_bytes();
+    out[1] = lzp_emit_tile_bytes();
+    out[2] = (uint32_t)RS_TILE;
+    out[3] = FRONT_MAX_BATCH;
+}
+BZIP3_API void bz3_hip_debug_set_front_batch(int b) { g_front_batch.store(b < 0 ? -1 : b > (int)FRONT_MAX_BATCH ? (int)FRONT_MAX_BATCH : b < 1 ? 1 : b); }
 
 BZIP3_API int32_t bz3_hip_stage_unbwt(const uint8_t * in, uint8_t * out, int32_t n, int32_t idx) {
     return stage_guard([&]() -> s32 {
diff --git a/bzip3_amd/csrc/api_internal.hpp b/bzip3_amd/csrc/api_internal.hpp
--- a/bzip3_amd/csrc/api_internal.hpp
+++ b/bzip3_amd/csrc/api_internal.hpp
@@ -76,6 +76,7 @@
 };
 
 extern std::atomic<int> g_lean, g_cm_mode, g_keep_ws, g_front_duo;
+extern std::atomic<int> g_front_batch;
 extern std::atomic<long long> g_ws_headroom;
 extern std::atomic<int> g_front_end_ring, g_arena_swaps, g_groups_running, g_groups_peak;
 extern std::atomic<unsigned> g_cm_given_up, g_crc_launches, g_cm_launches, g_cm_routed_full;
diff --git a/bzip3_amd/csrc/lzp.hip b/bzip3_amd/csrc/lzp.hip
--- a/bzip3_amd/csrc/lzp.hip
+++ b/bzip3_amd/csrc/lzp.hip
@@ -461,9 +461,9 @@
 }
 
 template <int MODE>
-__global__ void __launch_bounds__(LZ_BLOCK) k_lzp_emit(const u8 * __restrict__ in, u32 n, u32 * __restrict__ prev, const u32 * __restrict__ skip,
-                                                      const u32 * __restrict__ mstart, const u32 * __restrict__ mpos, const u32 * __restrict__ mlen,
-                                                      const LzDriverOut * __restrict__ drv, u32 * __restrict__ tile_sum, u8 * __restrict__ out) {
+__device__ __forceinline__ void lzp_emit_body(const u8 * __restrict__ in, u32 n, u32 * __restrict__ prev, const u32 * __restrict__ skip,
+                                              const u32 * __restrict__ mstart, const u32 * __restrict__ mpos, const u32 * __restrict__ mlen,
+                                              const LzDriverOut * __restrict__ drv, u32 * __restrict__ tile_sum, u8 * __restrict__ out) {
     __shared__ u32 lds[LZ_BLOCK / WAVE + 1];
     const u32 nm = drv->n_matches;
     const u64 base = (u64)blockIdx.x * LZ_ETILE + (u64)threadIdx.x * LZ_ITEMS;
@@ -496,6 +496,30 @@
             if (cnt[k] == 2) out[o++] = 255;
         }
     }
+}
+template <int MODE>
+__global__ void __launch_bounds__(LZ_BLOCK) k_lzp_emit(const u8 * __restrict__ in, u32 n, u32 * __restrict__ prev, const u32 * __restrict__ skip,
+                                                      const u32 * __restrict__ mstart, const u32 * __restrict__ mpos, const u32 * __restrict__ mlen,
+                                                      const LzDriverOut * __restrict__ drv, u32 * __restrict__ tile_sum, u8 * __restrict__ out) {
+    lzp_emit_body<MODE>(in, n, prev, skip, mstart, mpos, mlen, drv, tile_sum, out);
+}
+
+struct LzpEmitBatch {
+    struct Job {
+        const u8 * in;
+        u32 * prev;
+        const u32 *skip, *mstart, *mpos, *mlen;
+        const LzDriverOut * drv;
+        u32 * tile_sum;
+        u8 * out;
+        u32 n, tiles;
+    } job[FRONT_MAX_BATCH];
+};
+template <int MODE>
+__global__ void __launch_bounds__(LZ_BLOCK) k_lzp_emit_many(LzpEmitBatch b) {
+    const LzpEmitBatch::Job & j = b.job[blockIdx.y];
+    if (blockIdx.x >= j.tiles) return;
+    lzp_emit_body<MODE>(j.in, j.n, j.prev, j.skip, j.mstart, j.mpos, j.mlen, j.drv, j.tile_sum, j.out);
 }
 
 size_t lzp_encode_ctx_bytes(u64 n) { return n * 8 + (n / 32 + 8) * 12 + (n / LZ_MIN + 8) * 8 + 4096; }
@@ -605,6 +629,63 @@
     return result;
 }
 
+u32 lzp_emit_tile_bytes() { return (u32)LZ_ETILE; }
+
+size_t lzp_encode_finish_scratch_bytes(u64 n) {
+    const u64 tiles = n / LZ_ETILE + 1;
+    return (size_t)(tiles + 1) * 4 + scan_temp_words(tiles) * 4 + 6 * 256;
+}
+
+void lzp_encode_finish_many(const LzpEncodeCtx * const * c, u8 * const * d_out, s32 * result, u32 count, Arena & tmp, hipStream_t s) {
+    if (count == 0 || count > FRONT_MAX_BATCH) throw HipError{hipErrorUnknown, "LZP batch of a size the job table does not hold", __FILE__, __LINE__};
+    const size_t mk = tmp.mark();
+    u32 * d_totals = tmp.take<u32>(count);
+    LzpEmitBatch b;
+    u32 * tables[FRONT_MAX_BATCH];
+    u32 * tots[FRONT_MAX_BATCH];
+    u64 words[FRONT_MAX_BATCH];
+    u32 most = 0;
+    for (u32 k = 0; k < count; k++) {
+        const LzpEncodeCtx & x = *c[k];
+        if (!x.active) throw HipError{hipErrorUnknown, "LZP batch with an inactive context", __FILE__, __LINE__};
+        const u32 tiles = (x.n + LZ_ETILE - 1) / LZ_ETILE;
+        tables[k] = tmp.take<u32>(tiles + 1);
+        tots[k] = d_totals + k;
+        words[k] = tiles;
+        b.job[k] = LzpEmitBatch::Job{x.in, x.prev, x.skip, x.mstart, x.mpos, x.mlen, x.d_res, tables[k], nullptr, x.n, tiles};
+        most = tiles > most ? tiles : most;
+    }
+    for (u32 k = count; k < FRONT_MAX_BATCH; k++) b.job[k] = b.job[0];
+    launch(k_lzp_emit_many<0>, dim3(most, count), dim3(LZ_BLOCK), 0, s, b);
+    exclusive_scan_u32_many(tables, words, tots, count, tmp, s);
+    u32 total[FRONT_MAX_BATCH] = {0u, 0u, 0u, 0u};
+    HIP_CHECK(hipMemcpyAsync(total, d_totals, sizeof(u32) * count, hipMemcpyDeviceToHost, s));
+    HIP_CHECK(hipStreamSynchronize(s));
+    static const bool trace = getenv("BZ3_HIP_TRACE") != nullptr;
+    LzpEmitBatch w;
+    u32 nw = 0, most_w = 0;
+    for (u32 k = 0; k < count; k++) {
+        if (trace) {
+            LzDriverOut h;
+            HIP_CHECK(hipMemcpy(&h, c[k]->d_res, sizeof h, hipMemcpyDeviceToHost));
+            fprintf(stderr, "[bz3 lzp] n=%u matches=%u driver_iterations=%u evaluated=%u out=%u\n", c[k]->n, h.n_matches, h.iterations, h.evaluated, total[k]);
+        }
+        result[k] = -1;
+        if (total[k] < c[k]->n - 8) {
+            w.job[nw] = b.job[k];
+            w.job[nw].out = d_out[k];
+            most_w = w.job[nw].tiles > most_w ? w.job[nw].tiles : most_w;
+            nw++;
+            result[k] = (s32)total[k];
+        }
+    }
+    if (nw) {
+        for (u32 k = nw; k < FRONT_MAX_BATCH; k++) w.job[k] = w.job[0];
+        launch(k_lzp_emit_many<1>, dim3(most_w, nw), dim3(LZ_BLOCK), 0, s, w);
+    }
+    tmp.release(mk);
+}
+
 s32 lzp_encode(const u8 * d_in, u32 n, u8 * d_out, Arena & tmp, hipStream_t s, LzDriverOut * h_drv) {
     const size_t mk = tmp.mark();
     LzpEncodeCtx c;
diff --git a/bzip3_amd/csrc/mrle.hip b/bzip3_amd/csrc/mrle.hip
--- a/bzip3_amd/csrc/mrle.hip
+++ b/bzip3_amd/csrc/mrle.hip
@@ -21,7 +21,7 @@
 }
 
 
-__global__ void __launch_bounds__(MR_BLOCK) k_mrle_heads(const u8 * __restrict__ in, u32 n, u32 * __restrict__ tile_head) {
+__device__ __forceinline__ void mrle_heads_body(const u8 * __restrict__ in, u32 n, u32 * __restrict__ tile_head) {
     __shared__ u32 lds[MR_BLOCK / WAVE];
     const u64 base = (u64)blockIdx.x * MR_TILE + (u64)threadIdx.x * MR_ITEMS;
     u8 b[MR_ITEMS];
@@ -37,8 +37,9 @@
     best = block_max<MR_BLOCK>(best, lds);
     if (threadIdx.x == 0) tile_head[blockIdx.x] = best;
 }
-
-__global__ void __launch_bounds__(1024) k_mrle_head_spine(u32 * __restrict__ tile_head, u32 tiles) {
+__global__ void __launch_bounds__(MR_BLOCK) k_mrle_heads(const u8 * __restrict__ in, u32 n, u32 * __restrict__ tile_head) { mrle_heads_body(in, n, tile_head); }
+
+__device__ __forceinline__ void mrle_head_spine_body(u32 * __restrict__ tile_head, u32 tiles) {
     __shared__ u32 lds[1024 / WAVE];
     __shared__ u32 carry_s;
     if (threadIdx.x == 0) carry_s = 0;
@@ -60,6 +61,7 @@
         __syncthreads();
     }
 }
+__global__ void __launch_bounds__(1024) k_mrle_head_spine(u32 * __restrict__ tile_head, u32 tiles) { mrle_head_spine_body(tile_head, tiles); }
 
 struct MrleView {
     u8 b[MR_ITEMS];
@@ -100,7 +102,7 @@
     }
 }
 
-__global__ void __launch_bounds__(MR_BLOCK) k_mrle_gain(const u8 * __restrict__ in, u32 n, const u32 * __restrict__ carry, s32 * __restrict__ gain) {
+__device__ __forceinline__ void mrle_gain_body(const u8 * __restrict__ in, u32 n, const u32 * __restrict__ carry, s32 * __restrict__ gain) {
     __shared__ u32 lds[MR_BLOCK / WAVE];
     __shared__ s32 g[256];
     g[threadIdx.x] = 0;
@@ -124,6 +126,9 @@
     __syncthreads();
     if (g[threadIdx.x] != 0) atomicAdd(&gain[threadIdx.x], g[threadIdx.x]);
 }
+__global__ void __launch_bounds__(MR_BLOCK) k_mrle_gain(const u8 * __restrict__ in, u32 n, const u32 * __restrict__ carry, s32 * __restrict__ gain) {
+    mrle_gain_body(in, n, carry, gain);
+}
 
 __device__ __forceinline__ u32 mrle_emit_count(bool flagged, u32 r, bool last) {
     if (!flagged) return 1u;
@@ -133,57 +138,44 @@
 template <int MODE>
 __global__ void __launch_bounds__(MR_BLOCK) k_mrle_emit(const u8 * __restrict__ in, u32 n, const u32 * __restrict__ carry, const s32 * __restrict__ gain,
                                                        u32 * __restrict__ tile_sum, u8 * __restrict__ out) {
-    __shared__ u32 lds[MR_BLOCK / WAVE + 1];
-    __shared__ u8 flag[256];
-    flag[threadIdx.x] = gain[threadIdx.x] > 0;
-    __syncthreads();
-    MrleView v;
-    mrle_view<MR_BLOCK>(in, n, carry[blockIdx.x], lds, v);
-    const u64 base = (u64)blockIdx.x * MR_TILE + (u64)threadIdx.x * MR_ITEMS;
-    u32 cnt = 0;
-#pragma unroll
-    for (int k = 0; k < MR_ITEMS; k++)
-        if (base + k < n) cnt += mrle_emit_count(flag[v.b[k]], v.r[k], v.last[k]);
-    u32 tot;
-    u32 pre = block_excl_add<MR_BLOCK>(cnt, lds, tot);
-    if (MODE == 0) {
-        if (threadIdx.x == 0) tile_sum[blockIdx.x] = tot;
-        return;
-    }
-    if (blockIdx.x == 0 && threadIdx.x < 32) {
-        u8 m = 0;
-#pragma unroll
-        for (int j = 0; j < 8; j++) m |= (u8)(flag[threadIdx.x * 8 + j] << j);
-        out[threadIdx.x] = m;
-    }
-    u64 o = 32ull + tile_sum[blockIdx.x] + pre;
-    if (base + MR_ITEMS <= n && cnt == (u32)MR_ITEMS) {
-        bool plain = true;
-        PackedU128 q;
-        q.v[0] = q.v[1] = q.v[2] = q.v[3] = 0u;
-#pragma unroll
-        for (int k = 0; k < MR_ITEMS; k++) {
-            plain = plain && !flag[v.b[k]];
-            q.v[k >> 2] |= (u32)v.b[k] << (8 * (k & 3));
-        }
-        if (plain) {
-            *reinterpret_cast<PackedU128 *>(out + o) = q;
-            return;
-        }
-    }
-#pragma unroll
-    for (int k = 0; k < MR_ITEMS; k++) {
-        if (base + k >= n) break;
-        const u8 c = v.b[k];
-        const u32 r = v.r[k];
-        if (!flag[c]) {
-            out[o++] = c;
-        } else {
-            if (r == 0) out[o++] = c;
-            if (r > 0 && r % 255u == 0) out[o++] = 255;
-            if (v.last[k]) out[o++] = (u8)(r % 255u);
-        }
-    }
+#include "mrle_emit_body.hpp"
+}
+
+struct MrleBatch {
+    struct Job {
+        const u8 * in;
+        u32 * carry;
+        u32 * tile_sum;
+        s32 * gain;
+        u8 * out;
+        u32 n, tiles;
+    } job[FRONT_MAX_BATCH];
+};
+__global__ void __launch_bounds__(MR_BLOCK) k_mrle_heads_many(MrleBatch b) {
+    const MrleBatch::Job & j = b.job[blockIdx.y];
+    if (blockIdx.x >= j.tiles) return;
+    mrle_heads_body(j.in, j.n, j.carry);
+}
+__global__ void __launch_bounds__(1024) k_mrle_head_spine_many(MrleBatch b) {
+    const MrleBatch::Job & j = b.job[blockIdx.y];
+    mrle_head_spine_body(j.carry, j.tiles);
+}
+__global__ void __launch_bounds__(MR_BLOCK) k_mrle_gain_many(MrleBatch b) {
+    const MrleBatch::Job & j = b.job[blockIdx.y];
+    if (blockIdx.x >= j.tiles) return;
+    mrle_gain_body(j.in, j.n, j.carry, j.gain);
+}
+template <int MODE>
+__global__ void __launch_bounds__(MR_BLOCK) k_mrle_emit_many(MrleBatch b) {
+    const MrleBatch::Job & j = b.job[blockIdx.y];
+    if (blockIdx.x >= j.tiles) return;
+    const u8 * __restrict__ in = j.in;
+    const u32 n = j.n;
+    const u32 * __restrict__ carry = j.carry;
+    const s32 * __restrict__ gain = j.gain;
+    u32 * __restrict__ tile_sum = j.tile_sum;
+    u8 * __restrict__ out = j.out;
+#include "mrle_emit_body.hpp"
 }
 
 void mrle_encode_size(const u8 * d_in, u32 n, MrleEncScratch & sc, Arena & tmp, hipStream_t s) {
@@ -203,6 +195,59 @@
 
 void mrle_encode_write(const u8 * d_in, u32 n, const MrleEncScratch & sc, u8 * d_out, hipStream_t s) {
     launch(k_mrle_emit<1>, dim3(sc.tiles), dim3(MR_BLOCK), 0, s, d_in, n, (const u32 *)sc.carry, (const s32 *)sc.gain, sc.tile_sum, d_out);
+}
+
+static MrleBatch mrle_batch(const u8 * const * d_in, const u32 * n, const MrleEncScratch * sc, u8 * const * d_out, u32 count, u32 & most) {
+    if (count == 0 || count > FRONT_MAX_BATCH) throw HipError{hipErrorUnknown, "mRLE batch of a size the job table does not hold", __FILE__, __LINE__};
+    MrleBatch b;
+    most = 0;
+    for (u32 k = 0; k < FRONT_MAX_BATCH; k++) {
+        const u32 j = k < count ? k : 0;
+        b.job[k] = MrleBatch::Job{d_in[j], sc[j].carry, sc[j].tile_sum, sc[j].gain, d_out ? d_out[j] : nullptr, n[j], sc[j].tiles};
+        if (k < count && sc[j].tiles > most) most = sc[j].tiles;
+    }
+    return b;
+}
+
+u32 mrle_tile_bytes() { return (u32)MR_TILE; }
+
+size_t mrle_encode_scratch_bytes(u64 n) {
+    const u64 tiles = n / MR_TILE + 1;
+    return (size_t)(tiles + 1) * 8 + 256 * sizeof(s32) + scan_temp_words(tiles) * 4 + 8 * 256;
+}
+
+void mrle_encode_size_many(const u8 * const * d_in, const u32 * n, MrleEncScratch * sc, u32 count, Arena & tmp, hipStream_t s) {
+    if (count == 0 || count > FRONT_MAX_BATCH) throw HipError{hipErrorUnknown, "mRLE batch of a size the job table does not hold", __FILE__, __LINE__};
+    s32 * gains = tmp.take<s32>((size_t)256 * count);
+    u32 * totals = tmp.take<u32>(count);
+    u32 * tables[FRONT_MAX_BATCH];
+    u32 * tots[FRONT_MAX_BATCH];
+    u64 words[FRONT_MAX_BATCH];
+    for (u32 k = 0; k < count; k++) {
+        const u32 tiles = n[k] ? (n[k] + MR_TILE - 1) / MR_TILE : 1u;
+        sc[k].tiles = tiles;
+        sc[k].carry = tmp.take<u32>(tiles + 1);
+        sc[k].tile_sum = tmp.take<u32>(tiles + 1);
+        sc[k].gain = gains + (size_t)256 * k;
+        sc[k].total = totals + k;
+        tables[k] = sc[k].tile_sum;
+        tots[k] = sc[k].total;
+        words[k] = tiles;
+    }
+    u32 most = 0;
+    const MrleBatch b = mrle_batch(d_in, n, sc, nullptr, count, most);
+    HIP_CHECK(hipMemsetAsync(gains, 0, (size_t)256 * count * sizeof(s32), s));
+    launch(k_mrle_heads_many, dim3(most, count), dim3(MR_BLOCK), 0, s, b);
+    launch(k_mrle_head_spine_many, dim3(1, count), dim3(1024), 0, s, b);
+    launch(k_mrle_gain_many, dim3(most, count), dim3(MR_BLOCK), 0, s, b);
+    launch(k_mrle_emit_many<0>, dim3(most, count), dim3(MR_BLOCK), 0, s, b);
+    exclusive_scan_u32_many(tables, words, tots, count, tmp, s);
+}
+
+void mrle_encode_write_many(const u8 * const * d_in, const u32 * n, const MrleEncScratch * sc, u8 * const * d_out, u32 count, hipStream_t s) {
+    u32 most = 0;
+    const MrleBatch b = mrle_batch(d_in, n, sc, d_out, count, most);
+    launch(k_mrle_emit_many<1>, dim3(most, count), dim3(MR_BLOCK), 0, s, b);
 }
 
 __device__ __forceinline__ u32 mr_compose(u32 f, u32 g) {
diff --git a/bzip3_amd/csrc/mrle_emit_body.hpp b/bzip3_amd/csrc/mrle_emit_body.hpp
--- /dev/null
+++ b/bzip3_amd/csrc/mrle_emit_body.hpp
@@ -0,0 +1,51 @@
+    __shared__ u32 lds[MR_BLOCK / WAVE + 1];
+    __shared__ u8 flag[256];
+    flag[threadIdx.x] = gain[threadIdx.x] > 0;
+    __syncthreads();
+    MrleView v;
+    mrle_view<MR_BLOCK>(in, n, carry[blockIdx.x], lds, v);
+    const u64 base = (u64)blockIdx.x * MR_TILE + (u64)threadIdx.x * MR_ITEMS;
+    u32 cnt = 0;
+#pragma unroll
+    for (int k = 0; k < MR_ITEMS; k++)
+        if (base + k < n) cnt += mrle_emit_count(flag[v.b[k]], v.r[k], v.last[k]);
+    u32 tot;
+    u32 pre = block_excl_add<MR_BLOCK>(cnt, lds, tot);
+    if (MODE == 0) {
+        if (threadIdx.x == 0) tile_sum[blockIdx.x] = tot;
+        return;
+    }
+    if (blockIdx.x == 0 && threadIdx.x < 32) {
+        u8 m = 0;
+#pragma unroll
+        for (int j = 0; j < 8; j++) m |= (u8)(flag[threadIdx.x * 8 + j] << j);
+        out[threadIdx.x] = m;
+    }
+    u64 o = 32ull + tile_sum[blockIdx.x] + pre;
+    if (base + MR_ITEMS <= n && cnt == (u32)MR_ITEMS) {
+        bool plain = true;
+        PackedU128 q;
+        q.v[0] = q.v[1] = q.v[2] = q.v[3] = 0u;
+#pragma unroll
+        for (int k = 0; k < MR_ITEMS; k++) {
+            plain = plain && !flag[v.b[k]];
+            q.v[k >> 2] |= (u32)v.b[k] << (8 * (k & 3));
+        }
+        if (plain) {
+            *reinterpret_cast<PackedU128 *>(out + o) = q;
+            return;
+        }
+    }
+#pragma unroll
+    for (int k = 0; k < MR_ITEMS; k++) {
+        if (base + k >= n) break;
+        const u8 c = v.b[k];
+        const u32 r = v.r[k];
+        if (!flag[c]) {
+            out[o++] = c;
+        } else {
+            if (r == 0) out[o++] = c;
+            if (r > 0 && r % 255u == 0) out[o++] = 255;
+            if (v.last[k]) out[o++] = (u8)(r % 255u);
+        }
+    }
diff --git a/bzip3_amd/csrc/stages.hpp b/bzip3_amd/csrc/stages.hpp
--- a/bzip3_amd/csrc/stages.hpp
+++ b/bzip3_amd/csrc/stages.hpp
@@ -30,6 +30,11 @@
 };
 void mrle_encode_size(const u8 * d_in, u32 n, MrleEncScratch & sc, Arena & tmp, hipStream_t s);
 void mrle_encode_write(const u8 * d_in, u32 n, const MrleEncScratch & sc, u8 * d_out, hipStream_t s);
+constexpr u32 FRONT_MAX_BATCH = 4;
+void mrle_encode_size_many(const u8 * const * d_in, const u32 * n, MrleEncScratch * sc, u32 count, Arena & tmp, hipStream_t s);
+void mrle_encode_write_many(const u8 * const * d_in, const u32 * n, const MrleEncScratch * sc, u8 * const * d_out, u32 count, hipStream_t s);
+u32 mrle_tile_bytes();
+size_t mrle_encode_scratch_bytes(u64 n);
 void mrle_decode(const u8 * d_enc, u32 m, u8 * d_out, u32 outlen, u32 * d_total, Arena & tmp, hipStream_t s);
 
 struct LzDriverOut {
@@ -57,6 +62,9 @@
 LzpDriverJob lzp_driver_job(const LzpEncodeCtx & c);
 void lzp_driver_batch(const LzpDriverJob * h_jobs, LzpDriverJob * d_jobs, u32 njobs, hipStream_t s);
 s32 lzp_encode_finish(const LzpEncodeCtx & c, u8 * d_out, Arena & tmp, hipStream_t s);
+void lzp_encode_finish_many(const LzpEncodeCtx * const * c, u8 * const * d_out, s32 * result, u32 count, Arena & tmp, hipStream_t s);
+u32 lzp_emit_tile_bytes();
+size_t lzp_encode_finish_scratch_bytes(u64 n);
 s32 lzp_encode(const u8 * d_in, u32 n, u8 * d_out, Arena & tmp, hipStream_t s, LzDriverOut * h_drv = nullptr);
 void lzp_driver_geometry(u32 & event_cap, u32 & window_positions);
 struct LzpDecodeJob {
diff --git a/include/bz3_hip.h b/include/bz3_hip.h
--- a/include/bz3_hip.h
+++ b/include/bz3_hip.h
@@ -141,6 +141,8 @@
 BZIP3_API int32_t bz3_hip_debug_unbwt_many(const uint8_t * const * in, uint8_t * const * out, const int32_t * n, const int32_t * idx, int32_t count);
 BZIP3_API int32_t bz3_hip_debug_bwt_many(const uint8_t * const * in, uint8_t * const * out, const int32_t * n, int32_t * idx_out, int32_t count);
 BZIP3_API void bz3_hip_debug_set_bwt_batch(int b);
+BZIP3_API void bz3_hip_debug_set_front_batch(int b);
+BZIP3_API void bz3_hip_debug_front_geometry(uint32_t * out);
 BZIP3_API float bz3_hip_stage_last_ms(void);
 BZIP3_API int32_t bz3_hip_stage_cm_encode(const uint8_t * in, int32_t n, uint8_t * out);
 BZIP3_API void bz3_hip_stage_cm_decode(const uint8_t * in, int32_t in_size, uint8_t * out, int32_t n);
```
